# tatsy/opengl-raytracer

Measured on AMD Instinct MI355X. Metric: Mrays/s at 1920x1080, 8 bounces, higher is better.
Workload: dtype f32

## Files before the change

opengl-raytracer_amd/csrc/glrtx.hip:

```cpp
#include "glrtx.h"

#include <hip/hip_runtime.h>

#include <algorithm>
#include <cmath>
#include <cstdarg>
#include <cstdio>
#include <cstdlib>
#include <cstring>
#include <new>
#include <limits>
#include <string>
#include <vector>

#include "glrt_host.h"
#include "pt_kernel.hip.h"
#include "accumulate.hip.h"
#include "lbvh.hip.h"
#include "sahl.hip.h"
#include "refit.hip.h"
#include "query.hip.h"
#include "features.hip.h"
#include "denoise.hip.h"
#include "variance.hip.h"
// ... 1012 lines not shown
    k.fn = kWgwfKernels[trav][k.adapt][L.req.count_rays(c)];
    k.name = kWgwfNames[k.vol ? 2 : k.vine ? 0 : 1][k.adapt];
    k.lds = wgwf_lds_base(c) + (k.compact ? c->sc.n_crank * (int)sizeof(uint2) : 0);
    if (k.lds > 160 * 1024) return fail(c, GLRTX_EDEVICE, "wgwf kernel needs %d B of LDS (> 160 KiB)", k.lds);
    if (k.lds > 64 * 1024) HIP_TRY(c, hipFuncSetAttribute((const void *)k.fn, hipFuncAttributeMaxDynamicSharedMemorySize, k.lds));
    k.per_cu = 0;
    HIP_TRY(c, hipOccupancyMaxActiveBlocksPerMultiprocessor(&k.per_cu, k.fn, kBlockThreads, k.lds));
    k.per_cu = std::max(1, std::min(k.per_cu, GLRTX_WGWF_WAVES));
    if (const char *v = std::getenv("GLRTX_WGS_PER_CU")) k.per_cu = std::max(1, std::min(k.per_cu, std::atoi(v)));
    k.wg_slots = (size_t)c->n_cu * (size_t)k.per_cu;
    return GLRTX_OK;
}

void wgwf_shape(const glrtx_ctx *c, const WgwfLaunch &L, bool overlapped, bool is_fed, int share, bool device_busy, int &block_paths, int &grid) {
    const int n_frames = L.n_frames, fed_cap = L.f.fed_cap, n_samples = L.p->n_samples;
    const size_t total = L.total;
    const int resident = std::max(1, L.k.per_cu / std::max(share, 1)) * c->n_cu;
    const size_t work = total * (size_t)(is_fed ? std::max(n_frames, std::min(16, fed_cap)) : n_frames);
    block_paths = kWgPathsMax;
    if (overlapped && device_busy) { block_paths = 256; while (block_paths < kWgPathsMax && (size_t)resident * block_paths < work) block_paths *= 2; }
    else {
        const size_t tenths = (n_samples > 1 || (n_frames == 1 && !is_fed)) ? 39 : 19;
        while (block_paths > 512 && work * 10 < tenths * (size_t)resident * block_paths) block_paths /= 2;
        while (block_paths > 256 && work < (size_t)resident * block_paths) block_paths /= 2;
    }
    if (const char *v = std::getenv("GLRTX_BLOCK_PATHS")) { const int x = std::atoi(v); if (x >= 256 && x <= kWgPathsMax && (x & (x - 1)) == 0) block_paths = x; }
    grid = std::max(1, (int)std::min<size_t>((size_t)resident, (work + block_paths - 1) / block_paths));
}

int wgwf_pipe_slot(glrtx_ctx *c, WgwfLaunch &L) {
    WgwfLaunch::Form &f = L.f;
    const int n_frames = L.n_frames;
    const size_t frame_bytes = L.frame_bytes;
    glrtx_ctx::PipeSlot *&slot = L.slot = nullptr;
    int &pipe_busy = L.pipe_busy = 0, &block_paths = L.block_paths = 0, &grid = L.grid = 0;
    if (f.piped) {
        const bool fed = f.fed, busy = f.busy;
        wgwf_shape(c, L, !fed, fed, 1, busy, block_paths, grid);
        size_t slot_state_entries = (size_t)grid * block_paths;
        if (!fed) { int b2 = 0, g2 = 0; wgwf_shape(c, L, true, false, 1, !busy, b2, g2); slot_state_entries = std::max(slot_state_entries, (size_t)g2 * b2); }
        const size_t per_slot = (fed ? 0 : (size_t)kWfStatePlanes * slot_state_entries * sizeof(float4)) + (size_t)grid * kWgQueueF4 * sizeof(float4) + (fed ? 0 : frame_bytes);
        unsigned allowed = (unsigned)std::min<size_t>(c->pipe_slots, frames_budget(c) / std::max<size_t>(per_slot, 1));
        if (fed) allowed = std::min(allowed, kFedSlots);
        c->st.pipe_slots = (int32_t)allowed;
        if (allowed >= 1) {
            unsigned pick = c->pipe_next % allowed;
            for (unsigned k = 0; k < allowed; k++) {
                glrtx_ctx::PipeSlot &o = c->pipe[(c->pipe_next + k) % allowed];
                if (!o.used || hipEventQuery(o.acc_done) == hipSuccess) { pick = (c->pipe_next + k) % allowed; break; }
            }
            (void)hipGetLastError();
            c->pipe_next = pick + 1;
            slot = &c->pipe[pick];
            for (unsigned k = 0; k < kPipeSlots; k++)
                if (k != pick && c->pipe[k].used && hipEventQuery(c->pipe[k].render_done) == hipErrorNotReady) pipe_busy++;
            (void)hipGetLastError();
            if (c->pipe_share > 1 && pipe_busy > 0 && !fed) wgwf_shape(c, L, true, false, c->pipe_share, busy, block_paths, grid);
            bool ok = true;
            if (fed && slot->used) (void)hipEventSynchronize(slot->render_done);
            if (fed && slot->chunk_bytes != frame_bytes) {
                if (slot->used) (void)hipEventSynchronize(slot->acc_done);
                for (auto &ch : slot->chunks) dev_free(ch);
                std::memset(slot->feed_h->chunks, 0, sizeof slot->feed_h->chunks);
                slot->chunk_bytes = frame_bytes;
            }
            if (!fed) ok = ok && ensure(c, slot->state, (size_t)kWfStatePlanes * slot_state_entries * sizeof(float4)) == GLRTX_OK;
            ok = ok && ensure(c, slot->queues, (size_t)grid * kWgQueueF4 * sizeof(float4)) == GLRTX_OK;
            if (fed) ok = ok && ensure(c, slot->feed_d, sizeof(FeedDev)) == GLRTX_OK && feed_ensure_chunks(c, *slot, 0, n_frames, f.fed_cap, frame_bytes) == GLRTX_OK;
            else ok = ok && ensure(c, slot->planes, frame_bytes) == GLRTX_OK;
            if (!ok) {
                (void)hipGetLastError();
                c->err.clear();
                if (slot->used) (void)hipEventSynchronize(slot->acc_done);
                for (unsigned k = pick; k < kPipeSlots; k++) {
                    glrtx_ctx::PipeSlot &o = c->pipe[k];
                    if (o.used) (void)hipEventSynchronize(o.acc_done);
                    dev_free(o.state); dev_free(o.planes); dev_free(o.queues); dev_free(o.feed_d);
                    for (auto &ch : o.chunks) dev_free(ch);
                    if (o.feed_h) std::memset(o.feed_h->chunks, 0, sizeof o.feed_h->chunks);
                    o.chunk_bytes = 0;
                    o.used = false;
                }
                (void)hipGetLastError();
                c->pipe_slots = pick;
                if (pick == 0) c->pipeline = false;
                c->st.pipe_slots = (int32_t)pick;
                slot = nullptr;
                pipe_busy = 0;
            }
        }
        if (!slot) { f.piped = false; f.fed = false; }
    }
    if (!slot) {
        if (n_frames > frames_cap(c, L.p, 1)) return fail(c, GLRTX_ENOMEM, "glrtx_render_frames: %d frames exceed the frames-in-flight memory budget", n_frames);
        wgwf_shape(c, L, false, false, 1, f.busy, block_paths, grid);
    }
    if (slot) c->st.pipe_resident_max = std::max<int32_t>(c->st.pipe_resident_max, pipe_busy + 1);
    return GLRTX_OK;
}

int wgwf_args(glrtx_ctx *c, WgwfLaunch &L) {
    const glrtx_params *p = L.p;
    glrtx_ctx::PipeSlot *const slot = L.slot;
    const bool fed = L.f.fed, adapt = L.k.adapt, moments = L.req.kind == RenderReq::Moments;
    const int n_frames = L.n_frames, grid = L.grid;
    int rc;
    L.ctx_state = !slot || fed;
    L.stateBuf = L.ctx_state ? &c->wfState : &slot->state;
    L.queueBuf = slot ? &slot->queues : &c->wfQ;
    L.planeBuf = slot ? &slot->planes : &c->wfPlanes;
    L.workPtr = (unsigned *)(slot ? slot->work.p : c->work.p);
    L.rstream = slot ? slot->stream : c->stream;
    L.state_entries = (size_t)grid * (size_t)L.block_paths;
    L.state_bytes = (size_t)kWfStatePlanes * L.state_entries * sizeof(float4);
    if ((rc = ensure(c, *L.stateBuf, L.state_bytes))) return rc;
    if ((rc = ensure(c, *L.queueBuf, (size_t)grid * kWgQueueF4 * sizeof(float4)))) return rc;
    WfArgs &w = L.w;
    std::memset(&w, 0, sizeof w);
    w.state = (float4 *)L.stateBuf->p;
    w.ids = L.state_entries;
    c->st.wf_state_mib = (int32_t)((L.state_bytes + ((size_t)1 << 20) - 1) >> 20);
    w.total = (int)L.total;
    w.tiles8_x = L.tiles8_x;
    w.refill_min = kRefillMin;
    if (const char *v = std::getenv("GLRTX_REFILL_MIN")) w.refill_min = std::max(1, std::min(64, std::atoi(v)));
    w.n_frames = fed ? std::max(L.f.fed_cap, 2) : n_frames;
    w.tiles_per_frame = (int)(L.total >> 6);
    if (fed) {
        FeedHost *fh = slot->feed_h;
        for (int i = 0; i < n_frames; i++) fh->seeds[i] = make_float2(L.seeds_xy[2 * i], L.seeds_xy[2 * i + 1]);
        __atomic_store_n(&fh->frames_pub, (unsigned)n_frames, __ATOMIC_RELEASE);
        w.feed_host = slot->feed_h_dev;
        w.feed_dev = (FeedDev *)slot->feed_d.p;
        w.feed_plane_f4 = L.plane_f4;
        w.feed_margin = 64 * 4 * grid;
        if (const char *v = std::getenv("GLRTX_FEED_MARGIN")) w.feed_margin = std::max(0, std::atoi(v));
    } else {
        if (n_frames > 1) {
            if ((rc = ensure(c, c->wfSeeds, (size_t)n_frames * sizeof(float2)))) return rc;
            HIP_TRY(c, hipMemcpyAsync(c->wfSeeds.p, L.seeds_xy, (size_t)n_frames * sizeof(float2), hipMemcpyHostToDevice, c->stream));
            w.seeds = (const float2 *)c->wfSeeds.p;
            w.seeds_in_lds = n_frames <= kLdsSeeds ? 1 : 0;
        }
        if (n_frames > 1 || slot || adapt || moments) {
            if ((rc = ensure(c, *L.planeBuf, (size_t)std::max(L.n_planes, 1) * L.plane_f4 * sizeof(float4)))) return rc;
            w.planes = (float4 *)L.planeBuf->p;
        }
    }
    w.block_paths = L.block_paths;
    w.gss_div = (slot && !fed) ? 0 : 4 * grid;
    if (const char *v = std::getenv("GLRTX_GSS_DIV")) w.gss_div = std::max(0, std::atoi(v));
    w.suspend_max = kSuspendMax;
    if (const char *v = std::getenv("GLRTX_SUSPEND_MAX")) w.suspend_max = std::max(0, std::min(64, std::atoi(v)));
    w.trip_limit = (int)std::min<long long>(INT32_MAX, 64ll * std::max(p->n_samples, 1) * (p->max_depth + 2) + 64);
    if (L.k.vol) w.trip_limit = (int)std::min<long long>(INT32_MAX, 64ll * std::max(p->n_samples, 1) * 9 * (p->max_depth + 2) + 64);
    if (const char *v = std::getenv("GLRTX_TRIP_LIMIT")) w.trip_limit = std::max(1, std::atoi(v));
    w.err = c->guard_dev;
    return GLRTX_OK;
}

int wgwf_check(glrtx_ctx *c, const WgwfLaunch &L) {
    const glrtx_params *p = L.p;
    const glrtx_ctx::PipeSlot *const slot = L.slot;
    const WfArgs &w = L.w;
    const bool fed = L.f.fed, moments = L.req.kind == RenderReq::Moments;
    const int n_frames = L.n_frames, grid = L.grid, block_paths = L.block_paths, fed_cap = L.f.fed_cap;
    const size_t state_entries = L.state_entries, total = L.total, max_id = L.ids - 1;
    const size_t max_sidx = (size_t)kWfSetPlanes * state_entries + (size_t)grid * block_paths - 1;
    const size_t slice_f4 = 2 * (size_t)2 * 2 * block_paths  + (2 * (size_t)block_paths * sizeof(unsigned) + 15) / 16 ;
    static_assert(kWgSuspendAt + (size_t)kSuspendF4 * kBlockThreads == kWgQueueF4, "the suspend area closes a workgroup's slice");
    bool ok = slice_f4 <= kWgSuspendAt && max_id < (size_t)WF_INVALID && 2 * max_sidx + 1 < (size_t)WF_INVALID && (size_t)grid * block_paths <= state_entries &&
              (size_t)kWfStatePlanes * state_entries * sizeof(float4) < ((size_t)1 << 32) && (block_paths & (block_paths - 1)) == 0 && block_paths >= 256 &&
              block_paths <= kWgPathsMax && slice_f4 <= kWgQueueF4 && L.queueBuf->bytes >= (size_t)grid * kWgQueueF4 * sizeof(float4) &&
              L.stateBuf->bytes >= L.state_bytes && w.ids == state_entries && grid >= 1 && (size_t)grid <= L.k.wg_slots &&
              p->max_depth <= kWfDepthMax && p->n_samples <= kWfSampleMax && L.workPtr != nullptr;
    if (L.k.vol) ok = ok && p->n_samples <= kWfVolSampleMax && c->ext_flags == GLRTX_EXT_VOLUME && c->have_volume && c->vol.density != nullptr &&
                      c->vol.temperature != nullptr && c->n_spheres == 0 && !L.k.vine && L.k.fetch == 0 && !L.k.compact;
    if (!fed && n_frames > 1) ok = ok && c->wfSeeds.bytes >= (size_t)n_frames * sizeof(float2);
    if (w.planes) ok = ok && L.planeBuf->bytes >= (size_t)std::max(L.n_planes, 1) * L.plane_f4 * sizeof(float4);
    if (L.k.adapt) ok = ok && !fed && !slot && w.planes && c->ad_selected && c->ad_tiles == (int)(total >> 6) && c->adList.bytes >= (total >> 6) * sizeof(int) &&
                        c->adMask.bytes >= (total >> 6) && c->adHalf.bytes >= (size_t)c->ad_pitch * c->owned_rows && c->ad_pitch == c->pitch_bytes;
    if (moments) ok = ok && !fed && !slot && w.planes && c->mmM.p && c->mm_pitch == c->pitch_bytes && c->mm_rows == c->owned_rows &&
                      c->mmM.bytes >= c->pitch_bytes * (size_t)c->owned_rows;
    if (fed) ok = ok && n_frames >= 1 && n_frames <= fed_cap && fed_cap <= kFeedMaxFrames && slot->feed_d.bytes >= sizeof(FeedDev) && w.feed_host != nullptr &&
                  slot->chunks[(n_frames - 1) / kFeedChunkFrames].p != nullptr && slot->chunk_bytes == L.frame_bytes;
    if (!ok) return fail(c, GLRTX_EDEVICE, "internal: wgwf launch shapes inconsistent (ids %zu, max id %zu, grid %d of %zu slots (%d per CU), block_paths %d, frames %d, fed %d)", L.ids, max_id,
                         grid, L.k.wg_slots, L.k.per_cu, block_paths, n_frames, (int)fed);
    return GLRTX_OK;
}

template <class Src, class Sink>
void accumulate_launch(glrtx_ctx *c, const accumulate::Image &im, const Src &src, const Sink &sink) {
    hipLaunchKernelGGL(accumulate::entry(src, sink), dim3((im.width + 63) / 64, (im.rows + 3) / 4), dim3(256), 0, c->stream, im, src, sink);
}

int wgwf_issue(glrtx_ctx *c, const WgwfLaunch &L) {
    const glrtx_params *p = L.p;
    glrtx_ctx::PipeSlot *const slot = L.slot;
    const WfArgs &w = L.w;
    const bool fed = L.f.fed, adapt = L.k.adapt, vol = L.k.vol;
    const int n_frames = L.n_frames, n_planes = L.n_planes;
    const hipStream_t rstream = L.rstream;
    glrtx_ctx::LaunchRec *rec = nullptr;
    int rc;
    if ((rc = next_launch_rec(c, rec))) return rc;
    if (slot && slot->used) HIP_TRY(c, hipStreamWaitEvent(rstream, slot->acc_done, 0));
    if (L.ctx_state && c->state_used) HIP_TRY(c, hipStreamWaitEvent(rstream, c->state_done, 0));
    HIP_TRY(c, hipMemsetAsync(L.workPtr, 0, sizeof(unsigned), rstream));
    if (fed) {
        hipLaunchKernelGGL(feed_prefill_kernel, dim3(1), dim3(64), 0, rstream, (FeedDev *)slot->feed_d.p, (const FeedHost *)slot->feed_h_dev, n_frames);
        HIP_TRY(c, hipGetLastError());
    }
    HIP_TRY(c, hipEventRecord(rec->ev0, rstream));
    c->last_kernel = L.k.name;
    c->counters_stale = c->counters_stale || L.req.count_rays(c);
    const VolArgs va = vol ? c->vol : VolArgs{};
    hipLaunchKernelGGL(L.k.fn, dim3(L.grid), dim3(kBlockThreads), L.k.lds, rstream, L.a, w, L.workPtr, (float4 *)L.queueBuf->p, adapt ? (const int *)c->adList.p : nullptr,
                       adapt ? (const unsigned *)c->adCount.p : nullptr, va);
    HIP_TRY(c, hipGetLastError());
#ifdef GLRTX_RAY_LOG
    g_dbg_last = {L.a, w, L.k.lds, L.grid, (float4 *)L.queueBuf->p, L.k.fetch};
#endif
    HIP_TRY(c, hipEventRecord(rec->evm, rstream));
    if (L.ctx_state) { HIP_TRY(c, hipEventRecord(c->state_done, rstream)); c->state_used = true; }
    if (slot) {
        HIP_TRY(c, hipEventRecord(slot->render_done, rstream));
        HIP_TRY(c, hipStreamWaitEvent(c->stream, slot->render_done, 0));
        HIP_TRY(c, hipEventRecord(rec->eva, c->stream));
    }
    rec->has_eva = slot != nullptr;
    const bool pres = L.req.presents(c);
    const bool pres_fused = pres && (fed || w.planes);
    if (pres_fused && (rc = present_pass_begin(c))) return rc;
    {
        const accumulate::Image im{L.a.accum, L.a.pitch_f4, c->width, c->owned_rows};
        const accumulate::Planes flat{(const float4 *)L.planeBuf->p, n_frames, p->n_samples};
        const accumulate::Fed feed{fed ? (const FeedDev *)slot->feed_d.p : nullptr, p->n_samples};
        const glrtx_ctx::Present &P = c->pres;
        const accumulate::Present ring{(uchar4 *)P.dev.p, (size_t)c->width * (size_t)c->owned_rows, P.ring, pres ? (int)(P.seq % (uint64_t)P.ring) : 0, P.inv_gamma, P.flip};
        if (adapt) accumulate_launch(c, im, flat, accumulate::Half{(float4 *)c->adHalf.p, (const unsigned char *)c->adMask.p, L.tiles8_x});
        else if (L.req.kind == RenderReq::Moments) { if (n_planes > 0) accumulate_launch(c, im, flat, accumulate::Moments{(float4 *)c->mmM.p}); }
        else if (fed && pres) accumulate_launch(c, im, feed, ring);
        else if (fed) accumulate_launch(c, im, feed, accumulate::None{});
        else if (w.planes && pres) accumulate_launch(c, im, flat, ring);
        else if (w.planes && n_planes > 0) accumulate_launch(c, im, flat, accumulate::None{});
        HIP_TRY(c, hipGetLastError());
    }
    if (pres_fused && (rc = present_pass_end(c, n_frames))) return rc;
    if (slot) { HIP_TRY(c, hipEventRecord(slot->acc_done, c->stream)); slot->used = true; }
    HIP_TRY(c, hipEventRecord(rec->ev1, c->stream));
    rec->kernel = c->last_kernel; rec->frames = n_frames;
    c->ring_head++;
    c->st.frames_last = n_frames;
    c->st.paths += (uint64_t)c->owned_rows * (uint64_t)c->width * (uint64_t)p->n_samples * (uint64_t)n_frames;
    c->last_render_done = slot ? slot->render_done : c->state_done;
    if (fed) {
        c->open.slot = slot; c->open.p = *p; c->open.frames = n_frames; c->open.cap = L.f.fed_cap; c->open.rec = rec; c->open.frame_bytes = L.frame_bytes; c->open.vol = vol;
        c->st.feed_launches++;
    } else c->open.slot = nullptr;
    if (pres && !pres_fused) return present_resolve(c);
    return GLRTX_OK;
}

int launch_wgwf(glrtx_ctx *c, const KernelArgs &a, const glrtx_params *p, const RenderReq &req) {
    WgwfLaunch L{};
    L.p = p; L.req = req; L.a = a; L.n_frames = req.n_frames;
    L.seeds_xy = req.n_frames == 1 ? p->seed : req.seeds;
    L.tiles8_x = (c->width + 7) / 8;
    L.total = (size_t)L.tiles8_x * ((c->owned_rows + 7) / 8) * 64;
    if (L.total * 2 >= (size_t)INT32_MAX) return fail(c, GLRTX_EINVAL, "image too large for the wgwf variant");
    L.plane_f4 = (size_t)a.pitch_f4 * (size_t)c->owned_rows;
    L.plane_bytes = L.plane_f4 * sizeof(float4);
    L.frame_bytes = (size_t)std::max(p->n_samples, 1) * L.plane_bytes;
    L.n_planes = L.n_frames * p->n_samples;
    L.f = wgwf_form(c, L);
    L.ids = L.total * (size_t)(L.f.fed ? L.f.fed_cap : L.n_frames);
    if (L.ids + 1 >= (size_t)UINT32_MAX) return fail(c, GLRTX_EINVAL, "glrtx_render_frames: %d frames of %zu pixels exceed the 32-bit ray id space", L.n_frames, L.total);
    if (int rc = wgwf_kernel(c, L)) return rc;
    if (int rc = wgwf_pipe_slot(c, L)) return rc;
    if (int rc = wgwf_args(c, L)) return rc;
    if (int rc = wgwf_check(c, L)) return rc;
    return wgwf_issue(c, L);
}


void denoise_release(glrtx_ctx *c) {
    dev_free(c->ftN); dev_free(c->ftA); dev_free(c->ftCounter); dev_free(c->dnP[0]); dev_free(c->dnP[1]); dev_free(c->dnD);
    c->ft_w = 0; c->ft_rows = -1; c->dn_have = false;
    dev_free(c->ftN_spare); dev_free(c->ftA_spare); dev_free(c->accum_spare); dev_free(c->rpCount);
    c->rp_have = false;
    dev_free(c->ftG); dev_free(c->ftG_spare);
    c->mt_g_have = false;
    for (DevBuf &v : c->dnV) dev_free(v);
}

struct FilterCfg { int iterations; float sigma_c, sigma_normal, sigma_depth; int demodulate; };
FilterCfg filter_cfg(const glrtx_denoise_cfg &k) { return {k.iterations, k.sigma_color, k.sigma_normal, k.sigma_depth, k.demodulate}; }
FilterCfg filter_cfg(const glrtx_denoise_var_cfg &k) { return {k.iterations, k.sigma_lum, k.sigma_normal, k.sigma_depth, k.demodulate}; }

template <class Cfg>
int denoise_cfg_check(glrtx_ctx *c, const Cfg *cfg, const char *fn, FilterCfg &k) {
    if (!cfg) return fail(c, GLRTX_EINVAL, "%s: NULL cfg", fn);
    k = filter_cfg(*cfg);
    if (k.iterations < 1 || k.iterations > 6) return fail(c, GLRTX_EINVAL, "%s: iterations %d outside 1..6", fn, k.iterations);
    const float sg[3] = {k.sigma_c, k.sigma_normal, k.sigma_depth};
    for (float v : sg)
// ... 1921 lines not shown
    const glrtx_stats st_was = c->st;
    if ((rc = ensure(c, hist, n_rec * sizeof(unsigned))) == GLRTX_OK && (rc = ensure(c, scratch, c->pitch_bytes * (size_t)c->owned_rows)) == GLRTX_OK) {
        hipError_t e = hipMemsetAsync(hist.p, 0, n_rec * sizeof(unsigned), c->stream);
        if (e == hipSuccess) e = hipMemsetAsync(scratch.p, 0, c->pitch_bytes * (size_t)c->owned_rows, c->stream);
        if (e != hipSuccess) rc = fail(c, GLRTX_EDEVICE, "glrtx_hit_histogram: %s", hipGetErrorString(e));
        if (rc == GLRTX_OK) {
            rc = render_one(c, p, RenderReq{RenderReq::Calibration, nullptr, 1, (unsigned *)hist.p, (float4 *)scratch.p});
            seal_feed(c);
            if (rc == GLRTX_OK) rc = glrtx_sync(c);
        }
        if (rc == GLRTX_OK) {
            std::vector<unsigned> h(n_rec);
            if (hipMemcpy(h.data(), hist.p, n_rec * sizeof(unsigned), hipMemcpyDeviceToHost) != hipSuccess) rc = fail(c, GLRTX_EDEVICE, "glrtx_hit_histogram: read-back failed");
            else {
                std::fill(hist_out, hist_out + n_tri, 0u);
                for (size_t k = 0; k + 1 < n_rec; k++) hist_out[c->leaf_tri[k]] += h[k + 1];
            }
        }
    }
    dev_free(hist); dev_free(scratch);
    c->st = st_was;
    return rc;
}

int glrtx_get_stats(const glrtx_ctx *c, glrtx_stats *out) {
    if (!c || !out) return GLRTX_EINVAL;
    int dev_before = -1;
    const bool have_dev = hipGetDevice(&dev_before) == hipSuccess;
    if (hipSetDevice(c->device) == hipSuccess) (void)fold_launches(const_cast<glrtx_ctx *>(c), false);
    *out = c->st;
    if (c->counters_stale && c->counter.p && hipSetDevice(c->device) == hipSuccess &&
        hipMemcpy(c->counters_host, c->counter.p, sizeof c->counters_host, hipMemcpyDeviceToHost) == hipSuccess)
        c->counters_stale = false;
    out->rays = c->counters_host[0]; out->rays_untraced = c->counters_host[1];
    out->shadow_limited = c->sc.shadow_limited;
    if (have_dev && dev_before != c->device) (void)hipSetDevice(dev_before);
    return GLRTX_OK;
}

int glrtx_reset_stats(glrtx_ctx *c) {
    if (!c) return GLRTX_EINVAL;
    seal_feed(c);
    if (int rc = glrtx_sync(c)) return rc;
    HIP_TRY(c, hipMemset(c->counter.p, 0, 2 * sizeof(unsigned long long)));
    c->counters_host[0] = c->counters_host[1] = 0; c->counters_stale = false;
    c->st.rays = 0; c->st.rays_untraced = 0; c->st.paths = 0; c->st.launches = 0; c->st.kernel_launches = 0; c->st.kernel_ms_total = 0.0; c->st.accumulate_ms_total = 0.0; c->st.kernel_ms_last = 0.f; c->st.fallback_launches = 0; c->st.pipe_resident_max = 0; c->st.feed_launches = 0; c->st.feed_appended = 0;
    return GLRTX_OK;
}

int glrtx_present_enable(glrtx_ctx *c, int ring_images, float gamma, int flip_y) {
    if (!c) return GLRTX_EINVAL;
    return present_start(c, ring_images, gamma, flip_y, false);
}

int glrtx_present_acquire(glrtx_ctx *c, int wait, glrtx_image *out) {
    if (!c || !out) return GLRTX_EINVAL;
    glrtx_ctx::Present &P = c->pres;
    if (P.ring == 0) return fail(c, GLRTX_EINVAL, "glrtx_present_acquire: presentation is off (glrtx_present_enable)");
    if (P.acq == P.seq) { P.st.busy_returns++; return fail(c, GLRTX_EBUSY, "glrtx_present_acquire: no frame rendered since the last image was acquired"); }
    glrtx_ctx::Present::Image &im = P.img[P.acq % P.ring];
    HIP_TRY(c, hipSetDevice(c->device));
    const hipError_t e = wait ? hipEventSynchronize(im.ev) : hipEventQuery(im.ev);
    if (e == hipErrorNotReady) { (void)hipGetLastError(); P.st.busy_returns++; return fail(c, GLRTX_EBUSY, "glrtx_present_acquire: the next image is not ready"); }
    if (e != hipSuccess) return fail(c, GLRTX_EDEVICE, "glrtx_present_acquire: the image's copy failed: %s", hipGetErrorString(e));
    im.state = glrtx_ctx::Present::Image::HELD;
    P.acq++;
    P.st.delivered++;
    out->rgba = im.host;
    out->pitch_bytes = (size_t)im.width * 4;
    out->width = im.width;
    out->rows = im.rows;
    out->frame = im.frame;
    return GLRTX_OK;
}

int glrtx_present_release(glrtx_ctx *c, const glrtx_image *img) {
    if (!c || !img) return GLRTX_EINVAL;
    for (auto &im : c->pres.img)
        if (im.state == glrtx_ctx::Present::Image::HELD && im.host == img->rgba) { im.state = glrtx_ctx::Present::Image::FREE; return GLRTX_OK; }
    return fail(c, GLRTX_EINVAL, "glrtx_present_release: not an acquired image of this context");
}

int glrtx_present_get_stats(const glrtx_ctx *c, glrtx_present_stats *out) {
    if (!c || !out) return GLRTX_EINVAL;
    glrtx_ctx::Present &P = const_cast<glrtx_ctx *>(c)->pres;
    if (P.timed && P.t1) {
        int dev_before = -1;
        const bool have_dev = hipGetDevice(&dev_before) == hipSuccess;
        if (hipSetDevice(c->device) == hipSuccess && hipEventQuery(P.t1) == hipSuccess) {
            float ms = 0.f;
            if (hipEventElapsedTime(&ms, P.t0, P.t1) == hipSuccess) P.st.pass_ms_last = ms;
            P.timed = false;
        }
        (void)hipGetLastError();
        if (have_dev && dev_before != c->device) (void)hipSetDevice(dev_before);
    }
    *out = P.st;
    out->ring_images = P.ring;
    out->pending = (int32_t)(P.seq - P.acq);
    out->held = 0;
    for (const auto &im : P.img) out->held += im.state == glrtx_ctx::Present::Image::HELD;
    out->copies_last = P.copies_last;
    return GLRTX_OK;
}

#ifdef GLRTX_TRAV_STATS
int glrtx_debug_trav_stats(unsigned long long out[8]) { return take_symbol(g_trav_stats, out); }
int glrtx_debug_trav_trips(unsigned long long out[4]) { return take_symbol(g_trav_trips, out); }
int glrtx_debug_trav_sp_hist(unsigned long long out[16]) { return take_symbol(g_trav_sp_hist, out); }
int glrtx_debug_trav_hist(unsigned long long out[16]) { return take_symbol(g_trav_hist, out); }
#endif

#ifdef GLRTX_RAY_LOG
int glrtx_debug_ray_log_begin(glrtx_ctx *c, unsigned long long max_rays, unsigned max_trips) {
    if (!c) return GLRTX_EINVAL;
    HIP_TRY(c, hipSetDevice(c->device));
    int rc;
    if ((rc = ensure(c, g_dbg_log_rays, (size_t)max_rays * 2 * sizeof(float4)))) return rc;
    if ((rc = ensure(c, g_dbg_log_trips, (size_t)max_trips * sizeof(uint2)))) return rc;
    RayLog lg{(float4 *)g_dbg_log_rays.p, (uint2 *)g_dbg_log_trips.p, max_rays, max_trips, max_rays > 0 ? 1u : 0u};
    unsigned long long z = 0; unsigned zt = 0;
    HIP_TRY(c, hipMemcpyToSymbol(HIP_SYMBOL(g_ray_log), &lg, sizeof lg));
    HIP_TRY(c, hipMemcpyToSymbol(HIP_SYMBOL(g_ray_log_n), &z, sizeof z));
    HIP_TRY(c, hipMemcpyToSymbol(HIP_SYMBOL(g_ray_log_trips), &zt, sizeof zt));
    return GLRTX_OK;
}
int glrtx_debug_ray_log_copy(glrtx_ctx *c, float *rays_host, unsigned long long n_records, unsigned *trips_host, unsigned n_trips, int to_device) {
    if (!c) return GLRTX_EINVAL;
    if (int rc = glrtx_sync(c)) return rc;
    if ((size_t)n_records * 32 > g_dbg_log_rays.bytes || (size_t)n_trips * 8 > g_dbg_log_trips.bytes) return fail(c, GLRTX_EINVAL, "ray log: copy larger than the log");
    if (rays_host) HIP_TRY(c, to_device ? hipMemcpy(g_dbg_log_rays.p, rays_host, (size_t)n_records * 32, hipMemcpyHostToDevice)
                                        : hipMemcpy(rays_host, g_dbg_log_rays.p, (size_t)n_records * 32, hipMemcpyDeviceToHost));
    if (trips_host) HIP_TRY(c, to_device ? hipMemcpy(g_dbg_log_trips.p, trips_host, (size_t)n_trips * 8, hipMemcpyHostToDevice)
                                         : hipMemcpy(trips_host, g_dbg_log_trips.p, (size_t)n_trips * 8, hipMemcpyDeviceToHost));
    return GLRTX_OK;
}
int glrtx_debug_ray_log_replay(glrtx_ctx *c, int reps, double out[4]) {
    if (!c) return GLRTX_EINVAL;
    if (int rc = glrtx_sync(c)) return rc;
    RayLog lg{};
    unsigned long long n = 0; unsigned nt = 0;
    HIP_TRY(c, hipMemcpyFromSymbol(&lg, HIP_SYMBOL(g_ray_log), sizeof lg));
    HIP_TRY(c, hipMemcpyFromSymbol(&n, HIP_SYMBOL(g_ray_log_n), sizeof n));
    HIP_TRY(c, hipMemcpyFromSymbol(&nt, HIP_SYMBOL(g_ray_log_trips), sizeof nt));
    lg.on = 0u;
    HIP_TRY(c, hipMemcpyToSymbol(HIP_SYMBOL(g_ray_log), &lg, sizeof lg));
    nt = std::min(nt, lg.cap_trips);
    std::vector<uint2> tr(nt);
    HIP_TRY(c, hipMemcpy(tr.data(), lg.trips, (size_t)nt * sizeof(uint2), hipMemcpyDeviceToHost));
    unsigned long long logged = 0;
    for (const uint2 &t : tr) logged += t.y;
    DbgLastLaunch L = g_dbg_last;
    L.w.suspend_max = 0;
    using RKernel = void (*)(const KernelArgs, const WfArgs, unsigned *, float4 *, const float4 *, const uint2 *, int);
    int fetch = L.fetch;
    if (const char *v = std::getenv("GLRTX_REPLAY_PAIR_FETCH")) fetch = std::max(0, std::min(2, std::atoi(v)));
    const RKernel rk = fetch == 2 ? (RKernel)pt_replay_traverse<2> : fetch == 1 ? (RKernel)pt_replay_traverse<1> : (RKernel)pt_replay_traverse<0>;
    if (L.lds > 64 * 1024) HIP_TRY(c, hipFuncSetAttribute((const void *)rk, hipFuncAttributeMaxDynamicSharedMemorySize, L.lds));
    int per_cu = 0;
    HIP_TRY(c, hipOccupancyMaxActiveBlocksPerMultiprocessor(&per_cu, rk, kBlockThreads, L.lds));
    if (const char *v = std::getenv("GLRTX_WGS_PER_CU")) per_cu = std::max(1, std::min(per_cu, std::atoi(v)));
    const int grid = std::max(1, std::min(L.grid, per_cu * c->n_cu));
    float ms = 0.f;
    for (int r = 0; r < reps; r++) {
        HIP_TRY(c, hipMemsetAsync(c->work.p, 0, sizeof(unsigned), c->stream));
        HIP_TRY(c, hipEventRecord(c->tm0, c->stream));
        hipLaunchKernelGGL(rk, dim3(grid), dim3(kBlockThreads), L.lds, c->stream, L.a, L.w, (unsigned *)c->work.p, L.queues,
                           (const float4 *)lg.rays, (const uint2 *)lg.trips, (int)nt);
        HIP_TRY(c, hipGetLastError());
        HIP_TRY(c, hipEventRecord(c->tm1, c->stream));
        HIP_TRY(c, hipEventSynchronize(c->tm1));
        HIP_TRY(c, hipEventElapsedTime(&ms, c->tm0, c->tm1));
    }
    out[0] = ms; out[1] = (double)logged; out[2] = (double)nt; out[3] = (double)n;
    return GLRTX_OK;
}
#endif

#ifdef GLRTX_STEP_TIMING
int glrtx_debug_step_timing(unsigned long long out[4]) { return take_symbol(g_step_timing, out); }
#endif

#ifdef GLRTX_PHASE_STATS
int glrtx_debug_trip_log(unsigned out[16 * 64 * 4]) { return take_symbol(g_trip_log, out); }
int glrtx_debug_phase_cycles(unsigned long long out[8]) { return take_symbol(g_phase_cycles, out); }
#endif

int glrtx_timer_begin(glrtx_ctx *c) {
    if (!c) return GLRTX_EINVAL;
    seal_feed(c);
    HIP_TRY(c, hipSetDevice(c->device));
    HIP_TRY(c, hipEventRecord(c->tm0, c->stream));
    return GLRTX_OK;
}

int glrtx_timer_end(glrtx_ctx *c, float *ms) {
    if (!c || !ms) return GLRTX_EINVAL;
    seal_feed(c);
    HIP_TRY(c, hipSetDevice(c->device));
    HIP_TRY(c, hipEventRecord(c->tm1, c->stream));
    HIP_TRY(c, hipEventSynchronize(c->tm1));
    HIP_TRY(c, hipEventElapsedTime(ms, c->tm0, c->tm1));
    return GLRTX_OK;
}

}

struct glrtx_group {
    std::vector<glrtx_ctx *> ctx;
    std::vector<hipEvent_t> done;
    DevBuf full, full8;
    std::vector<char> peer_ok;
    int gather_copies = 0;
    int width = 0, height = 0;
    std::vector<uint8_t *> pres_host;
    std::vector<size_t> pres_bytes;
    std::string err;
};

namespace {

int gfail(glrtx_group *g, int code, const char *fmt, ...) {
    char buf[512];
    va_list ap;
    va_start(ap, fmt);
    vsnprintf(buf, sizeof buf, fmt, ap);
    va_end(ap);
    if (g) g->err = buf; else g_create_error = buf;
    return code;
}
int gsub(glrtx_group *g, int i, int rc) {
    if (rc != GLRTX_OK) g->err = "context " + std::to_string(i) + " (device " + std::to_string(g->ctx[i]->device) + "): " + g->ctx[i]->err;
    return rc;
}
#define GHIP_TRY(g, call)                                                                       \
    do {                                                                                        \
        hipError_t e_ = (call);                                                                 \
        if (e_ != hipSuccess) return gfail(g, GLRTX_EDEVICE, "%s failed: %s", #call, hipGetErrorString(e_)); \
    } while (0)

int group_gather(glrtx_group *g) {
    for (glrtx_ctx *m : g->ctx) seal_feed(m);
    glrtx_ctx *r = g->ctx[0];
    if (g->width < 1) return gfail(g, GLRTX_EINVAL, "glrtx_group: call glrtx_group_resize first");
    const size_t pitch = r->pitch_bytes;
    GHIP_TRY(g, hipSetDevice(r->device));
    if (g->full.bytes < pitch * (size_t)g->height) {
        dev_free(g->full);
        GHIP_TRY(g, hipMalloc(&g->full.p, pitch * (size_t)g->height));
        g->full.bytes = pitch * (size_t)g->height;
    }
    const int n = (int)g->ctx.size();
    g->gather_copies = 0;
    for (int i = 0; i < n; i++) {
        glrtx_ctx *c = g->ctx[i];
        if (c->pitch_bytes != pitch) return gfail(g, GLRTX_EINVAL, "glrtx_group: member accumulators have different pitches");
        if (c->owned_rows == 0) continue;
        const size_t stripe_b = (size_t)c->stripe * pitch;
        const int full_stripes = c->owned_rows / c->stripe, tail_rows = c->owned_rows % c->stripe;
        char *dst0 = (char *)g->full.p + (size_t)c->rank * stripe_b;
        if (g->peer_ok[i]) {
            GHIP_TRY(g, hipSetDevice(c->device));
            if (full_stripes > 0) {
                GHIP_TRY(g, hipMemcpy2DAsync(dst0, (size_t)c->world * stripe_b, c->accum, stripe_b, stripe_b, (size_t)full_stripes, hipMemcpyDeviceToDevice, c->stream));
                g->gather_copies++;
            }
            if (tail_rows > 0) {
                GHIP_TRY(g, hipMemcpyAsync(dst0 + (size_t)full_stripes * c->world * stripe_b, (const char *)c->accum + (size_t)full_stripes * stripe_b,
                                           (size_t)tail_rows * pitch, hipMemcpyDeviceToDevice, c->stream));
                g->gather_copies++;
            }
            GHIP_TRY(g, hipEventRecord(g->done[i], c->stream));
            GHIP_TRY(g, hipSetDevice(r->device));
            GHIP_TRY(g, hipStreamWaitEvent(r->stream, g->done[i], 0));
        } else {
            GHIP_TRY(g, hipSetDevice(c->device));
            GHIP_TRY(g, hipEventRecord(g->done[i], c->stream));
            GHIP_TRY(g, hipSetDevice(r->device));
            GHIP_TRY(g, hipStreamWaitEvent(r->stream, g->done[i], 0));
            for (int row = 0; row < c->owned_rows; row += c->stripe) {
                const int rows = std::min(c->stripe, c->owned_rows - row);
                const int y = ((row / c->stripe) * c->world + c->rank) * c->stripe;
                GHIP_TRY(g, hipMemcpyPeerAsync((char *)g->full.p + (size_t)y * pitch, r->device, (const char *)c->accum + (size_t)row * pitch, c->device,
                                               (size_t)rows * pitch, r->stream));
                g->gather_copies++;
            }
        }
    }
    return GLRTX_OK;
}

int group_present_prepare(glrtx_group *g, int n) {
    if (g->pres_host.empty() || n < 1) return GLRTX_OK;
    for (size_t i = 0; i < g->ctx.size(); i++)
        if (int rc = gsub(g, (int)i, present_prepare(g->ctx[i], n))) return rc;
    glrtx_ctx::Present &P0 = g->ctx[0]->pres;
    const size_t bytes = std::max<size_t>((size_t)g->width * 4 * (size_t)g->height, 64);
    for (int k = 0; k < n; k++) {
        const size_t at = (size_t)((P0.seq + k) % (uint64_t)P0.ring);
        if (g->pres_bytes[at] >= bytes) continue;
        if (g->pres_host[at]) GHIP_TRY(g, hipHostFree(g->pres_host[at]));
        g->pres_host[at] = nullptr; g->pres_bytes[at] = 0;
        GHIP_TRY(g, hipHostMalloc((void **)&g->pres_host[at], bytes, hipHostMallocPortable));
        g->pres_bytes[at] = bytes;
        for (glrtx_ctx *m : g->ctx) m->pres.img[at].host = g->pres_host[at];
    }
// ... 281 lines not shown
```

opengl-raytracer_amd/csrc/pt_kernel.hip.h:

```cpp
#pragma once
#include <hip/hip_runtime.h>
#include <stdint.h>

#include "trav_asm.hip.h"
#include "scan_asm.hip.h"

namespace glrtx {

constexpr int kBlockThreads = 256;
constexpr int kTile = 16;
constexpr int REF_ABSENT = INT32_MIN;
constexpr int REF_FIN = INT32_MIN;
constexpr int kMaxLdsMaterials = 256;
constexpr int kMaxLdsLights = 64;
constexpr int kTopForks = 128;

constexpr float PT_EPS = 1.0e-4f;
constexpr float PT_INFTY = 1.0e8f;
constexpr float PT_PI = 3.14159274101257324f;
constexpr float PT_2PI = 6.28318548202514648f;

struct DevScene {
    const float4 *forks;
    const float4 *nodes0;
// ... 266 lines not shown
    m = __builtin_fmaxf(m, __builtin_fmaf(dist, GLRTX_SHADOW_REL, dist));
    return limited ? fmin_c(m, PT_INFTY) : PT_INFTY;
}

struct Trav {
    float ox, oy, oz, dx, dy, dz, ix, iy, iz;
    Hit h;
    float stop_d;
    int cur, sp;
#ifdef GLRTX_TRAV_STATS
    unsigned iters;
#endif
};

DEV bool trav_init(const DevScene &sc, const float4 *root, Trav &T, float ox, float oy, float oz, float dx, float dy, float dz,
                   float limit = PT_INFTY, float stop_d = -__builtin_inff()) {
    T.ox = ox; T.oy = oy; T.oz = oz; T.dx = dx; T.dy = dy; T.dz = dz;
    T.ix = frcp(dx); T.iy = frcp(dy); T.iz = frcp(dz);
    T.h.t = limit; T.h.tri = -1; T.h.u = 0.f; T.h.v = 0.f;
    T.stop_d = stop_d;
    T.sp = 0;
    T.cur = sc.root_ref;
#ifdef GLRTX_TRAV_STATS
    T.iters = 0;
#endif
    if (sc.root_boxed) {
        float t0;
        if (!box_pass(root[0], root[1], ox, oy, oz, T.ix, T.iy, T.iz, T.h.t, t0)) return false;
    }
    return true;
}

template <bool CLOSEST, bool COMPACT = false, bool ANY = false>
DEV bool trav_step(const DevScene &sc, int *stack, Trav &T, const uint2 *ranks = nullptr, float tmin = PT_EPS) {
#ifdef GLRTX_TRAV_STATS
    trav_stats_iter(T.cur, (const void *)(sc.forks + 4 * (ptrdiff_t)T.cur), T.stop_d == -__builtin_inff(), T.sp);
    T.iters++;
#define TS_DONE atomicAdd(&g_trav_hist[T.iters <= 1 ? 0 : (32 - __clz((int)T.iters - 1)) > 15 ? 15 : (32 - __clz((int)T.iters - 1))], 1ull)
#else
#define TS_DONE
#endif
    const int cur = T.cur;
    bool need_pop = true;
    uint2 rw = make_uint2(0u, 0u);
    if constexpr (COMPACT) rw = ranks[(unsigned)cur >> 5];
    const bool is_fork = COMPACT ? ((rw.x >> ((unsigned)cur & 31u)) & 1u) != 0u : cur >= 0;
    const float4 *N = COMPACT ? sc.cnodes + 3 * (size_t)(unsigned)cur
                              : reinterpret_cast<const float4 *>(reinterpret_cast<const char *>(sc.nodes0) + ((unsigned)cur * 64u + sc.node_bias));
    float4 A, B, C, D;
    if constexpr (COMPACT) {
        A = N[0]; B = N[1]; C = N[2];
        asm volatile("" : "+v"(A.w), "+v"(B.w), "+v"(C.w));
        D = make_float4(A.w, B.w, C.w, 0.f);
    } else {
        A = N[0]; B = N[1]; C = N[2]; D = N[3];
        asm volatile("" : "+v"(A.w), "+v"(B.w), "+v"(D.x), "+v"(D.y), "+v"(D.z));
    }
    if (is_fork) {
        int l = __float_as_int(A.w), r = __float_as_int(B.w);
        if constexpr (COMPACT) {
            const unsigned rank = rw.y + (unsigned)__popc(rw.x & ((1u << ((unsigned)cur & 31u)) - 1u));
            l = (int)(2u * rank + 1u);
            r = l + 1;
        }
        float t0l, t0r;
        const bool bl = box_pass(A, B, T.ox, T.oy, T.oz, T.ix, T.iy, T.iz, T.h.t, t0l);
        const bool br = box_pass(C, D, T.ox, T.oy, T.oz, T.ix, T.iy, T.iz, T.h.t, t0r);
        const bool pl = bl;
        const bool pr = br;
        if (pl && pr) {
            reinterpret_cast<int2 *>(stack)[T.sp * kBlockThreads] = make_int2(__float_as_int(t0l), l);
            T.sp++;
        }
        T.cur = pr ? r : l;
        need_pop = !(pl || pr);
    }
    if (!is_fork) {
        const int t = COMPACT ? __float_as_int(A.w) : ~cur;
        const float tx = T.ox - A.x, ty = T.oy - A.y, tz = T.oz - A.z;
        const float px = T.dy * C.z - T.dz * C.y;
        const float py = T.dz * C.x - T.dx * C.z;
        const float pz = T.dx * C.y - T.dy * C.x;
        const float det = dot3(B.x, B.y, B.z, px, py, pz);
        const float U = dot3(tx, ty, tz, px, py, pz);
        const float inv = rcp_newton(det);
        const float u = U * inv;
        const float qx = ty * B.z - tz * B.y;
        const float qy = tz * B.x - tx * B.z;
        const float qz = tx * B.y - ty * B.x;
        const float V = dot3(T.dx, T.dy, T.dz, qx, qy, qz);
        const float v = V * inv;
        const float tt = dot3(C.x, C.y, C.z, qx, qy, qz) * inv;
        const bool hit = !(-PT_EPS < det && det < PT_EPS) && !(u < 0.0f || 1.0f < u) &&
                         !(v < 0.0f || 1.0f < inv * (U + V)) &&
                         !(tmin >= tt);
        const bool closer = hit && tt < T.h.t;
        T.h.tri = closer ? t : T.h.tri;
        if (CLOSEST) { T.h.u = closer ? u : T.h.u; T.h.v = closer ? v : T.h.v; }
        T.h.t = closer ? tt : T.h.t;
        const bool stopped = ANY ? closer : T.stop_d - T.h.t >= PT_EPS;
        const int next = __float_as_int(B.w);
        T.cur = stopped ? REF_FIN : next;
        need_pop = !stopped && next == REF_FIN;
    }
    if (need_pop) {
        float t0;
        int sp = T.sp, ref = REF_FIN;
        unsigned long long save;
        unsigned addr;
        const unsigned lds_base = (unsigned)(uintptr_t)stack;
        asm volatile(
            "s_mov_b64 %[save], exec\n"
            "1:\n\t"
            "v_cmp_ne_u32 vcc, 0, %[sp]\n\t"
            "v_cndmask_b32 %[ref], %[fin], %[ref], vcc\n\t"
            "s_and_b64 exec, exec, vcc\n\t"
            "s_cbranch_execz 2f\n\t"
            "v_add_u32 %[sp], -1, %[sp]\n\t"
            "v_lshl_add_u32 %[addr], %[sp], 11, %[base]\n\t"
            "ds_read_b32 %[ref], %[addr] offset:4\n\t"
            "ds_read_b32 %[t0], %[addr]\n\t"
            "s_waitcnt lgkmcnt(0)\n\t"
            "v_cmp_gt_f32 vcc, %[t0], %[th]\n\t"
            "s_and_b64 exec, exec, vcc\n\t"
            "s_cbranch_execnz 1b\n"
            "2:\n\t"
            "s_mov_b64 exec, %[save]"
            : [t0] "=&v"(t0), [ref] "+&v"(ref), [sp] "+&v"(sp), [save] "=&s"(save), [addr] "=&v"(addr)
            : [base] "v"(lds_base), [th] "v"(T.h.t), [fin] "v"(REF_FIN)
            : "vcc", "scc", "memory");
        static_assert(kBlockThreads * 8 == 1 << 11, "the pop loop shifts the stack index by 11: entry e of lane l at byte (e * kBlockThreads + l) * 8");
        T.sp = sp;
        T.cur = ref;
    }
#ifdef GLRTX_TRAV_STATS
    if (T.cur == REF_FIN) { TS_DONE; }
#endif
    return T.cur == REF_FIN;
}

#ifdef GLRTX_STEP_TIMING
__device__ unsigned long long g_step_timing[4];
struct StepTiming { unsigned t = 0, w = 0, n = 0; };
#define GLRTX_TS_PARAM , StepTiming &ST
#define GLRTX_TS_OPERANDS , [tt] "+&v"(ST.t), [tw] "+&v"(ST.w), [tn] "+&v"(ST.n)
#define GLRTX_TS_CLOBBERS , "s90", "s91", "s92", "s93", "s94", "s95"
#else
#define GLRTX_TS_PARAM
#define GLRTX_TS_OPERANDS
#define GLRTX_TS_CLOBBERS
#endif
constexpr int kWgwfCompact = 8;
constexpr int kWgwfVolume = 16;
template <int FETCH>
DEV void trav_steps_asm(const DevScene &sc, int *stack, Trav &T, unsigned rk GLRTX_TS_PARAM) {
    unsigned long long s_entry, s_act, s_leaf, s_bl, s_br, s_pop, s_tmp;
    const unsigned stk = (unsigned)(uintptr_t)stack;
    static_assert(kBlockThreads * 8 == 1 << 11, "trav_asm.hip.h shifts the stack index by 11: entry e of lane l at byte (e * kBlockThreads + l) * 8");
    static_assert(REF_FIN == INT32_MIN, "trav_asm.hip.h materialises REF_FIN with v_bfrev_b32 v, 1");
    const unsigned par16 = (threadIdx.x & 1u) << 4;
    const unsigned bias_e = sc.node_bias + par16, bias_o = sc.node_bias + 16u - par16;
    if constexpr ((FETCH & kWgwfCompact) != 0) {
        static_assert((FETCH & ~kWgwfCompact) == 0, "the compact layout has the one-record-per-lane fetch only");
        asm volatile(
            "s_mov_b64 %[entry], exec\n\t"
            "s_mov_b64 %[act], exec\n\t"
            GLRTX_ASM_SET_VBASE
            "v_bfrev_b32 v[GLRTX_VB+22], 1\n\t"
            GLRTX_REP(GLRTX_STEPS_PER_TRIP, GLRTX_TRAV_STEP_ASM_COMPACT)
            "99:\n\t"
            "s_mov_b64 exec, %[entry]"
            : [th] "+&v"(T.h.t), [tri] "+&v"(T.h.tri), [hu] "+&v"(T.h.u), [hv] "+&v"(T.h.v), [cur] "+&v"(T.cur), [sp] "+&v"(T.sp),
              [entry] "=&s"(s_entry), [act] "=&s"(s_act), [leaf] "=&s"(s_leaf), [bl] "=&s"(s_bl), [br] "=&s"(s_br), [pop] "=&s"(s_pop), [tmp] "=&s"(s_tmp) GLRTX_TS_OPERANDS
            : [ox] "v"(T.ox), [oy] "v"(T.oy), [oz] "v"(T.oz), [dx] "v"(T.dx), [dy] "v"(T.dy), [dz] "v"(T.dz), [ix] "v"(T.ix), [iy] "v"(T.iy), [iz] "v"(T.iz),
              [sd] "v"(T.stop_d), [stk] "v"(stk), [cbase] "s"(sc.cnodes), [rk] "s"(rk), [eps] "s"(PT_EPS)
            : "vcc", "scc", "memory", GLRTX_ASM_VCLOBBERS_COMPACT GLRTX_TS_CLOBBERS);
        return;
    }
    if (FETCH == 2) {
        asm volatile(
            "s_mov_b64 %[entry], exec\n\t"
            "s_mov_b64 %[act], exec\n\t"
            GLRTX_ASM_SET_VBASE
            "v_bfrev_b32 v[GLRTX_VB+11], 1\n\t"
            GLRTX_REP(GLRTX_STEPS_PER_TRIP_HALF, GLRTX_TRAV_STEP_ASM_PAIR GLRTX_TRAV_STEP_ASM_LANE)
            "99:\n\t"
            "s_mov_b64 exec, %[entry]"
            : [th] "+&v"(T.h.t), [tri] "+&v"(T.h.tri), [hu] "+&v"(T.h.u), [hv] "+&v"(T.h.v), [cur] "+&v"(T.cur), [sp] "+&v"(T.sp),
              [entry] "=&s"(s_entry), [act] "=&s"(s_act), [leaf] "=&s"(s_leaf), [bl] "=&s"(s_bl), [br] "=&s"(s_br), [pop] "=&s"(s_pop), [tmp] "=&s"(s_tmp) GLRTX_TS_OPERANDS
            : [ox] "v"(T.ox), [oy] "v"(T.oy), [oz] "v"(T.oz), [dx] "v"(T.dx), [dy] "v"(T.dy), [dz] "v"(T.dz), [ix] "v"(T.ix), [iy] "v"(T.iy), [iz] "v"(T.iz),
              [sd] "v"(T.stop_d), [stk] "v"(stk), [base] "s"(sc.nodes0), [bias] "s"(sc.node_bias), [eps] "s"(PT_EPS),
              [odd] "s"(0xAAAAAAAAAAAAAAAAull), [biase] "v"(bias_e), [biaso] "v"(bias_o)
            : "vcc", "scc", "memory", GLRTX_ASM_VCLOBBERS_PAIR GLRTX_TS_CLOBBERS);
        return;
    }
    if (FETCH == 1) {
        asm volatile(
            "s_mov_b64 %[entry], exec\n\t"
            "s_mov_b64 %[act], exec\n\t"
            GLRTX_ASM_SET_VBASE
            "v_bfrev_b32 v[GLRTX_VB+11], 1\n\t"
            GLRTX_REP(GLRTX_STEPS_PER_TRIP, GLRTX_TRAV_STEP_ASM_PAIR)
            "99:\n\t"
            "s_mov_b64 exec, %[entry]"
            : [th] "+&v"(T.h.t), [tri] "+&v"(T.h.tri), [hu] "+&v"(T.h.u), [hv] "+&v"(T.h.v), [cur] "+&v"(T.cur), [sp] "+&v"(T.sp),
              [entry] "=&s"(s_entry), [act] "=&s"(s_act), [leaf] "=&s"(s_leaf), [bl] "=&s"(s_bl), [br] "=&s"(s_br), [pop] "=&s"(s_pop), [tmp] "=&s"(s_tmp) GLRTX_TS_OPERANDS
            : [ox] "v"(T.ox), [oy] "v"(T.oy), [oz] "v"(T.oz), [dx] "v"(T.dx), [dy] "v"(T.dy), [dz] "v"(T.dz), [ix] "v"(T.ix), [iy] "v"(T.iy), [iz] "v"(T.iz),
              [sd] "v"(T.stop_d), [stk] "v"(stk), [base] "s"(sc.nodes0), [eps] "s"(PT_EPS),
              [odd] "s"(0xAAAAAAAAAAAAAAAAull), [biase] "v"(bias_e), [biaso] "v"(bias_o)
            : "vcc", "scc", "memory", GLRTX_ASM_VCLOBBERS_PAIR GLRTX_TS_CLOBBERS);
        return;
    }
    asm volatile(
        "s_mov_b64 %[entry], exec\n\t"
        "s_mov_b64 %[act], exec\n\t"
        GLRTX_ASM_SET_VBASE
        "v_bfrev_b32 v[GLRTX_VB+11], 1\n\t"
        GLRTX_REP(GLRTX_STEPS_PER_TRIP, GLRTX_TRAV_STEP_ASM_LANE)
        "99:\n\t"
        "s_mov_b64 exec, %[entry]"
        : [th] "+&v"(T.h.t), [tri] "+&v"(T.h.tri), [hu] "+&v"(T.h.u), [hv] "+&v"(T.h.v), [cur] "+&v"(T.cur), [sp] "+&v"(T.sp),
          [entry] "=&s"(s_entry), [act] "=&s"(s_act), [leaf] "=&s"(s_leaf), [bl] "=&s"(s_bl), [br] "=&s"(s_br), [pop] "=&s"(s_pop), [tmp] "=&s"(s_tmp) GLRTX_TS_OPERANDS
        : [ox] "v"(T.ox), [oy] "v"(T.oy), [oz] "v"(T.oz), [dx] "v"(T.dx), [dy] "v"(T.dy), [dz] "v"(T.dz), [ix] "v"(T.ix), [iy] "v"(T.iy), [iz] "v"(T.iz),
          [sd] "v"(T.stop_d), [stk] "v"(stk), [base] "s"(sc.nodes0), [bias] "s"(sc.node_bias), [eps] "s"(PT_EPS)
        : "vcc", "scc", "memory", GLRTX_ASM_VCLOBBERS GLRTX_TS_CLOBBERS);
}

template <bool CLOSEST>
DEV void tri_test(Hit &h, int t, float ox, float oy, float oz, float dx, float dy, float dz, float v0x, float v0y, float v0z, float e1x,
                  float e1y, float e1z, float e2x, float e2y, float e2z, float tmin = PT_EPS) {
    const float tx = ox - v0x, ty = oy - v0y, tz = oz - v0z;
    const float px = dy * e2z - dz * e2y;
    const float py = dz * e2x - dx * e2z;
    const float pz = dx * e2y - dy * e2x;
    const float det = dot3(e1x, e1y, e1z, px, py, pz);
    const float U = dot3(tx, ty, tz, px, py, pz);
    const float inv = rcp_newton(det);
    const float u = U * inv;
    const bool ok_u = !(-PT_EPS < det && det < PT_EPS) && !(u < 0.0f || 1.0f < u);
    if (!__any(ok_u)) return;
    const float qx = ty * e1z - tz * e1y;
    const float qy = tz * e1x - tx * e1z;
    const float qz = tx * e1y - ty * e1x;
    const float V = dot3(dx, dy, dz, qx, qy, qz);
    const float v = V * inv;
    const bool ok_v = ok_u && !(v < 0.0f || 1.0f < inv * (U + V));
    if (!__any(ok_v)) return;
    const float tt = dot3(e2x, e2y, e2z, qx, qy, qz) * inv;
    const bool hit = ok_v && !(tmin >= tt);
    const bool closer = hit && tt < h.t;
    h.tri = closer ? t : h.tri;
    if (CLOSEST) { h.u = closer ? u : h.u; h.v = closer ? v : h.v; }
    h.t = hit ? __builtin_fminf(h.t, tt) : h.t;
}

template <bool CLOSEST, int QUERY = 0>
DEV Hit trav_scan(const DevScene &sc, float ox, float oy, float oz, float dx, float dy, float dz, bool valid,
              float limit = PT_INFTY, float stop_d = -__builtin_inff(), float tmin = PT_EPS) {
    Hit h;
    h.t = limit; h.tri = -1; h.u = 0.f; h.v = 0.f;
    const float ix = frcp(dx), iy = frcp(dy), iz = frcp(dz);
    bool alive = valid;
    float t0u = 0.f, t1u = 0.f;
    if (sc.vine_uniform) {
        const float4 lo = sc.vine[0], hi = sc.vine[1];
        const float fx = (hi.x - ox) * ix, fy = (hi.y - oy) * iy, fz = (hi.z - oz) * iz;
        const float nx = (lo.x - ox) * ix, ny = (lo.y - oy) * iy, nz = (lo.z - oz) * iz;
        t1u = __builtin_fminf(__builtin_fmaxf(fx, nx), __builtin_fminf(__builtin_fmaxf(fy, ny), __builtin_fmaxf(fz, nz)));
        t0u = __builtin_fmaxf(__builtin_fminf(fx, nx), __builtin_fmaxf(__builtin_fminf(fy, ny), __builtin_fminf(fz, nz)));
#ifndef GLRTX_SCAN_CXX
        if constexpr (QUERY == 0) {
        if (valid) {
            unsigned groups = (unsigned)sc.vine_main >> 2;
            unsigned long long s_entry, s_alive, s_tmp;
            asm volatile(GLRTX_SCAN_UNIFORM_ASM
                         : [th] "+&v"(h.t), [tri] "+&v"(h.tri), [hu] "+&v"(h.u), [hv] "+&v"(h.v), [grp] "+&s"(groups), [entry] "=&s"(s_entry), [alive] "=&s"(s_alive),
                           [tmp] "=&s"(s_tmp)
                         : [ox] "v"(ox), [oy] "v"(oy), [oz] "v"(oz), [dx] "v"(dx), [dy] "v"(dy), [dz] "v"(dz), [ix] "v"(ix), [iy] "v"(iy), [iz] "v"(iz), [sd] "v"(stop_d),
                           [t0u] "v"(t0u), [t1u] "v"(t1u), [ptr] "s"(sc.vine), [eps] "s"(PT_EPS)
                         : "vcc", "scc", "memory", GLRTX_ASM_VCLOBBERS, GLRTX_SCAN_SCLOBBERS);
        }
        return h;
        }
#endif
    }
    const int n = sc.n_vine, last_at = sc.vine_main;
    typedef float rec_t __attribute__((ext_vector_type(16)));
    auto issue = [&](rec_t &r, int i) { asm volatile("s_load_dwordx16 %0, %1, 0x0" : "=s"(r) : "s"(sc.vine + 4 * (size_t)(i < n - 1 ? i : last_at + (i - (n - 1)))) : "memory"); };
    auto pair_arrive = [&](rec_t &a, rec_t &b) { asm volatile("s_waitcnt lgkmcnt(0)" : "+s"(a), "+s"(b) : : "memory"); };
    auto step = [&](const rec_t &r, int i) {
        if (alive) {
            bool pass;
            if (sc.vine_uniform && i + 1 < n) pass = __builtin_fminf(t1u, h.t) >= t0u;
            else {
                float t0;
                pass = box_pass(make_float4(r[0], r[1], r[2], 0.f), make_float4(r[4], r[5], r[6], 0.f), ox, oy, oz, ix, iy, iz, h.t, t0);
            }
            alive = pass;
            if (pass) {
                tri_test<CLOSEST>(h, __float_as_int(r[15]), ox, oy, oz, dx, dy, dz, r[3], r[7], r[8], r[9], r[10], r[11], r[12], r[13], r[14], tmin);
                if (stop_d - h.t >= PT_EPS) alive = false;
                if (QUERY == 2 && h.tri >= 0) alive = false;
            }
        }
    };
    rec_t a0, a1, b0, b1;
    issue(a0, 0);
    issue(a1, 1);
    pair_arrive(a0, a1);
    for (int i = 0; i < n; i += 4) {
        if (!__any(alive)) break;
        issue(b0, i + 2);
        issue(b1, i + 3);
        step(a0, i);
        if (i + 1 < n) step(a1, i + 1);
// ... 695 lines not shown
            acc.y = acc.y + fmin_c(P.Ly, 100.0f);
            acc.z = acc.z + fmin_c(P.Lz, 100.0f);
            acc.w = acc.w + 1.0f;
        }
        *px = acc;
    }
    flush_rays<COUNT_RAYS>(a, rays);
}

constexpr int kChunk = 256;

struct PersistKernArgs {
    KernelArgs a;
    unsigned *work_counter;
    ExtArgs ex;
    VolArgs vol;
};
DEV const PersistKernArgs *persist_kernargs() {
    auto p = __builtin_amdgcn_kernarg_segment_ptr();
    asm volatile("" : "+s"(p));
    return (const PersistKernArgs *)p;
}

template <bool COUNT_RAYS, bool EXT = false, bool VOL = false>
__global__ __launch_bounds__(kBlockThreads) void pt_render_persistent(const KernelArgs a_entry, unsigned *work_counter_entry, const ExtArgs ex_entry,
                                                                      const VolArgs vol_entry) {
    extern __shared__ __attribute__((aligned(16))) unsigned char lds_raw[];
    float4 *lds_mats;
    int *stack;
    (void)work_counter_entry; (void)ex_entry; (void)vol_entry;
    static_assert(!VOL || EXT, "the volume kernel is an extension kernel");
    lds_setup(a_entry, lds_raw, lds_mats, stack);
    float4 *lds_spheres = nullptr;
    if (EXT) lds_spheres = ext_stage_spheres(a_entry, ex_entry, lds_raw);
    const KernelArgs &a = persist_kernargs()->a;

    const int lane = threadIdx.x & 63;
    const unsigned long long lt_mask = (1ull << lane) - 1ull;
    const int tiles8_x = (a.width + 7) >> 3, tiles8_y = (a.owned_rows + 7) >> 3;
    const int total = tiles8_x * tiles8_y * 64;

    int chunk_next = 0, chunk_end = 0;
    bool exhausted = false;
    bool alive = false, fresh = false;
    int px_off = 0, sample = 0;
    float fcx = 0.f, fcy = 0.f;
    Rng rng = {0.f, 0.f, a.seed_x, a.seed_y};
    float4 acc = make_float4(0.f, 0.f, 0.f, 0.f);
    Path P;
    path_begin(P, 0.f, 0.f, 0.f, 0.f, 0.f, 1.f);
    unsigned long long rays = 0;

    for (;;) {
        const PersistKernArgs *ka = persist_kernargs();
        const KernelArgs &a = ka->a;
        unsigned *const work_counter = ka->work_counter;
        unsigned long long idle = __ballot(!alive);
        while (idle != 0ull && !exhausted) {
            if (chunk_next >= chunk_end) {
                int base = 0;
                if (lane == 0) base = (int)atomicAdd(work_counter, (unsigned)kChunk);
                base = __builtin_amdgcn_readfirstlane(base);
                if (base >= total) { exhausted = true; break; }
                chunk_next = base;
                chunk_end = base + kChunk < total ? base + kChunk : total;
            }
            const int n = __popcll(idle);
            const int avail = chunk_end - chunk_next;
            const int take = n < avail ? n : avail;
            const int rank = __popcll(idle & lt_mask);
            if (!alive && rank < take) {
                const int id = chunk_next + rank;
                const int t = id >> 6, w = id & 63;
                const int lx = (t % tiles8_x) * 8 + (w & 7);
                const int lrow = (t / tiles8_x) * 8 + (w >> 3);
                if (lx < a.width && lrow < a.owned_rows && a.n_samples > 0) {
                    const int gy = local_row_to_y(a, lrow);
                    fcx = (float)lx + 0.5f; fcy = (float)gy + 0.5f;
                    rng.x = fcx / (float)a.width; rng.y = fcy / (float)a.height;
                    px_off = lrow * a.pitch_f4 + lx;
                    acc = a.accum[px_off];
                    sample = 0;
                    alive = true; fresh = true;
                }
            }
            chunk_next += take;
            idle = __ballot(!alive);
        }
        if (!__any(alive)) {
            if (exhausted) break;
            continue;
        }
        if (alive) {
            if (fresh) {
                camera_ray(a, a.cam, rng, fcx, fcy, P);
                fresh = false;
            }
            bool finished = true;
            if (a.max_depth > 0) {
                if (VOL) finished = bounce_ext<true>(a, ka->ex, lds_spheres, lds_mats, stack, rng, P, rays, &ka->vol);
                else finished = EXT ? bounce_ext(a, ka->ex, lds_spheres, lds_mats, stack, rng, P, rays) : bounce(a, lds_mats, stack, rng, P, rays);
            }
            if (finished) {
                acc.x = acc.x + fmin_c(P.Lx, 100.0f);
                acc.y = acc.y + fmin_c(P.Ly, 100.0f);
                acc.z = acc.z + fmin_c(P.Lz, 100.0f);
                acc.w = acc.w + 1.0f;
                sample++;
                if (sample >= a.n_samples) {
                    a.accum[px_off] = acc;
                    alive = false;
                } else {
                    fresh = true;
                }
            }
        }
    }
    flush_rays<COUNT_RAYS>(persist_kernargs()->a, rays);
}

constexpr int kFeedMaxFrames = 1024;
constexpr int kFeedChunkFrames = 16;
constexpr int kFeedChunks = kFeedMaxFrames / kFeedChunkFrames;
constexpr unsigned kFeedClosed = 0x80000000u;
struct FeedHost {
    unsigned frames_pub;
    unsigned pad[31];
    float2 seeds[kFeedMaxFrames];
    float4 *chunks[kFeedChunks];
};
struct FeedDev {
    unsigned frames_known;
    unsigned pad[31];
    unsigned long long seeds[kFeedMaxFrames];
    unsigned long long chunks[kFeedChunks];
};
constexpr int kCamFloatsPadded = 36;
constexpr int kLdsSeeds = 64;
constexpr int kWfSetPlanes = 6;
struct WfArgs {
    float4 *state;
    size_t ids;
    DEV size_t plane(int k) const { size_t n = ids; asm volatile("" : "+s"(n)); return (size_t)k * n; }
    DEV float4 *A(int k, unsigned sidx) const { return reinterpret_cast<float4 *>(reinterpret_cast<char *>(state + plane(k)) + (size_t)(sidx * 16u)); }
    DEV float4 *H(unsigned sidx) const { return A(5, sidx); }
    DEV unsigned set_base(int set, int wg) const { size_t n = ids; asm volatile("" : "+s"(n)); return (unsigned)((size_t)set * kWfSetPlanes * n) + (unsigned)wg * (unsigned)block_paths; }
    int total;
    int tiles8_x;
    int refill_min;
    int block_paths;
    int gss_div;
    int suspend_max;
    int trip_limit;
    unsigned *err;
    FeedHost *feed_host;
    FeedDev *feed_dev;
    size_t feed_plane_f4;
    int feed_margin;
    const float2 *seeds;
    int seeds_in_lds;
    float4 *planes;
    int n_frames;
    int tiles_per_frame;
    DEV void split(int id, int &frame, int &pid) const {
        if (n_frames > 1) { frame = (int)((unsigned)id / (unsigned)total); pid = id - frame * total; }
        else { frame = 0; pid = id; }
    }
};
constexpr int kWfStatePlanes = 2 * kWfSetPlanes;
constexpr int kWfDepthMax = 255;
constexpr int kWfSampleMax = (1 << 20) - 1;
constexpr int kWfVolSampleMax = (1 << 16) - 1;
constexpr unsigned kWfVolShift = 24;
constexpr unsigned kWfVolPassed = 9;
constexpr unsigned WF_PENDING = 1u << 28;
constexpr unsigned WF_FINISHING = 1u << 29;
constexpr unsigned WF_RESOLVED = 1u << 30;
constexpr unsigned WF_ACCEPTED = 1u << 31;
constexpr unsigned WF_INVALID = 0xFFFFFFFFu;
constexpr int kSuspendMax = 24;
constexpr float kHitSuspended = -1.0f;
constexpr int kSuspendF4 = 4;
constexpr int kRefillMin = 16;
#ifdef GLRTX_FAULT_INJECT
constexpr unsigned kFaultPoison = 0xFFFFFFFEu;
#endif

DEV bool wf_pixel(const KernelArgs &a, const WfArgs &w, int id, int &lx, int &lrow) {
    int frame, pid;
    w.split(id, frame, pid);
    const int t = pid >> 6, k = pid & 63;
    lx = (t % w.tiles8_x) * 8 + (k & 7);
    lrow = (t / w.tiles8_x) * 8 + (k >> 3);
    return lx < a.width && lrow < a.owned_rows;
}

DEV float2 wf_seed(const KernelArgs &a, const WfArgs &w, const float *cam, int id) {
    if (w.n_frames > 1) {
        int frame, pid;
        w.split(id, frame, pid);
        if (w.seeds_in_lds) {
            const float *sd = cam + kCamFloatsPadded + 2 * frame;
            return make_float2(sd[0], sd[1]);
        }
        if (w.feed_dev != nullptr) {
            const nfloat2 v = ((glb_cf2)&w.feed_dev->seeds[0])[frame];
            return make_float2(v.x, v.y);
        }
        const nfloat2 v = ((glb_cf2)w.seeds)[frame];
        return make_float2(v.x, v.y);
    }
    return make_float2(a.seed_x, a.seed_y);
}

DEV void wf_add_sample(const KernelArgs &a, const WfArgs &w, int id, int lx, int lrow, unsigned sample, float Lx, float Ly, float Lz) {
    if (w.feed_dev != nullptr) {
        int frame, pid;
        w.split(id, frame, pid);
        typedef __attribute__((address_space(1))) nfloat4 *glb_f4;
        const glb_f4 chunk = (glb_f4)w.feed_dev->chunks[frame / kFeedChunkFrames];
        const size_t slot = (size_t)(frame % kFeedChunkFrames) * (size_t)a.n_samples + sample;
        nfloat4 v; v.x = fmin_c(Lx, 100.0f); v.y = fmin_c(Ly, 100.0f); v.z = fmin_c(Lz, 100.0f); v.w = 1.0f;
        __builtin_nontemporal_store(v, &chunk[slot * w.feed_plane_f4 + (size_t)lrow * (size_t)a.pitch_f4 + lx]);
    } else if (w.planes != nullptr) {
        int frame, pid;
        w.split(id, frame, pid);
        const size_t slot = (size_t)frame * (size_t)a.n_samples + sample;
        st_stream(&w.planes[(slot * (size_t)a.owned_rows + (size_t)lrow) * (size_t)a.pitch_f4 + lx],
                  make_float4(fmin_c(Lx, 100.0f), fmin_c(Ly, 100.0f), fmin_c(Lz, 100.0f), 1.0f));
    } else {
        float4 *px = a.accum + (size_t)lrow * a.pitch_f4 + lx;
        float4 acc = *px;
        acc.x = acc.x + fmin_c(Lx, 100.0f);
        acc.y = acc.y + fmin_c(Ly, 100.0f);
        acc.z = acc.z + fmin_c(Lz, 100.0f);
        acc.w = acc.w + 1.0f;
        *px = acc;
    }
}

DEV bool wf_start(const KernelArgs &a, const WfArgs &w, const float *cam, int id, int lx, int lrow, Rng &rng, float fcx, float fcy, Path &P, unsigned &sample) {
    for (;;) {
        if ((int)sample >= a.n_samples) return false;
        camera_ray(a, cam, rng, fcx, fcy, P);
        if (a.max_depth > 0) return true;
        wf_add_sample(a, w, id, lx, lrow, sample, 0.0f, 0.0f, 0.0f);
        sample++;
    }
}

DEV bool wf_generate_one(const KernelArgs &a, const WfArgs &w, const float *cam, int id, unsigned sidx, float4 &ray_o, float4 &ray_d) {
    int lx, lrow;
    bool go = false;
    const float2 sd = wf_seed(a, w, cam, id);
    Rng rng = {0.f, 0.f, sd.x, sd.y};
    Path P;
    unsigned sample = 0;
    if (wf_pixel(a, w, id, lx, lrow)) {
        const int gy = local_row_to_y(a, lrow);
        const float fcx = (float)lx + 0.5f, fcy = (float)gy + 0.5f;
        rng.x = fcx / (float)a.width; rng.y = fcy / (float)a.height;
        go = wf_start(a, w, cam, id, lx, lrow, rng, fcx, fcy, P, sample);
    }
    if (go) {
        st_stream(w.A(0, sidx), make_float4(P.ox, P.oy, P.oz, rng.x));
        st_stream(w.A(1, sidx), make_float4(P.dx, P.dy, P.dz, rng.y));
        st_stream(w.A(2, sidx), make_float4(1.f, 1.f, 1.f, __uint_as_float(sample << 8)));
        st_stream(w.A(3, sidx), make_float4(0.f, 0.f, 0.f, __uint_as_float((unsigned)id)));
        ray_o = make_float4(P.ox, P.oy, P.oz, __uint_as_float(sidx * 2u));
        ray_d = make_float4(P.dx, P.dy, P.dz, 0.f);
    } else st_stream(w.A(3, sidx), make_float4(0.f, 0.f, 0.f, __uint_as_float(WF_INVALID)));
    return go;
}

constexpr int kWfVolEnd = 0, kWfVolNext = 1, kWfVolExit = 2;
DEV const VolArgs *wgwf_vol();
DEV int wf_vol_trial(const KernelArgs &a, const WfArgs &w, unsigned sidx, Rng &rng, Path &P, const Hit &h, unsigned k) {
    if (h.tri < 0) { P.Lx = 1.0f; P.Ly = 0.0f; P.Lz = 1.0f; return kWfVolEnd; }
    const float ox = P.ox, oy = P.oy, oz = P.oz, dx = P.dx, dy = P.dy, dz = P.dz;
    float t = 0.0f;
    bool pass = false;
    for (int i = 0; i < 256; i++) {
        const VolArgs &vo = *wgwf_vol();
        const float dm = vo.density_max;
        t = t - lp_log(fmax_c(1.0f - pt_rand(rng), PT_EPS)) / (dm * VOL_SIGT);
        if (t >= h.t) { pass = true; break; }
        const float density = vol_lookup(vo.density, vo, ox + t * dx, oy + t * dy, oz + t * dz);
        if (density / dm > pt_rand(rng)) { pass = true; break; }
    }
    if (!pass) { P.Lx = 0.0f; P.Ly = 0.0f; P.Lz = 0.0f; return kWfVolEnd; }
    {
        unsigned si = sidx;
        asm volatile("" : "+v"(si));
        const float4 b = ld_stream(w.A(2, si)), l = ld_stream(w.A(3, si));
        P.bx = b.x; P.by = b.y; P.bz = b.z; P.Lx = l.x; P.Ly = l.y; P.Lz = l.z;
    }
    if (t >= h.t) {
        const float te = h.t + PT_EPS;
        P.ox = ox + te * dx; P.oy = oy + te * dy; P.oz = oz + te * dz;
    } else {
        P.ox = ox + t * dx; P.oy = oy + t * dy; P.oz = oz + t * dz;
        float R, G, B;
        const VolArgs &vo = *wgwf_vol();
        vol_blackbody(vol_lookup(vo.temperature, vo, P.ox, P.oy, P.oz), R, G, B);
        P.Lx = P.Lx + (P.bx * R) / VOL_SIGT; P.Ly = P.Ly + (P.by * G) / VOL_SIGT; P.Lz = P.Lz + (P.bz * B) / VOL_SIGT;
        const float theta = lp_acos(2.0f * pt_rand(rng) + -1.0f);
// ... 17 lines not shown
}

template <bool VOL = false>
DEV void wf_shade_path(const KernelArgs &a, const WfArgs &w, const float4 *lds_mats, const float *cam, unsigned &id, unsigned sidx, bool light_accepted, bool &push_ext,
                       bool &push_sh, bool &requeue, float4 &ray_o, float4 &ray_d, float4 &ray_sd, float4 &st2, float4 &st3, float4 &st4, bool &has4, unsigned long long &rays) {
    const float4 s0 = ld_stream(w.A(0, sidx)), s1 = ld_stream(w.A(1, sidx)), s2 = ld_stream(w.A(2, sidx)), s3 = ld_stream(w.A(3, sidx));
    const float4 hh = *w.H(sidx);
    id = __float_as_uint(s3.w);
    if (id == WF_INVALID) return;
    const float2 sd = wf_seed(a, w, cam, (int)id);
    Rng rng = {s0.w, s1.w, sd.x, sd.y};
    const unsigned meta = __float_as_uint(s2.w);
    unsigned sample = (meta >> 8) & (VOL ? (unsigned)kWfVolSampleMax : 0xFFFFFu);
    const unsigned vstate = VOL ? (meta >> kWfVolShift) & 0xFu : 0u;
    Path P;
    P.ox = s0.x; P.oy = s0.y; P.oz = s0.z; P.dx = s1.x; P.dy = s1.y; P.dz = s1.z;
    P.bx = s2.x; P.by = s2.y; P.bz = s2.z;
    P.depth = (int)(meta & 0xFFu);
    P.Lx = s3.x; P.Ly = s3.y; P.Lz = s3.z;
    if (meta & WF_RESOLVED) light_accepted = (meta & WF_ACCEPTED) != 0u;
    const bool rejected = (meta & WF_PENDING) != 0u && !light_accepted;
    float4 s4 = make_float4(0.f, 0.f, 0.f, 0.f);
    if (rejected) {
        s4 = ld_stream(w.A(4, sidx));
        P.Lx = s4.x; P.Ly = s4.y; P.Lz = s4.z;
    }
    bool ended = (meta & WF_FINISHING) != 0u;
    Shade sh;
    sh.has_shadow = false;
    bool vtrial = false;
    int vtrial_next = 0;
    if constexpr (VOL) {
        vtrial = vstate >= 1u && vstate <= 8u && hh.x != kHitSuspended;
        if (vtrial) {
            Hit h;
            h.t = hh.x; h.tri = __float_as_int(hh.y); h.u = hh.z; h.v = hh.w;
            const int r = wf_vol_trial(a, w, sidx, rng, P, h, vstate);
            vtrial_next = r == kWfVolNext ? (int)vstate + 1 : r == kWfVolExit ? (int)kWfVolPassed : 0;
        }
    }
    if (!ended) {
        if (hh.x == kHitSuspended) {
            unsigned m2 = meta;
            if ((meta & WF_PENDING) && !(meta & WF_RESOLVED)) m2 = meta | WF_RESOLVED | (light_accepted ? WF_ACCEPTED : 0u);
            ray_o = s0; ray_d = s1;
            st2 = make_float4(s2.x, s2.y, s2.z, __uint_as_float(m2));
            st3 = s3;
            st4 = s4;
            has4 = rejected;
            requeue = true;
            return;
        }
        Hit h;
        h.t = hh.x; h.tri = __float_as_int(hh.y); h.u = hh.z; h.v = hh.w;
        if (a.hit_hist != nullptr && h.tri >= 0) atomicAdd(&a.hit_hist[h.tri], 1u);
        if constexpr (VOL) {
            int vnext = -1;
            if (vtrial) {
                vnext = vtrial_next;
                if (vnext == 0) ended = true;
            } else if (h.tri >= 0) {
                const Surf S = surf_tri(a.sc, h);
                const Mat M = load_mat(a.sc, lds_mats, S.mtrl);
                const int type = __float_as_int(M.m0.w);
                if (type == 5 && (-(P.dz * S.nz) - (P.dy * S.ny)) - (P.dx * S.nx) >= PT_EPS) {
                    const float tt = h.t + PT_EPS;
                    P.ox = P.ox + tt * P.dx; P.oy = P.oy + tt * P.dy; P.oz = P.oz + tt * P.dz;
                    vnext = 1;
                } else if (vstate == kWfVolPassed) {
                    P.Lx = P.Lx + P.bx * M.m0.x; P.Ly = P.Ly + P.by * M.m0.y; P.Lz = P.Lz + P.bz * M.m0.z;
                }
            }
            if (vnext >= 0) {
                if (!ended) {
                    push_ext = true;
                    ray_o = make_float4(P.ox, P.oy, P.oz, rng.x);
                    ray_d = make_float4(P.dx, P.dy, P.dz, rng.y);
                    st2 = make_float4(P.bx, P.by, P.bz, __uint_as_float((unsigned)P.depth | (sample << 8) | ((unsigned)vnext << kWfVolShift)));
                    st3 = make_float4(P.Lx, P.Ly, P.Lz, s3.w);
                    return;
                }
            } else {
                shade_hit(a, lds_mats, rng, P, h, sh);
            }
        } else {
            shade_hit(a, lds_mats, rng, P, h, sh);
        }
        if (!(VOL && ended)) {
            if (sh.untraced) rays += (1ull << 32) + 1ull;
            if (sh.ended && !sh.has_shadow) { P.Lx = sh.Lpx; P.Ly = sh.Lpy; P.Lz = sh.Lpz; }
            ended = sh.ended && !sh.has_shadow;
        }
    }
    if (ended) {
        int lx, lrow;
        wf_pixel(a, w, (int)id, lx, lrow);
        const int gy = local_row_to_y(a, lrow);
        const float fcx = (float)lx + 0.5f, fcy = (float)gy + 0.5f;
        wf_add_sample(a, w, (int)id, lx, lrow, sample, P.Lx, P.Ly, P.Lz);
        sample++;
        push_ext = wf_start(a, w, cam, (int)id, lx, lrow, rng, fcx, fcy, P, sample);
        if (push_ext) {
            ray_o = make_float4(P.ox, P.oy, P.oz, rng.x);
            ray_d = make_float4(P.dx, P.dy, P.dz, rng.y);
            st2 = make_float4(1.f, 1.f, 1.f, __uint_as_float(sample << 8));
            st3 = make_float4(0.f, 0.f, 0.f, s3.w);
        }
    } else {
        push_sh = sh.has_shadow;
        push_ext = !sh.ended;
        const unsigned m2 = (unsigned)P.depth | (sample << 8) | (push_sh ? WF_PENDING : 0u) | (sh.ended ? WF_FINISHING : 0u);
        ray_o = make_float4(P.ox, P.oy, P.oz, rng.x);
        ray_d = make_float4(P.dx, P.dy, P.dz, rng.y);
        st2 = make_float4(P.bx, P.by, P.bz, __uint_as_float(m2));
        st3 = make_float4(sh.Lpx, sh.Lpy, sh.Lpz, s3.w);
        if (push_sh) { st4 = make_float4(sh.Lfx, sh.Lfy, sh.Lfz, 0.f); has4 = true; }
        ray_sd = make_float4(sh.sdx, sh.sdy, sh.sdz, sh.dist);
    }
}

#ifndef GLRTX_STEPS_PER_TRIP
#define GLRTX_STEPS_PER_TRIP 6
#endif
constexpr int kWgCtlWords = 32;
constexpr int kWgPathsMax = 4096;
constexpr size_t kWgSuspendAt = 8 * (size_t)kWgPathsMax + (size_t)kWgPathsMax / 2;
constexpr size_t kWgQueueF4 = kWgSuspendAt + (size_t)kSuspendF4 * kBlockThreads;
#ifndef GLRTX_PRIO_TRAVERSE
#define GLRTX_PRIO_TRAVERSE 3
#define GLRTX_PRIO_SHADE 0
#endif
#ifndef GLRTX_WGWF_WAVES
#define GLRTX_WGWF_WAVES 4
#endif

#ifdef GLRTX_PHASE_STATS
__device__ unsigned long long g_phase_cycles[8];
__device__ uint4 g_trip_log[16][64];
#define PH_STAMP(var) const unsigned long long var = __builtin_amdgcn_s_memtime()
#define PH_ADD(i, t0, t1) do { if (threadIdx.x == 0) atomicAdd(&g_phase_cycles[i], (t1) - (t0)); } while (0)
#else
#define PH_STAMP(var)
#define PH_ADD(i, t0, t1)
#endif

#ifdef GLRTX_RAY_LOG
struct RayLog { float4 *rays; uint2 *trips; unsigned long long cap_rays; unsigned cap_trips; unsigned on; };
__device__ RayLog g_ray_log;
__device__ unsigned long long g_ray_log_n;
__device__ unsigned g_ray_log_trips;
#endif

DEV int wgwf_suspend_max();

template <bool VINE, int FETCH>
DEV void wg_traverse_phase(const KernelArgs &a, const WfArgs &w, const float4 *root, int *stack, const float4 *rq, int n_rays,
                           unsigned *ray_head, unsigned *light_bits, unsigned long long &rays, float4 *suspend_area) {
    const int lane = threadIdx.x & 63;
    const uint2 *ranks = reinterpret_cast<const uint2 *>(light_bits + kWgPathsMax / 32);
    if (VINE) {
        for (;;) {
            int base = 0;
            if (lane == 0) base = (int)atomicAdd(ray_head, 64u);
            base = __builtin_amdgcn_readfirstlane(base);
            if (base >= n_rays) break;
            float4 o = make_float4(0.f, 0.f, 0.f, __uint_as_float(WF_INVALID)), d = o;
            if (base + lane < n_rays) { o = ld_stream(&rq[2 * (size_t)(base + lane)]); d = ld_stream(&rq[2 * (size_t)(base + lane) + 1]); }
            const unsigned r = __float_as_uint(o.w);
            const bool shadow = (r & 1u) != 0u;
            const Hit h = trav_scan<true>(a.sc, o.x, o.y, o.z, d.x, d.y, d.z, r != WF_INVALID, shadow ? shadow_limit(d.w, a.sc.shadow_limited) : PT_INFTY,
                                          shadow ? d.w : -__builtin_inff());
            if (r != WF_INVALID) {
                rays++;
                if (r & 1u) { if (nee_accepted(d.w, h.t, h.tri >= 0)) atomicOr(&light_bits[r >> 6], 1u << ((r >> 1) & 31u)); }
                else st_stream(w.H(r >> 1), make_float4(h.t, __int_as_float(h.tri), h.u, h.v));
            }
        }
        return;
    }
    const unsigned long long lt_mask = (1ull << lane) - 1ull;
    const float4 none = make_float4(0.f, 0.f, 0.f, __uint_as_float(WF_INVALID));
    float4 cur_o = none, cur_d = none;
    float cur_ix = 0.f, cur_iy = 0.f, cur_iz = 0.f;
    int cur_pos = 0, cur_cnt = 0;
    auto fetch = [&](float4 &o, float4 &d) -> int {
        int base = 0;
        if (lane == 0) base = (int)atomicAdd(ray_head, 64u);
        base = __builtin_amdgcn_readfirstlane(base);
        int cnt = n_rays - base;
        cnt = cnt < 0 ? 0 : (cnt > 64 ? 64 : cnt);
        if (lane < cnt) {
            o = ld_stream(&rq[2 * (size_t)(base + lane)]);
            d = ld_stream(&rq[2 * (size_t)(base + lane) + 1]);
            cur_ix = frcp(d.x); cur_iy = frcp(d.y); cur_iz = frcp(d.z);
            const bool shadow = (__float_as_uint(o.w) & 1u) != 0u;
            float t0;
            if (a.sc.root_boxed && !box_pass(root[0], root[1], o.x, o.y, o.z, cur_ix, cur_iy, cur_iz, shadow ? shadow_limit(d.w, a.sc.shadow_limited) : PT_INFTY, t0))
                d.w = __uint_as_float(__float_as_uint(d.w) | 0x80000000u);
        }
        return cnt;
    };
    cur_cnt = fetch(cur_o, cur_d);
    bool exhausted = cur_cnt == 0;
    const bool fetched_any = cur_cnt > 0;
    bool active = false;
    bool unsaved = false;
    unsigned rid = 0;
    Trav T;
    T.cur = 0; T.sp = 0;
    T.h.t = PT_INFTY; T.h.tri = -1; T.h.u = 0.f; T.h.v = 0.f;
#ifdef GLRTX_STEP_TIMING
    StepTiming step_timing;
#endif
    float4 *const susp = suspend_area + (size_t)kSuspendF4 * threadIdx.x;
    {
        const float4 s3 = susp[3];
        if (s3.z != 0.0f) {
            const float4 s0 = susp[0], s1 = susp[1], s2 = susp[2];
            susp[3] = make_float4(0.f, 0.f, 0.f, 0.f);
            T.ox = s0.x; T.oy = s0.y; T.oz = s0.z;
            rid = __float_as_uint(w.H(__float_as_uint(s0.w) >> 1)->y);
#ifdef GLRTX_FAULT_INJECT
            const bool fault_dropped = rid == kFaultPoison;
#endif
            T.dx = s1.x; T.dy = s1.y; T.dz = s1.z; T.stop_d = s1.w;
            T.ix = frcp(T.dx); T.iy = frcp(T.dy); T.iz = frcp(T.dz);
            T.h.t = s2.x; T.h.tri = __float_as_int(s2.y); T.h.u = s2.z; T.h.v = s2.w;
            T.cur = __float_as_int(s3.x); T.sp = __float_as_int(s3.y);
#ifdef GLRTX_TRAV_STATS
            T.iters = 0;
#endif
            active = true;
#ifdef GLRTX_FAULT_INJECT
            if (fault_dropped) active = false;
#endif
        }
    }
    auto save_hit = [&]() {
        const unsigned id = rid >> 1;
        if (rid & 1u) {
            if (nee_accepted(T.stop_d, T.h.t, T.h.tri >= 0)) atomicOr(&light_bits[id >> 5], 1u << (id & 31u));
        } else *w.H(id) = make_float4(T.h.t, __int_as_float(T.h.tri), T.h.u, T.h.v);
        unsaved = false;
    };
#ifdef GLRTX_PHASE_STATS
    unsigned long long ph_refill = 0ull, ph_refills = 0ull, ph_step = 0ull;
#endif
    for (;;) {
        unsigned long long idle = __ballot(!active);
        if ((int)__popcll(idle) >= w.refill_min || idle == ~0ull) {
#ifdef GLRTX_PHASE_STATS
            const unsigned long long rf0 = __builtin_amdgcn_s_memtime();
#endif
            while (idle != 0ull && !exhausted) {
                if (cur_pos >= cur_cnt) {
                    cur_cnt = cur_cnt == 64 ? fetch(cur_o, cur_d) : 0;
                    cur_pos = 0;
                    if (cur_cnt == 0) { exhausted = true; break; }
                }
                const int n = __popcll(idle);
                const int avail = cur_cnt - cur_pos;
                const int take = n < avail ? n : avail;
                const int rank = __popcll(idle & lt_mask);
                const int src = (cur_pos + rank) & 63;
                const float ox = __shfl(cur_o.x, src), oy = __shfl(cur_o.y, src), oz = __shfl(cur_o.z, src);
                const unsigned new_rid = (unsigned)__shfl((int)__float_as_uint(cur_o.w), src);
                const float dx = __shfl(cur_d.x, src), dy = __shfl(cur_d.y, src), dz = __shfl(cur_d.z, src);
                const float dist_m = __shfl(cur_d.w, src);
                const float ix = __shfl(cur_ix, src), iy = __shfl(cur_iy, src), iz = __shfl(cur_iz, src);
                if (!active && rank < take) {
                    if (unsaved) save_hit();
                    rid = new_rid;
                    if (rid != WF_INVALID) {
                        rays++;
                        const bool shadow = (rid & 1u) != 0u;
                        const float dist = __builtin_fabsf(dist_m);
                        T.ox = ox; T.oy = oy; T.oz = oz; T.dx = dx; T.dy = dy; T.dz = dz; T.ix = ix; T.iy = iy; T.iz = iz;
                        T.h.t = shadow ? shadow_limit(dist, a.sc.shadow_limited) : PT_INFTY; T.h.tri = -1; T.h.u = 0.f; T.h.v = 0.f;
                        T.stop_d = shadow ? dist : -__builtin_inff();
                        T.sp = 0;
                        T.cur = (FETCH & kWgwfCompact) ? 0 : a.sc.root_ref;
#ifdef GLRTX_TRAV_STATS
                        T.iters = 0;
#endif
                        active = (__float_as_uint(dist_m) & 0x80000000u) == 0u;
                        unsaved = !active;
                    }
                }
                cur_pos += take;
                idle = __ballot(!active);
            }
#ifdef GLRTX_PHASE_STATS
            ph_refill += __builtin_amdgcn_s_memtime() - rf0; ph_refills += 1ull;
#endif
        }
        if (!__any(active)) {
            if (exhausted) break;
            continue;
        }
        if (exhausted && fetched_any) {
            const unsigned long long ma = __ballot(active);
            const int suspend_max = wgwf_suspend_max();
            if (__ballot(active && (rid & 1u) != 0u) == 0ull && (int)__popcll(ma) <= suspend_max) {
                if (active) {
                    susp[0] = make_float4(T.ox, T.oy, T.oz, __uint_as_float(rid));
                    susp[1] = make_float4(T.dx, T.dy, T.dz, T.stop_d);
                    susp[2] = make_float4(T.h.t, __int_as_float(T.h.tri), T.h.u, T.h.v);
                    susp[3] = make_float4(__int_as_float(T.cur), __int_as_float(T.sp), 1.0f, 0.f);
                    float mark = kHitSuspended, zero = 0.f;
                    asm volatile("" : "+v"(mark), "+v"(zero));
                    *w.H(rid >> 1) = make_float4(mark, zero, zero, zero);
                    active = false;
                }
                break;
            }
        }
#ifdef GLRTX_PHASE_STATS
        const unsigned long long sb0 = __builtin_amdgcn_s_memtime();
#endif
#ifdef GLRTX_TRAV_STATS
        {
            const unsigned long long ma = __ballot(active);
            if (lane == 0) {
                atomicAdd(&g_trav_trips[0], 1ull); atomicAdd(&g_trav_trips[1], (unsigned long long)__popcll(ma));
                if (exhausted) { atomicAdd(&g_trav_trips[2], 1ull); atomicAdd(&g_trav_trips[3], (unsigned long long)__popcll(ma)); }
            }
        }
#endif
        if (active) {
#if defined(GLRTX_TRAV_STATS) || defined(GLRTX_CXX_STEP)
            constexpr bool CP = (FETCH & kWgwfCompact) != 0;
            bool fin = trav_step<true, CP>(a.sc, stack, T, ranks);
#pragma unroll
            for (int k = 1; k < GLRTX_STEPS_PER_TRIP; k++)
                if (!fin) fin = trav_step<true, CP>(a.sc, stack, T, ranks);
#else
#ifdef GLRTX_STEP_TIMING
            trav_steps_asm<FETCH>(a.sc, stack, T, (unsigned)(uintptr_t)ranks, step_timing);
#else
            trav_steps_asm<FETCH>(a.sc, stack, T, (unsigned)(uintptr_t)ranks);
#endif
            const bool fin = T.cur == REF_FIN;
#endif
            if (fin) {
                active = false;
                unsaved = true;
            }
        }
#ifdef GLRTX_PHASE_STATS
        ph_step += __builtin_amdgcn_s_memtime() - sb0;
#endif
    }
    if (unsaved) save_hit();
#ifdef GLRTX_PHASE_STATS
    if (threadIdx.x == 0) { atomicAdd(&g_phase_cycles[5], ph_refill); atomicAdd(&g_phase_cycles[6], ph_refills); atomicAdd(&g_phase_cycles[7], ph_step); }
#endif
#ifdef GLRTX_STEP_TIMING
    atomicAdd(&g_step_timing[0], (unsigned long long)step_timing.n);
    atomicAdd(&g_step_timing[1], (unsigned long long)step_timing.t);
    atomicAdd(&g_step_timing[2], (unsigned long long)step_timing.w);
#endif
}

template <bool VOL = false>
DEV void wg_shade_phase(const KernelArgs &a, const WfArgs &w, const float4 *lds_mats, const float *cam, const unsigned *light_bits, int n_paths,
                        float4 *rq_next, unsigned *n_rays_next, unsigned *n_paths_next, unsigned cur_base, unsigned next_base, unsigned long long &rays,
                        unsigned *moved) {
    const int lane = threadIdx.x & 63;
    const unsigned long long lt_mask = (1ull << lane) - 1ull;
    for (int j0 = 0; j0 < n_paths; j0 += kBlockThreads) {
        const int i = j0 + (int)threadIdx.x;
        bool push_ext = false, push_sh = false, requeue = false, has4 = false;
        unsigned id = WF_INVALID;
        float4 ro = make_float4(0.f, 0.f, 0.f, 0.f), rd = ro, rsd = ro, st2 = ro, st3 = ro, st4 = ro;
        const bool light_accepted = i < n_paths && ((light_bits[i >> 5] >> (i & 31)) & 1u) != 0u;
        if (i < n_paths)
            wf_shade_path<VOL>(a, w, lds_mats, cam, id, cur_base + (unsigned)i, light_accepted, push_ext, push_sh, requeue, ro, rd, rsd, st2, st3, st4, has4, rays);
        const unsigned long long me = __ballot(push_ext), ms = __ballot(push_sh), mq = __ballot(requeue), mp = me | ms | mq;
        const unsigned long long mv = __ballot(id != WF_INVALID);
        unsigned br = 0, bp = 0;
        if (lane == 0) {
            if (mv & ~mq) *moved = 1u;
            if (mp) {
                br = atomicAdd(n_rays_next, (unsigned)(__popcll(me) + __popcll(ms)));
                bp = atomicAdd(n_paths_next, (unsigned)__popcll(mp));
            }
        }
        br = __builtin_amdgcn_readfirstlane(br);
        bp = __builtin_amdgcn_readfirstlane(bp);
        const unsigned pos_next = bp + (unsigned)__popcll(mp & lt_mask);
        const unsigned sidx_next = next_base + pos_next;
        if (push_ext || push_sh || requeue) {
            st_stream(w.A(0, sidx_next), ro);
            st_stream(w.A(1, sidx_next), rd);
            st_stream(w.A(2, sidx_next), st2);
            st_stream(w.A(3, sidx_next), st3);
            if (has4) st_stream(w.A(4, sidx_next), st4);
        }
#ifdef GLRTX_FAULT_INJECT
        if (requeue) {
            *w.H(cur_base + (unsigned)i) = make_float4(kHitSuspended, __uint_as_float(kFaultPoison), 0.f, 0.f);
            *w.H(sidx_next) = make_float4(kHitSuspended, 0.f, 0.f, 0.f);
        }
#else
        if (requeue) *w.H(cur_base + (unsigned)i) = make_float4(kHitSuspended, __uint_as_float(sidx_next * 2u), 0.f, 0.f);
#endif
        if (push_ext) {
            float4 *r = rq_next + 2 * (size_t)(br + __popcll(me & lt_mask));
            r[0] = make_float4(ro.x, ro.y, ro.z, __uint_as_float(sidx_next * 2u));
            r[1] = make_float4(rd.x, rd.y, rd.z, 0.f);
        }
        if (push_sh) {
            float4 *r = rq_next + 2 * (size_t)(br + __popcll(me) + __popcll(ms & lt_mask));
            r[0] = make_float4(ro.x, ro.y, ro.z, __uint_as_float(pos_next * 2u + 1u));
            r[1] = rsd;
        }
    }
}

struct WgwfKernArgs {
    KernelArgs a;
    WfArgs w;
    unsigned *work_counter;
    float4 *wg_queues;
    const int *adapt_list;
    const unsigned *adapt_count;
    VolArgs vol;
};
DEV const WgwfKernArgs *wgwf_kernargs() {
    auto p = __builtin_amdgcn_kernarg_segment_ptr();
    asm volatile("" : "+s"(p));
    return (const WgwfKernArgs *)p;
}

DEV int wgwf_suspend_max() { return wgwf_kernargs()->w.suspend_max; }
DEV const VolArgs *wgwf_vol() { return &wgwf_kernargs()->vol; }

template <bool VOL = false>
DEV void wg_feed_topup(int kWgPaths, unsigned *ctl, int cur, unsigned *work_counter) {
    const WgwfKernArgs *k = wgwf_kernargs();
    FeedHost *fh = k->w.feed_host;
    FeedDev *fd = k->w.feed_dev;
    int lane = threadIdx.x;
    if constexpr (VOL) asm volatile("" : "+v"(lane));
    const int tpf = k->w.tiles_per_frame, gss_div = k->w.gss_div;
    const int np = (int)ctl[4 + cur];
    const bool may_take = ctl[7] == 0u && ctl[13] == 0u;
    int want = (kWgPaths - np) >> 6;
    unsigned kw = __hip_atomic_load(&fd->frames_known, __ATOMIC_RELAXED, __HIP_MEMORY_SCOPE_AGENT);
    int known = (int)(kw & ~kFeedClosed);
    bool closed = (kw & kFeedClosed) != 0u;
    const int done = (int)__hip_atomic_load(work_counter, __ATOMIC_RELAXED, __HIP_MEMORY_SCOPE_AGENT);
    unsigned wg_id = blockIdx.x;
    asm volatile("" : "+s"(wg_id));
    const bool looker = (wg_id & 31u) == 0u || np == 0;
    if (looker && may_take && want > 0 && !closed && known * tpf - done < k->w.feed_margin) {
        unsigned v = 0u;
        if (lane == 0) v = __hip_atomic_load(&fh->frames_pub, __ATOMIC_RELAXED, __HIP_MEMORY_SCOPE_SYSTEM);
        v = (unsigned)__builtin_amdgcn_readfirstlane((int)v);
        int pub = (int)(v & ~kFeedClosed);
        pub = pub > kFeedMaxFrames ? kFeedMaxFrames : pub;
        if (pub > known) {
            for (int f = known + lane; f < pub; f += 64) {
                const float sx = __hip_atomic_load(&fh->seeds[f].x, __ATOMIC_RELAXED, __HIP_MEMORY_SCOPE_SYSTEM), sy = __hip_atomic_load(&fh->seeds[f].y, __ATOMIC_RELAXED, __HIP_MEMORY_SCOPE_SYSTEM);
                __hip_atomic_store(&fd->seeds[f], (unsigned long long)__float_as_uint(sx) | ((unsigned long long)__float_as_uint(sy) << 32), __ATOMIC_RELAXED, __HIP_MEMORY_SCOPE_AGENT);
            }
            for (int c = known / kFeedChunkFrames + lane; c <= (pub - 1) / kFeedChunkFrames; c += 64) {
                unsigned long long ptr = __hip_atomic_load(reinterpret_cast<unsigned long long *>(&fh->chunks[c]), __ATOMIC_RELAXED, __HIP_MEMORY_SCOPE_SYSTEM);
                __hip_atomic_store(&fd->chunks[c], ptr, __ATOMIC_RELAXED, __HIP_MEMORY_SCOPE_AGENT);
            }
            __builtin_amdgcn_fence(__ATOMIC_RELEASE, "agent");
            __builtin_amdgcn_wave_barrier();
            if (lane == 0) __hip_atomic_fetch_max(&fd->frames_known, (unsigned)pub, __ATOMIC_RELAXED, __HIP_MEMORY_SCOPE_AGENT);
            known = pub;
        }
        if ((v & kFeedClosed) != 0u && pub == known) {
            if (lane == 0) __hip_atomic_fetch_max(&fd->frames_known, (unsigned)known | kFeedClosed, __ATOMIC_RELAXED, __HIP_MEMORY_SCOPE_AGENT);
            closed = true;
        }
    }
    if (known != (int)ctl[18]) {
        __builtin_amdgcn_fence(__ATOMIC_ACQUIRE, "agent");
        if (lane == 0) ctl[18] = (unsigned)known;
    }
    if (lane != 0) return;
    const int n_tiles = known * tpf;
    if (want > 0 && gss_div > 0) {
        const int left = n_tiles - done;
        const int share = left > 0 ? (left + gss_div - 1) / gss_div : 1;
        want = want < share ? want : share;
    }
    int base = 0, got = 0;
    unsigned p_lo = ctl[16], p_hi = ctl[17];
    if (may_take) {
        if (p_lo < p_hi) {
            const int v_hi = (int)p_hi < n_tiles ? (int)p_hi : n_tiles;
            if ((int)p_lo < v_hi) { base = (int)p_lo; got = v_hi - (int)p_lo; p_lo += (unsigned)got; }
        } else if (want > 0 && !closed) {
            base = (int)atomicAdd(work_counter, (unsigned)want);
            const int hi = base + want;
            const int v_hi = hi < n_tiles ? hi : (base < n_tiles ? n_tiles : base);
            got = v_hi - base;
            if (hi > v_hi) { p_lo = (unsigned)v_hi; p_hi = (unsigned)hi; }
        }
    }
    unsigned again = 0u;
    if (may_take && got == 0 && np == 0) {
        if (!closed) {
            unsigned expect = (unsigned)known;
            if (__hip_atomic_compare_exchange_strong(&fh->frames_pub, &expect, (unsigned)known | kFeedClosed, __ATOMIC_RELAXED, __ATOMIC_RELAXED, __HIP_MEMORY_SCOPE_SYSTEM) ||
                expect == ((unsigned)known | kFeedClosed)) {
                __hip_atomic_fetch_max(&fd->frames_known, (unsigned)known | kFeedClosed, __ATOMIC_RELAXED, __HIP_MEMORY_SCOPE_AGENT);
                closed = true;
            } else again = 1u;
        }
    }
    const unsigned turns = again ? ctl[15] + 1u : 0u;
    ctl[15] = turns;
    if (turns > 4096u) {
        unsigned *e = k->w.err;
        __hip_atomic_store(e + 1, (unsigned)known, __ATOMIC_RELAXED, __HIP_MEMORY_SCOPE_SYSTEM);
        __hip_atomic_store(e + 2, turns, __ATOMIC_RELAXED, __HIP_MEMORY_SCOPE_SYSTEM);
        __hip_atomic_store(e + 3, 0u, __ATOMIC_RELAXED, __HIP_MEMORY_SCOPE_SYSTEM);
        __hip_atomic_store(e, 3u, __ATOMIC_RELAXED, __HIP_MEMORY_SCOPE_SYSTEM);
        ctl[13] = 1u;
        again = 0u;
    }
    if (closed && (int)p_lo >= n_tiles) { ctl[7] = 1u; p_lo = p_hi = 0u; }
    ctl[16] = p_lo; ctl[17] = p_hi;
    ctl[0] = (unsigned)base; ctl[6] = (unsigned)got; ctl[14] = again;
    if (np > 0) ctl[12] = got > 0 ? 0u : ctl[12] + 1u;
}

constexpr int kWgwfAdaptive = 4;
template <bool COUNT_RAYS, bool VINE, int FETCH = 0>
__global__ __launch_bounds__(kBlockThreads, GLRTX_WGWF_WAVES) void pt_render_wgwf(const KernelArgs a, const WfArgs w, unsigned *work_counter, float4 *wg_queues,
                                                                                  const int * , const unsigned * , const VolArgs ) {
    constexpr bool ADAPT = (FETCH & kWgwfAdaptive) != 0;
    constexpr bool VOL = (FETCH & kWgwfVolume) != 0;
    constexpr int NODE_FETCH = FETCH & ~(kWgwfAdaptive | kWgwfVolume);
    static_assert(!VOL || (!VINE && NODE_FETCH == 0), "the V form has the one-record-per-lane fetch on DevScene::nodes only");
    extern __shared__ __attribute__((aligned(16))) unsigned char lds_raw[];
    float4 *lds_mats = reinterpret_cast<float4 *>(lds_raw);
    const int mat_f4 = a.sc.lds_head_f4;
    unsigned char *pl = lds_raw + (size_t)mat_f4 * sizeof(float4);
    int *stack = reinterpret_cast<int *>(pl) + 2 * threadIdx.x;
    pl += (size_t)2 * a.sc.stack_entries * kBlockThreads * sizeof(int);
    unsigned *ctl = reinterpret_cast<unsigned *>(pl);
    float4 *lds_root = reinterpret_cast<float4 *>(pl + kWgCtlWords * sizeof(unsigned));
    float *lds_cam = reinterpret_cast<float *>(pl + kWgCtlWords * sizeof(unsigned) + 32);
    unsigned *light_bits = reinterpret_cast<unsigned *>(pl + kWgCtlWords * sizeof(unsigned) + 32 + kCamFloatsPadded * 4 + kLdsSeeds * 8);
    if (threadIdx.x < kCamFloats) lds_cam[threadIdx.x] = a.cam[threadIdx.x];
    if (w.seeds_in_lds && (int)threadIdx.x < 2 * w.n_frames) lds_cam[kCamFloatsPadded + threadIdx.x] = reinterpret_cast<const float *>(w.seeds)[threadIdx.x];
    if (threadIdx.x == 64) lds_root[0] = a.sc.root_lo;
    if (threadIdx.x == 65) lds_root[1] = a.sc.root_hi;
    float4 *rayQ = wg_queues + (size_t)blockIdx.x * kWgQueueF4;
    if (a.sc.mats_in_lds) stage_mats(a, lds_mats);
    stage_lights(a, lds_mats);
    if (FETCH & kWgwfCompact) {
        uint2 *lds_ranks = reinterpret_cast<uint2 *>(light_bits + kWgPathsMax / 32);
        for (int i = threadIdx.x; i < a.sc.n_crank; i += kBlockThreads) lds_ranks[i] = a.sc.cranks[i];
    }

    const int kWgPaths = w.block_paths;
    unsigned long long rays = 0;
#ifdef GLRTX_PHASE_STATS
    if (threadIdx.x == 0 && (blockIdx.x & 63) == 0 && blockIdx.x / 64 < 16)
        g_trip_log[blockIdx.x / 64][0].y = (unsigned)(__builtin_amdgcn_s_memtime() >> 4);
#endif
    if (threadIdx.x == 0) { ctl[2] = 0u; ctl[3] = 0u; ctl[4] = 0u; ctl[5] = 0u; ctl[7] = 0u; ctl[10] = 0u; ctl[11] = 0u; ctl[12] = 0u; ctl[13] = 0u; ctl[14] = 0u; ctl[15] = 0u; ctl[16] = 0u; ctl[17] = 0u; ctl[18] = 0u; }
    if (!VINE) rayQ[kWgSuspendAt + (size_t)kSuspendF4 * threadIdx.x + 3] = make_float4(0.f, 0.f, 0.f, 0.f);
    int cur = 0;
    __syncthreads();
    for (;;) {
        PH_STAMP(pg0);
        unsigned tid_topup = threadIdx.x;
        asm volatile("" : "+v"(tid_topup));
        if (wgwf_kernargs()->w.feed_dev != nullptr) {
            if (tid_topup < 64u) wg_feed_topup<VOL>(kWgPaths, ctl, cur, work_counter);
        } else if (tid_topup == 0u) {
            const int n_tiles = (ADAPT ? (int)*wgwf_kernargs()->adapt_count : wgwf_kernargs()->w.tiles_per_frame) * wgwf_kernargs()->w.n_frames;
            int want = (kWgPaths - (int)ctl[4 + cur]) >> 6;
            int base = 0, got = 0;
            const int gss_div = wgwf_kernargs()->w.gss_div;
            if (want > 0 && ctl[7] == 0u && gss_div > 0) {
                const int left = n_tiles - (int)__hip_atomic_load(work_counter, __ATOMIC_RELAXED, __HIP_MEMORY_SCOPE_AGENT);
                const int share = left > 0 ? (left + gss_div - 1) / gss_div : 1;
                want = want < share ? want : share;
            }
            if (want > 0 && ctl[7] == 0u && ctl[13] == 0u) {
                base = (int)atomicAdd(work_counter, (unsigned)want);
                got = base < n_tiles ? (want < n_tiles - base ? want : n_tiles - base) : 0;
                if (base + want >= n_tiles) ctl[7] = 1u;
            }
            ctl[0] = (unsigned)base; ctl[6] = (unsigned)got; ctl[14] = 0u;
            ctl[12] = got > 0 ? 0u : ctl[12] + 1u;
        }
        __syncthreads();
        if (ctl[13] != 0u) break;
        const bool look_again = ctl[14] != 0u;
        {
            const int got = (int)ctl[6] * 64, tile0 = (int)ctl[0];
            {
                unsigned tid = threadIdx.x;
                asm volatile("" : "+v"(tid));
                if (tid < kWgPathsMax / 32) light_bits[tid] = 0u;
            }
            const int nr = (int)ctl[2 + cur], np = (int)ctl[4 + cur];
            float4 *rq_w = rayQ + 2 * ((size_t)cur * 2 * kWgPaths + nr);
            const WgwfKernArgs *kt = wgwf_kernargs();
            const unsigned new_base = kt->w.set_base(cur, (int)blockIdx.x) + (unsigned)np;
            for (int k = threadIdx.x; k < got; k += kBlockThreads) {
                int id = tile0 * 64 + k;
                if (ADAPT) {
                    const int g = tile0 + (k >> 6), n_active = (int)*kt->adapt_count;
                    const int frame = g / n_active;
                    id = frame * kt->w.total + kt->adapt_list[g - frame * n_active] * 64 + (k & 63);
                }
                float4 ro = make_float4(0.f, 0.f, 0.f, __uint_as_float(WF_INVALID)), rd = ro;
                const bool go = wf_generate_one(kt->a, kt->w, lds_cam, id, new_base + (unsigned)k, ro, rd);
                rq_w[2 * k] = ro;
                rq_w[2 * k + 1] = rd;
                (void)go;
            }
            __syncthreads();
            if (tid_topup == 0u) { ctl[2 + cur] = (unsigned)(nr + got); ctl[4 + cur] = (unsigned)(np + got); ctl[1] = 0u; }
        }
        __syncthreads();
        PH_STAMP(pg1);
        PH_ADD(0, pg0, pg1);
        const int n_rays = (int)ctl[2 + cur], n_paths = (int)ctl[4 + cur];
        if (n_paths == 0) {
            if (look_again) continue;
            break;
        }
        const float4 *rq = rayQ + 2 * ((size_t)cur * 2 * kWgPaths);

#ifdef GLRTX_RAY_LOG
        if (g_ray_log.on) {
            if (threadIdx.x == 0) {
                const unsigned long long base = atomicAdd(&g_ray_log_n, (unsigned long long)n_rays);
                ctl[9] = 0u;
                if (base + (unsigned long long)n_rays <= g_ray_log.cap_rays) {
                    const unsigned t = atomicAdd(&g_ray_log_trips, 1u);
                    if (t < g_ray_log.cap_trips) { g_ray_log.trips[t] = make_uint2((unsigned)base, (unsigned)n_rays); ctl[8] = (unsigned)base; ctl[9] = 1u; }
                }
            }
            __syncthreads();
            if (ctl[9]) {
                float4 *dst = g_ray_log.rays + 2 * (size_t)ctl[8];
                for (int i = threadIdx.x; i < 2 * n_rays; i += kBlockThreads) dst[i] = rq[i];
            }
            __syncthreads();
        }
#endif
        PH_STAMP(pt0);
        __builtin_amdgcn_s_setprio(GLRTX_PRIO_TRAVERSE);
        wg_traverse_phase<VINE, NODE_FETCH>(a, w, lds_root, stack, rq, n_rays, &ctl[1], light_bits, rays, rayQ + kWgSuspendAt);
        __builtin_amdgcn_s_setprio(GLRTX_PRIO_SHADE);
        PH_STAMP(pt1);
        __syncthreads();
        PH_STAMP(pt2);
        PH_ADD(1, pt0, pt1);
        PH_ADD(2, pt1, pt2);

        const WgwfKernArgs *ks = wgwf_kernargs();
        wg_shade_phase<VOL>(ks->a, ks->w, lds_mats, lds_cam, light_bits, n_paths, rayQ + 2 * ((size_t)(cur ^ 1) * 2 * kWgPaths),
                            &ctl[2 + (cur ^ 1)], &ctl[4 + (cur ^ 1)], ks->w.set_base(cur, (int)blockIdx.x), ks->w.set_base(cur ^ 1, (int)blockIdx.x), rays, &ctl[10]);
        PH_STAMP(ps1);
        __syncthreads();
        PH_STAMP(ps2);
        PH_ADD(3, pt2, ps1);
        PH_ADD(4, ps1, ps2);
#ifdef GLRTX_PHASE_STATS
        if (threadIdx.x == 0 && (blockIdx.x & 63) == 0 && blockIdx.x / 64 < 16) {
            uint4 *lg = g_trip_log[blockIdx.x / 64];
            const unsigned n = lg[0].x + 1u;
            if (n < 64u) { lg[n] = make_uint4((unsigned)n_rays, (unsigned)n_paths, (unsigned)(pt2 - pt0), (unsigned)(ps2 - pt2)); lg[0].x = n; }
        }
#endif
        unsigned tid_end = threadIdx.x;
        asm volatile("" : "+v"(tid_end));
        if (tid_end == 0u) {
            ctl[2 + cur] = 0u; ctl[4 + cur] = 0u;
            const bool idle = n_rays == 0 && ctl[10] == 0u;
            ctl[10] = 0u;
            const unsigned idle_trips = idle ? ctl[11] + 1u : 0u;
            ctl[11] = idle_trips;
            const WgwfKernArgs *kg = wgwf_kernargs();
            const unsigned code = idle_trips >= 2u ? 1u : (ctl[12] > (unsigned)kg->w.trip_limit ? 2u : 0u);
            if (code != 0u) {
                unsigned *e = kg->w.err;
                unsigned wg;
                asm volatile("v_mov_b32 %0, %1" : "=v"(wg) : "s"((unsigned)blockIdx.x));
                __hip_atomic_store(e + 1, wg, __ATOMIC_RELAXED, __HIP_MEMORY_SCOPE_SYSTEM);
                __hip_atomic_store(e + 2, ctl[12], __ATOMIC_RELAXED, __HIP_MEMORY_SCOPE_SYSTEM);
                __hip_atomic_store(e + 3, ctl[4 + (cur ^ 1)], __ATOMIC_RELAXED, __HIP_MEMORY_SCOPE_SYSTEM);
                __hip_atomic_store(e, code, __ATOMIC_RELEASE, __HIP_MEMORY_SCOPE_SYSTEM);
                ctl[13] = 1u;
            }
        }
        cur ^= 1;
    }
#ifdef GLRTX_PHASE_STATS
    if (threadIdx.x == 0 && (blockIdx.x & 63) == 0 && blockIdx.x / 64 < 16)
        g_trip_log[blockIdx.x / 64][0].z = (unsigned)(__builtin_amdgcn_s_memtime() >> 4);
#endif
    flush_rays<COUNT_RAYS>(a, rays);
}

#ifdef GLRTX_RAY_LOG
template <int FETCH>
__global__ __launch_bounds__(kBlockThreads, GLRTX_WGWF_WAVES) void pt_replay_traverse(const KernelArgs a, const WfArgs w, unsigned *work_counter, float4 *wg_queues,
                                                                                      const float4 *log, const uint2 *trips, int n_trips) {
    extern __shared__ __attribute__((aligned(16))) unsigned char lds_raw[];
    const int mat_f4 = a.sc.lds_head_f4;
    unsigned char *pl = lds_raw + (size_t)mat_f4 * sizeof(float4);
    int *stack = reinterpret_cast<int *>(pl) + 2 * threadIdx.x;
    pl += (size_t)2 * a.sc.stack_entries * kBlockThreads * sizeof(int);
    unsigned *ctl = reinterpret_cast<unsigned *>(pl);
    float4 *lds_root = reinterpret_cast<float4 *>(pl + kWgCtlWords * sizeof(unsigned));
    unsigned *light_bits = reinterpret_cast<unsigned *>(pl + kWgCtlWords * sizeof(unsigned) + 32 + kCamFloatsPadded * 4 + kLdsSeeds * 8);
    if (threadIdx.x == 64) lds_root[0] = a.sc.root_lo;
    if (threadIdx.x == 65) lds_root[1] = a.sc.root_hi;
    float4 *rayQ = wg_queues + (size_t)blockIdx.x * kWgQueueF4;
    rayQ[kWgSuspendAt + (size_t)kSuspendF4 * threadIdx.x + 3] = make_float4(0.f, 0.f, 0.f, 0.f);
    unsigned long long rays = 0;
    __syncthreads();
    for (;;) {
        if (threadIdx.x == 0) { ctl[0] = atomicAdd(work_counter, 1u); ctl[1] = 0u; }
        if (threadIdx.x < kWgPathsMax / 32) light_bits[threadIdx.x] = 0u;
        __syncthreads();
        const unsigned t = ctl[0];
        if (t >= (unsigned)n_trips) break;
        const uint2 tr = trips[t];
        __builtin_amdgcn_s_setprio(GLRTX_PRIO_TRAVERSE);
        wg_traverse_phase<false, FETCH>(a, w, lds_root, stack, log + 2 * (size_t)tr.x, (int)tr.y, &ctl[1], light_bits, rays, rayQ + kWgSuspendAt);
        __builtin_amdgcn_s_setprio(GLRTX_PRIO_SHADE);
        __syncthreads();
    }
    flush_rays<true>(a, rays);
}
#endif


constexpr float kAdaptLumFloor = 1e-3f;
constexpr int kAdaptCompactThreads = 1024;

__global__ __launch_bounds__(256) void adaptive_select_kernel(const float4 *accum, const float4 *half, int pitch_f4, int width, int rows, int tiles8_x, int n_tiles,
                                                              float threshold, int min_samples, unsigned char *mask, float *tile_err) {
    const int tile = blockIdx.x * 4 + (threadIdx.x >> 6), k = threadIdx.x & 63;
    if (tile >= n_tiles) return;
    const int x = (tile % tiles8_x) * 8 + (k & 7), y = (tile / tiles8_x) * 8 + (k >> 3);
    const bool in = x < width && y < rows;
    float d = 0.0f;
    bool force = false;
    if (in) {
        const size_t at = (size_t)y * pitch_f4 + x;
        const float4 c = ld_stream(&accum[at]), h = ld_stream(&half[at]);
        force = c.w < (float)min_samples || h.w == 0.0f;
        const float ir = c.x / c.w, ig = c.y / c.w, ib = c.z / c.w;
        const float ar = h.x / h.w, ag = h.y / h.w, ab = h.z / h.w;
        const float num = (__builtin_fabsf(ir - ar) + __builtin_fabsf(ig - ag)) + __builtin_fabsf(ib - ab);
        d = num / __builtin_sqrtf(((ir + ig) + ib) + kAdaptLumFloor);
    }
#pragma unroll
    for (int h = 32; h >= 1; h >>= 1) d = d + __shfl_xor(d, h, 64);
    const unsigned long long in_mask = __ballot(in), force_mask = __ballot(force);
    if (k == 0) {
        const float e = d / (float)__popcll(in_mask);
// ... 126 lines not shown
```

opengl-raytracer_amd/csrc/trav_asm.hip.h:

```cpp
#pragma once

#ifndef GLRTX_STEPS_PER_TRIP
#define GLRTX_STEPS_PER_TRIP 6
#endif
#ifndef GLRTX_ASM_VBASE
#define GLRTX_ASM_VBASE 96
#endif
static_assert(GLRTX_STEPS_PER_TRIP % 2 == 0, "the alternating form of the node fetch unrolls steps in pairs");
#define GLRTX_STEPS_PER_TRIP_HALF_(n) GLRTX_HALF_##n
#define GLRTX_HALF_2 1
#define GLRTX_HALF_4 2
#define GLRTX_HALF_6 3
#define GLRTX_HALF_8 4
#define GLRTX_STEPS_PER_TRIP_HALF_X(n) GLRTX_STEPS_PER_TRIP_HALF_(n)
#define GLRTX_STEPS_PER_TRIP_HALF GLRTX_STEPS_PER_TRIP_HALF_X(GLRTX_STEPS_PER_TRIP)
#define GLRTX_STR_(x) #x
#define GLRTX_STR(x) GLRTX_STR_(x)
#define GLRTX_ASM_SET_VBASE ".set GLRTX_VB, " GLRTX_STR(GLRTX_ASM_VBASE) "\n\t"
#if GLRTX_ASM_VBASE == 96
#define GLRTX_ASM_VCLOBBERS "v96", "v97", "v98", "v99", "v100", "v101", "v102", "v103", "v104", "v105", "v106", "v107", "v108", "v109", "v110", "v111", "v112", "v113", "v114", "v115", "v116", "v117"
#define GLRTX_ASM_VCLOBBERS_PAIR GLRTX_ASM_VCLOBBERS, "v118", "v119"
#define GLRTX_ASM_VCLOBBERS_COMPACT GLRTX_ASM_VCLOBBERS_PAIR
#elif GLRTX_ASM_VBASE == 72
#define GLRTX_ASM_VCLOBBERS "v72", "v73", "v74", "v75", "v76", "v77", "v78", "v79", "v80", "v81", "v82", "v83", "v84", "v85", "v86", "v87", "v88", "v89", "v90", "v91", "v92", "v93"
#define GLRTX_ASM_VCLOBBERS_PAIR GLRTX_ASM_VCLOBBERS, "v94", "v95"
#define GLRTX_ASM_VCLOBBERS_COMPACT GLRTX_ASM_VCLOBBERS_PAIR
#else
#error "GLRTX_ASM_VBASE: add the clobber list for this base"
#endif

#ifdef GLRTX_STEP_TIMING
#define GLRTX_TS_BEGIN "s_memtime s[90:91]\n\t"
#define GLRTX_TS_WAIT0 "s_memtime s[92:93]\n\t"
#define GLRTX_TS_WAIT1 "s_memtime s[94:95]\n\ts_waitcnt lgkmcnt(0)\n\ts_sub_u32 s92, s94, s92\n\t"
#define GLRTX_TS_END "s_memtime s[94:95]\n\ts_waitcnt lgkmcnt(0)\n\ts_sub_u32 s94, s94, s90\n\tv_add_u32 %[tt], s94, %[tt]\n\tv_add_u32 %[tw], s92, %[tw]\n\tv_add_u32 %[tn], 1, %[tn]\n\t"
#else
#define GLRTX_TS_BEGIN
#define GLRTX_TS_WAIT0
#define GLRTX_TS_WAIT1
#define GLRTX_TS_END
#endif


#if defined(GLRTX_STEP_TIMING)
#define GLRTX_SINGLE_WAIT
#endif
#ifndef GLRTX_SINGLE_WAIT
#define GLRTX_W3 "s_waitcnt vmcnt(3)\n\t"
#define GLRTX_W2 "s_waitcnt vmcnt(2)\n\t"
#define GLRTX_W1 "s_waitcnt vmcnt(1)\n\t"
#define GLRTX_W0 "s_waitcnt vmcnt(0)\n\t"
#else
#define GLRTX_W3 "s_waitcnt vmcnt(0)\n\t"
#define GLRTX_W2
#define GLRTX_W1
#define GLRTX_W0
#endif
#define GLRTX_TRAV_STEP_ASM_PAIR \
    GLRTX_TS_BEGIN \
    "s_andn2_b64 %[tmp], %[act], %[odd]\n\t"    \
    "s_lshl_b64 %[tmp], %[tmp], 1\n\t" \
    "s_and_b64 %[pop], %[act], %[odd]\n\t" \
    "s_lshr_b64 %[pop], %[pop], 1\n\t" \
    "s_or_b64 %[tmp], %[tmp], %[pop]\n\t" \
    "s_or_b64 %[pop], %[tmp], %[act]\n\t"    \
    "s_mov_b64 exec, %[pop]\n\t" \
    "v_cndmask_b32_e64 v[GLRTX_VB+4], -1, %[cur], %[act]\n\t"    \
    "v_cmp_gt_i32_e64 %[leaf], 0, %[cur]\n\t"    \
    "s_nop 0\n\t"    \
    "v_mov_b32_dpp v[GLRTX_VB+15], v[GLRTX_VB+4] quad_perm:[0,0,2,2] row_mask:0xf bank_mask:0xf\n\t"    \
    "v_mov_b32_dpp v[GLRTX_VB+23], v[GLRTX_VB+4] quad_perm:[1,1,3,3] row_mask:0xf bank_mask:0xf\n\t"    \
    "v_lshl_add_u32 v[GLRTX_VB+15], v[GLRTX_VB+15], 6, %[biase]\n\t"    \
    "v_lshl_add_u32 v[GLRTX_VB+23], v[GLRTX_VB+23], 6, %[biaso]\n\t"    \
    "global_load_dwordx4 v[GLRTX_VB+0:GLRTX_VB+3], v[GLRTX_VB+15], %[base]\n\t" \
    "global_load_dwordx4 v[GLRTX_VB+16:GLRTX_VB+19], v[GLRTX_VB+23], %[base]\n\t" \
    "global_load_dwordx3 v[GLRTX_VB+8:GLRTX_VB+10], v[GLRTX_VB+15], %[base] offset:32\n\t" \
    "global_load_dwordx3 v[GLRTX_VB+20:GLRTX_VB+22], v[GLRTX_VB+23], %[base] offset:32\n\t" \
    GLRTX_TS_WAIT0 "s_waitcnt vmcnt(2)\n\t" GLRTX_TS_WAIT1 \
    "v_cndmask_b32_e64 v[GLRTX_VB+4], v[GLRTX_VB+16], v[GLRTX_VB+0], %[odd]\n\t"    \
    "v_cndmask_b32_e64 v[GLRTX_VB+5], v[GLRTX_VB+17], v[GLRTX_VB+1], %[odd]\n\t" \
    "v_cndmask_b32_e64 v[GLRTX_VB+6], v[GLRTX_VB+18], v[GLRTX_VB+2], %[odd]\n\t" \
    "v_cndmask_b32_e64 v[GLRTX_VB+7], v[GLRTX_VB+19], v[GLRTX_VB+3], %[odd]\n\t" \
    "v_cndmask_b32_e64 v[GLRTX_VB+0], v[GLRTX_VB+0], v[GLRTX_VB+16], %[odd]\n\t"    \
    "v_cndmask_b32_e64 v[GLRTX_VB+1], v[GLRTX_VB+1], v[GLRTX_VB+17], %[odd]\n\t" \
    "v_cndmask_b32_e64 v[GLRTX_VB+2], v[GLRTX_VB+2], v[GLRTX_VB+18], %[odd]\n\t" \
    "v_cndmask_b32_e64 v[GLRTX_VB+3], v[GLRTX_VB+3], v[GLRTX_VB+19], %[odd]\n\t" \
    "v_mov_b32_dpp v[GLRTX_VB+4], v[GLRTX_VB+4] quad_perm:[1,0,3,2] row_mask:0xf bank_mask:0xf\n\t"    \
    "v_mov_b32_dpp v[GLRTX_VB+5], v[GLRTX_VB+5] quad_perm:[1,0,3,2] row_mask:0xf bank_mask:0xf\n\t" \
    "v_mov_b32_dpp v[GLRTX_VB+6], v[GLRTX_VB+6] quad_perm:[1,0,3,2] row_mask:0xf bank_mask:0xf\n\t" \
    "v_mov_b32_dpp v[GLRTX_VB+7], v[GLRTX_VB+7] quad_perm:[1,0,3,2] row_mask:0xf bank_mask:0xf\n\t" \
    "s_andn2_b64 exec, %[act], %[leaf]\n\t"    \
    "v_sub_f32 v[GLRTX_VB+0], v[GLRTX_VB+0], %[ox]\n\t"       \
    "v_sub_f32 v[GLRTX_VB+1], v[GLRTX_VB+1], %[oy]\n\t"                                                            \
    "v_sub_f32 v[GLRTX_VB+2], v[GLRTX_VB+2], %[oz]\n\t"                                                            \
    "v_mul_f32 v[GLRTX_VB+0], v[GLRTX_VB+0], %[ix]\n\t"                                                            \
    "v_mul_f32 v[GLRTX_VB+1], v[GLRTX_VB+1], %[iy]\n\t"                                                            \
    "v_mul_f32 v[GLRTX_VB+2], v[GLRTX_VB+2], %[iz]\n\t"                                                            \
    "v_sub_f32 v[GLRTX_VB+4], v[GLRTX_VB+4], %[ox]\n\t"                                                            \
    "v_sub_f32 v[GLRTX_VB+5], v[GLRTX_VB+5], %[oy]\n\t"                                                            \
    "v_sub_f32 v[GLRTX_VB+6], v[GLRTX_VB+6], %[oz]\n\t"                                                            \
    "v_mul_f32 v[GLRTX_VB+4], v[GLRTX_VB+4], %[ix]\n\t"                                                            \
    "v_mul_f32 v[GLRTX_VB+5], v[GLRTX_VB+5], %[iy]\n\t"                                                            \
    "v_mul_f32 v[GLRTX_VB+6], v[GLRTX_VB+6], %[iz]\n\t"                                                            \
    "v_max_f32 v[GLRTX_VB+16], v[GLRTX_VB+4], v[GLRTX_VB+0]\n\t"                                                                                                                    \
    "v_min_f32 v[GLRTX_VB+0], v[GLRTX_VB+4], v[GLRTX_VB+0]\n\t"                                                                                                                     \
    "v_max_f32 v[GLRTX_VB+17], v[GLRTX_VB+5], v[GLRTX_VB+1]\n\t"                                                                                                                    \
    "v_min_f32 v[GLRTX_VB+1], v[GLRTX_VB+5], v[GLRTX_VB+1]\n\t"                                                                                                                     \
    "v_max_f32 v[GLRTX_VB+18], v[GLRTX_VB+6], v[GLRTX_VB+2]\n\t"                                                                                                                    \
    "v_min_f32 v[GLRTX_VB+4], v[GLRTX_VB+6], v[GLRTX_VB+2]\n\t"                                                                                                                    \
    "v_min3_f32 v[GLRTX_VB+16], v[GLRTX_VB+16], v[GLRTX_VB+17], v[GLRTX_VB+18]\n\t"                                                                                                    \
    "v_max3_f32 v[GLRTX_VB+2], v[GLRTX_VB+0], v[GLRTX_VB+1], v[GLRTX_VB+4]\n\t"                                              \
    "v_min_f32 v[GLRTX_VB+16], v[GLRTX_VB+16], %[th]\n\t"                                                                                                                  \
    "v_cmp_ge_f32_e64 %[bl], v[GLRTX_VB+16], v[GLRTX_VB+2]\n\t"                                                                                   \
    "s_mov_b64 exec, %[pop]\n\t"    \
    "s_waitcnt vmcnt(0)\n\t" \
    "v_cndmask_b32_e64 v[GLRTX_VB+12], v[GLRTX_VB+20], v[GLRTX_VB+8], %[odd]\n\t"    \
    "v_cndmask_b32_e64 v[GLRTX_VB+13], v[GLRTX_VB+21], v[GLRTX_VB+9], %[odd]\n\t" \
    "v_cndmask_b32_e64 v[GLRTX_VB+14], v[GLRTX_VB+22], v[GLRTX_VB+10], %[odd]\n\t" \
    "v_cndmask_b32_e64 v[GLRTX_VB+8], v[GLRTX_VB+8], v[GLRTX_VB+20], %[odd]\n\t"    \
    "v_cndmask_b32_e64 v[GLRTX_VB+9], v[GLRTX_VB+9], v[GLRTX_VB+21], %[odd]\n\t" \
    "v_cndmask_b32_e64 v[GLRTX_VB+10], v[GLRTX_VB+10], v[GLRTX_VB+22], %[odd]\n\t" \
    "v_mov_b32_dpp v[GLRTX_VB+12], v[GLRTX_VB+12] quad_perm:[1,0,3,2] row_mask:0xf bank_mask:0xf\n\t"    \
    "v_mov_b32_dpp v[GLRTX_VB+13], v[GLRTX_VB+13] quad_perm:[1,0,3,2] row_mask:0xf bank_mask:0xf\n\t" \
    "v_mov_b32_dpp v[GLRTX_VB+14], v[GLRTX_VB+14] quad_perm:[1,0,3,2] row_mask:0xf bank_mask:0xf\n\t" \
    "s_andn2_b64 exec, %[act], %[leaf]\n\t"    \
    "v_sub_f32 v[GLRTX_VB+8], v[GLRTX_VB+8], %[ox]\n\t"       \
    "v_sub_f32 v[GLRTX_VB+9], v[GLRTX_VB+9], %[oy]\n\t"                                                            \
    "v_sub_f32 v[GLRTX_VB+10], v[GLRTX_VB+10], %[oz]\n\t"                                                            \
    "v_mul_f32 v[GLRTX_VB+8], v[GLRTX_VB+8], %[ix]\n\t"                                                            \
    "v_mul_f32 v[GLRTX_VB+9], v[GLRTX_VB+9], %[iy]\n\t"                                                            \
    "v_mul_f32 v[GLRTX_VB+10], v[GLRTX_VB+10], %[iz]\n\t"                                                            \
    "v_sub_f32 v[GLRTX_VB+12], v[GLRTX_VB+12], %[ox]\n\t"                                                            \
    "v_sub_f32 v[GLRTX_VB+13], v[GLRTX_VB+13], %[oy]\n\t"                                                            \
    "v_sub_f32 v[GLRTX_VB+14], v[GLRTX_VB+14], %[oz]\n\t"                                                            \
    "v_mul_f32 v[GLRTX_VB+12], v[GLRTX_VB+12], %[ix]\n\t"                                                            \
    "v_mul_f32 v[GLRTX_VB+13], v[GLRTX_VB+13], %[iy]\n\t"                                                            \
    "v_mul_f32 v[GLRTX_VB+14], v[GLRTX_VB+14], %[iz]\n\t"                                                            \
    "v_max_f32 v[GLRTX_VB+16], v[GLRTX_VB+12], v[GLRTX_VB+8]\n\t"                                                                                                                   \
    "v_min_f32 v[GLRTX_VB+8], v[GLRTX_VB+12], v[GLRTX_VB+8]\n\t"                                                                                                                   \
    "v_max_f32 v[GLRTX_VB+17], v[GLRTX_VB+13], v[GLRTX_VB+9]\n\t"                                                                                                                   \
    "v_min_f32 v[GLRTX_VB+9], v[GLRTX_VB+13], v[GLRTX_VB+9]\n\t"                                                                                                                   \
    "v_max_f32 v[GLRTX_VB+18], v[GLRTX_VB+14], v[GLRTX_VB+10]\n\t"                                                                                                                   \
    "v_min_f32 v[GLRTX_VB+10], v[GLRTX_VB+14], v[GLRTX_VB+10]\n\t"                                                                                                                   \
    "v_min3_f32 v[GLRTX_VB+16], v[GLRTX_VB+16], v[GLRTX_VB+17], v[GLRTX_VB+18]\n\t"                                                                                                            \
    "v_max3_f32 v[GLRTX_VB+8], v[GLRTX_VB+8], v[GLRTX_VB+9], v[GLRTX_VB+10]\n\t"                                                                                                            \
    "v_min_f32 v[GLRTX_VB+16], v[GLRTX_VB+16], %[th]\n\t"                                                                                                                  \
    "v_cmp_ge_f32_e64 %[br], v[GLRTX_VB+16], v[GLRTX_VB+8]\n\t" \
    GLRTX_TRAV_STEP_TAIL
#define GLRTX_TRAV_LANE_LOADS \
    "v_lshl_add_u32 v[GLRTX_VB+15], %[cur], 6, %[bias]\n\t"                                                                                                      \
    "global_load_dwordx4 v[GLRTX_VB+0:GLRTX_VB+3], v[GLRTX_VB+15], %[base]\n\t"                                                                                                  \
    "global_load_dwordx4 v[GLRTX_VB+4:GLRTX_VB+7], v[GLRTX_VB+15], %[base] offset:16\n\t"                                                                                      \
    "global_load_dwordx3 v[GLRTX_VB+8:GLRTX_VB+10], v[GLRTX_VB+15], %[base] offset:32\n\t"                                                                                      \
    "global_load_dwordx3 v[GLRTX_VB+12:GLRTX_VB+14], v[GLRTX_VB+15], %[base] offset:48\n\t"
#define GLRTX_TRAV_LANE_CLASSIFY \
    "v_cmp_gt_i32_e64 %[leaf], 0, %[cur]\n\t"                                                                                 \
    "s_andn2_b64 exec, exec, %[leaf]\n\t"
#define GLRTX_TRAV_LANE_FORK \
    GLRTX_TS_WAIT0 GLRTX_W3 GLRTX_TS_WAIT1                                                                                                    \
    "v_sub_f32 v[GLRTX_VB+0], v[GLRTX_VB+0], %[ox]\n\t"       \
    "v_sub_f32 v[GLRTX_VB+1], v[GLRTX_VB+1], %[oy]\n\t"                                                            \
    "v_sub_f32 v[GLRTX_VB+2], v[GLRTX_VB+2], %[oz]\n\t"                                                            \
    "v_mul_f32 v[GLRTX_VB+0], v[GLRTX_VB+0], %[ix]\n\t"                                                            \
    "v_mul_f32 v[GLRTX_VB+1], v[GLRTX_VB+1], %[iy]\n\t"                                                            \
    "v_mul_f32 v[GLRTX_VB+2], v[GLRTX_VB+2], %[iz]\n\t"                                                            \
    GLRTX_W2                                                                                                                        \
    "v_sub_f32 v[GLRTX_VB+4], v[GLRTX_VB+4], %[ox]\n\t"                                                            \
    "v_sub_f32 v[GLRTX_VB+5], v[GLRTX_VB+5], %[oy]\n\t"                                                            \
    "v_sub_f32 v[GLRTX_VB+6], v[GLRTX_VB+6], %[oz]\n\t"                                                            \
    "v_mul_f32 v[GLRTX_VB+4], v[GLRTX_VB+4], %[ix]\n\t"                                                            \
    "v_mul_f32 v[GLRTX_VB+5], v[GLRTX_VB+5], %[iy]\n\t"                                                            \
    "v_mul_f32 v[GLRTX_VB+6], v[GLRTX_VB+6], %[iz]\n\t"                                                            \
    "v_max_f32 v[GLRTX_VB+16], v[GLRTX_VB+4], v[GLRTX_VB+0]\n\t"                                                                                                                    \
    "v_min_f32 v[GLRTX_VB+0], v[GLRTX_VB+4], v[GLRTX_VB+0]\n\t"                                                                                                                     \
    "v_max_f32 v[GLRTX_VB+17], v[GLRTX_VB+5], v[GLRTX_VB+1]\n\t"                                                                                                                    \
    "v_min_f32 v[GLRTX_VB+1], v[GLRTX_VB+5], v[GLRTX_VB+1]\n\t"                                                                                                                     \
    "v_max_f32 v[GLRTX_VB+18], v[GLRTX_VB+6], v[GLRTX_VB+2]\n\t"                                                                                                                    \
    "v_min_f32 v[GLRTX_VB+4], v[GLRTX_VB+6], v[GLRTX_VB+2]\n\t"                                                                                                                    \
    "v_min3_f32 v[GLRTX_VB+16], v[GLRTX_VB+16], v[GLRTX_VB+17], v[GLRTX_VB+18]\n\t"                                                                                                    \
    "v_max3_f32 v[GLRTX_VB+2], v[GLRTX_VB+0], v[GLRTX_VB+1], v[GLRTX_VB+4]\n\t"                                              \
    "v_min_f32 v[GLRTX_VB+16], v[GLRTX_VB+16], %[th]\n\t"                                                                                                                  \
    "v_cmp_ge_f32_e64 %[bl], v[GLRTX_VB+16], v[GLRTX_VB+2]\n\t"                                                                                   \
    GLRTX_W1                                                                                                                        \
    "v_sub_f32 v[GLRTX_VB+8], v[GLRTX_VB+8], %[ox]\n\t"       \
    "v_sub_f32 v[GLRTX_VB+9], v[GLRTX_VB+9], %[oy]\n\t"                                                            \
    "v_sub_f32 v[GLRTX_VB+10], v[GLRTX_VB+10], %[oz]\n\t"                                                            \
    "v_mul_f32 v[GLRTX_VB+8], v[GLRTX_VB+8], %[ix]\n\t"                                                            \
    "v_mul_f32 v[GLRTX_VB+9], v[GLRTX_VB+9], %[iy]\n\t"                                                            \
    "v_mul_f32 v[GLRTX_VB+10], v[GLRTX_VB+10], %[iz]\n\t"                                                            \
    GLRTX_W0                                                                                                                        \
    "v_sub_f32 v[GLRTX_VB+12], v[GLRTX_VB+12], %[ox]\n\t"                                                            \
    "v_sub_f32 v[GLRTX_VB+13], v[GLRTX_VB+13], %[oy]\n\t"                                                            \
    "v_sub_f32 v[GLRTX_VB+14], v[GLRTX_VB+14], %[oz]\n\t"                                                            \
    "v_mul_f32 v[GLRTX_VB+12], v[GLRTX_VB+12], %[ix]\n\t"                                                            \
    "v_mul_f32 v[GLRTX_VB+13], v[GLRTX_VB+13], %[iy]\n\t"                                                            \
    "v_mul_f32 v[GLRTX_VB+14], v[GLRTX_VB+14], %[iz]\n\t"                                                            \
    "v_max_f32 v[GLRTX_VB+16], v[GLRTX_VB+12], v[GLRTX_VB+8]\n\t"                                                                                                                   \
    "v_min_f32 v[GLRTX_VB+8], v[GLRTX_VB+12], v[GLRTX_VB+8]\n\t"                                                                                                                   \
    "v_max_f32 v[GLRTX_VB+17], v[GLRTX_VB+13], v[GLRTX_VB+9]\n\t"                                                                                                                   \
    "v_min_f32 v[GLRTX_VB+9], v[GLRTX_VB+13], v[GLRTX_VB+9]\n\t"                                                                                                                   \
    "v_max_f32 v[GLRTX_VB+18], v[GLRTX_VB+14], v[GLRTX_VB+10]\n\t"                                                                                                                   \
    "v_min_f32 v[GLRTX_VB+10], v[GLRTX_VB+14], v[GLRTX_VB+10]\n\t"                                                                                                                   \
    "v_min3_f32 v[GLRTX_VB+16], v[GLRTX_VB+16], v[GLRTX_VB+17], v[GLRTX_VB+18]\n\t"                                                                                                            \
    "v_max3_f32 v[GLRTX_VB+8], v[GLRTX_VB+8], v[GLRTX_VB+9], v[GLRTX_VB+10]\n\t"                                                                                                            \
    "v_min_f32 v[GLRTX_VB+16], v[GLRTX_VB+16], %[th]\n\t"                                                                                                                  \
    "v_cmp_ge_f32_e64 %[br], v[GLRTX_VB+16], v[GLRTX_VB+8]\n\t"
#define GLRTX_TRAV_STEP_ASM_LANE GLRTX_TS_BEGIN GLRTX_TRAV_LANE_LOADS GLRTX_TRAV_LANE_CLASSIFY GLRTX_TRAV_LANE_FORK GLRTX_TRAV_STEP_TAIL
#ifndef GLRTX_SINGLE_WAIT
#define GLRTX_CW2 "s_waitcnt vmcnt(2)\n\t"
#define GLRTX_CW1 "s_waitcnt vmcnt(1)\n\t"
#define GLRTX_CW0 "s_waitcnt vmcnt(0)\n\t"
#else
#define GLRTX_CW2 "s_waitcnt vmcnt(0)\n\t"
#define GLRTX_CW1
#define GLRTX_CW0
#endif
#define GLRTX_TRAV_STEP_ASM_COMPACT \
    GLRTX_TS_BEGIN \
    "v_lshrrev_b32 v[GLRTX_VB+23], 5, %[cur]\n\t"                                    \
    "v_lshl_add_u32 v[GLRTX_VB+23], v[GLRTX_VB+23], 3, %[rk]\n\t" \
    "ds_read_b64 v[GLRTX_VB+20:GLRTX_VB+21], v[GLRTX_VB+23]\n\t" \
    "v_mul_u32_u24 v[GLRTX_VB+15], 48, %[cur]\n\t"                                   \
    "global_load_dwordx4 v[GLRTX_VB+0:GLRTX_VB+3], v[GLRTX_VB+15], %[cbase]\n\t" \
    "global_load_dwordx4 v[GLRTX_VB+4:GLRTX_VB+7], v[GLRTX_VB+15], %[cbase] offset:16\n\t" \
    "global_load_dwordx4 v[GLRTX_VB+8:GLRTX_VB+11], v[GLRTX_VB+15], %[cbase] offset:32\n\t" \
    "s_waitcnt lgkmcnt(0)\n\t" \
    "v_bfe_u32 v[GLRTX_VB+19], v[GLRTX_VB+20], %[cur], 1\n\t"                        \
    "v_cmp_eq_u32_e64 %[leaf], 0, v[GLRTX_VB+19]\n\t"                                \
    "v_bfm_b32 v[GLRTX_VB+19], %[cur], 0\n\t"                                        \
    "v_and_b32 v[GLRTX_VB+19], v[GLRTX_VB+19], v[GLRTX_VB+20]\n\t" \
    "v_bcnt_u32_b32 v[GLRTX_VB+19], v[GLRTX_VB+19], v[GLRTX_VB+21]\n\t"              \
    "s_andn2_b64 exec, exec, %[leaf]\n\t"                                            \
    GLRTX_TS_WAIT0 GLRTX_CW2 GLRTX_TS_WAIT1 \
    "v_sub_f32 v[GLRTX_VB+0], v[GLRTX_VB+0], %[ox]\n\t"    \
    "v_sub_f32 v[GLRTX_VB+1], v[GLRTX_VB+1], %[oy]\n\t" \
    "v_sub_f32 v[GLRTX_VB+2], v[GLRTX_VB+2], %[oz]\n\t" \
    "v_mul_f32 v[GLRTX_VB+0], v[GLRTX_VB+0], %[ix]\n\t" \
    "v_mul_f32 v[GLRTX_VB+1], v[GLRTX_VB+1], %[iy]\n\t" \
    "v_mul_f32 v[GLRTX_VB+2], v[GLRTX_VB+2], %[iz]\n\t" \
    GLRTX_CW1 \
    "v_sub_f32 v[GLRTX_VB+4], v[GLRTX_VB+4], %[ox]\n\t" \
    "v_sub_f32 v[GLRTX_VB+5], v[GLRTX_VB+5], %[oy]\n\t" \
    "v_sub_f32 v[GLRTX_VB+6], v[GLRTX_VB+6], %[oz]\n\t" \
    "v_mul_f32 v[GLRTX_VB+4], v[GLRTX_VB+4], %[ix]\n\t" \
    "v_mul_f32 v[GLRTX_VB+5], v[GLRTX_VB+5], %[iy]\n\t" \
    "v_mul_f32 v[GLRTX_VB+6], v[GLRTX_VB+6], %[iz]\n\t" \
    "v_max_f32 v[GLRTX_VB+16], v[GLRTX_VB+4], v[GLRTX_VB+0]\n\t" \
    "v_min_f32 v[GLRTX_VB+0], v[GLRTX_VB+4], v[GLRTX_VB+0]\n\t" \
    "v_max_f32 v[GLRTX_VB+17], v[GLRTX_VB+5], v[GLRTX_VB+1]\n\t" \
    "v_min_f32 v[GLRTX_VB+1], v[GLRTX_VB+5], v[GLRTX_VB+1]\n\t" \
    "v_max_f32 v[GLRTX_VB+18], v[GLRTX_VB+6], v[GLRTX_VB+2]\n\t" \
    "v_min_f32 v[GLRTX_VB+4], v[GLRTX_VB+6], v[GLRTX_VB+2]\n\t" \
    "v_min3_f32 v[GLRTX_VB+16], v[GLRTX_VB+16], v[GLRTX_VB+17], v[GLRTX_VB+18]\n\t"    \
    "v_max3_f32 v[GLRTX_VB+2], v[GLRTX_VB+0], v[GLRTX_VB+1], v[GLRTX_VB+4]\n\t"        \
    "v_min_f32 v[GLRTX_VB+16], v[GLRTX_VB+16], %[th]\n\t" \
    "v_cmp_ge_f32_e64 %[bl], v[GLRTX_VB+16], v[GLRTX_VB+2]\n\t"                      \
    GLRTX_CW0 \
    "v_sub_f32 v[GLRTX_VB+8], v[GLRTX_VB+8], %[ox]\n\t"    \
    "v_sub_f32 v[GLRTX_VB+9], v[GLRTX_VB+9], %[oy]\n\t" \
    "v_sub_f32 v[GLRTX_VB+10], v[GLRTX_VB+10], %[oz]\n\t" \
    "v_mul_f32 v[GLRTX_VB+8], v[GLRTX_VB+8], %[ix]\n\t" \
    "v_mul_f32 v[GLRTX_VB+9], v[GLRTX_VB+9], %[iy]\n\t" \
    "v_mul_f32 v[GLRTX_VB+10], v[GLRTX_VB+10], %[iz]\n\t" \
    "v_sub_f32 v[GLRTX_VB+12], v[GLRTX_VB+3], %[ox]\n\t" \
    "v_sub_f32 v[GLRTX_VB+13], v[GLRTX_VB+7], %[oy]\n\t" \
    "v_sub_f32 v[GLRTX_VB+14], v[GLRTX_VB+11], %[oz]\n\t" \
    "v_mul_f32 v[GLRTX_VB+12], v[GLRTX_VB+12], %[ix]\n\t" \
    "v_mul_f32 v[GLRTX_VB+13], v[GLRTX_VB+13], %[iy]\n\t" \
    "v_mul_f32 v[GLRTX_VB+14], v[GLRTX_VB+14], %[iz]\n\t" \
    "v_max_f32 v[GLRTX_VB+16], v[GLRTX_VB+12], v[GLRTX_VB+8]\n\t" \
    "v_min_f32 v[GLRTX_VB+8], v[GLRTX_VB+12], v[GLRTX_VB+8]\n\t" \
    "v_max_f32 v[GLRTX_VB+17], v[GLRTX_VB+13], v[GLRTX_VB+9]\n\t" \
    "v_min_f32 v[GLRTX_VB+9], v[GLRTX_VB+13], v[GLRTX_VB+9]\n\t" \
    "v_max_f32 v[GLRTX_VB+18], v[GLRTX_VB+14], v[GLRTX_VB+10]\n\t" \
    "v_min_f32 v[GLRTX_VB+10], v[GLRTX_VB+14], v[GLRTX_VB+10]\n\t" \
    "v_min3_f32 v[GLRTX_VB+16], v[GLRTX_VB+16], v[GLRTX_VB+17], v[GLRTX_VB+18]\n\t" \
    "v_max3_f32 v[GLRTX_VB+8], v[GLRTX_VB+8], v[GLRTX_VB+9], v[GLRTX_VB+10]\n\t" \
    "v_min_f32 v[GLRTX_VB+16], v[GLRTX_VB+16], %[th]\n\t" \
    "v_cmp_ge_f32_e64 %[br], v[GLRTX_VB+16], v[GLRTX_VB+8]\n\t" \
    "v_lshl_add_u32 v[GLRTX_VB+3], v[GLRTX_VB+19], 1, 1\n\t"                         \
    "v_add_u32 v[GLRTX_VB+7], 1, v[GLRTX_VB+3]\n\t"                                  \
    GLRTX_TRAV_STEP_TAIL_X("", "v[GLRTX_VB+22]")
#define GLRTX_TRAV_STEP_TAIL GLRTX_TRAV_STEP_TAIL_X("v_not_b32 v[GLRTX_VB+3], %[cur]\n\t", "v[GLRTX_VB+11]")
#define GLRTX_TRAV_STEP_TAIL_X(TRI, FIN) \
    "v_cndmask_b32_e64 %[cur], v[GLRTX_VB+3], v[GLRTX_VB+7], %[br]\n\t"                                  \
    "s_or_b64 %[tmp], %[bl], %[br]\n\t"                                                                                                                \
    "s_andn2_b64 %[pop], exec, %[tmp]\n\t"                                                                     \
    "s_and_b64 exec, %[bl], %[br]\n\t"                                                               \
    "v_lshl_add_u32 v[GLRTX_VB+15], %[sp], 11, %[stk]\n\t"                                                                                                       \
    "ds_write_b64 v[GLRTX_VB+15], v[GLRTX_VB+2:GLRTX_VB+3]\n\t"                                                                                                                  \
    "v_add_u32 %[sp], 1, %[sp]\n\t"                                                                                                                    \
    "s_and_b64 exec, %[act], %[leaf]\n\t"                                \
    "s_cbranch_scc0 21f\n\t"                                                                                                                           \
    TRI                                                                                                                                      \
    "v_mov_b32 %[cur], v[GLRTX_VB+7]\n\t"                                                   \
    "v_mul_f32 v[GLRTX_VB+16], %[dy], v[GLRTX_VB+10]\n\t"                                                                                                  \
    "v_mul_f32 v[GLRTX_VB+19], %[dz], v[GLRTX_VB+9]\n\t"                                                                                                                  \
    "v_sub_f32 v[GLRTX_VB+16], v[GLRTX_VB+16], v[GLRTX_VB+19]\n\t"                                                                                                                   \
    "v_mul_f32 v[GLRTX_VB+17], %[dz], v[GLRTX_VB+8]\n\t"                                                                                                                  \
    "v_mul_f32 v[GLRTX_VB+19], %[dx], v[GLRTX_VB+10]\n\t"                                                                                                                  \
    "v_sub_f32 v[GLRTX_VB+17], v[GLRTX_VB+17], v[GLRTX_VB+19]\n\t"                                                                                                                   \
    "v_mul_f32 v[GLRTX_VB+18], %[dx], v[GLRTX_VB+9]\n\t"                                                                                                                  \
    "v_mul_f32 v[GLRTX_VB+19], %[dy], v[GLRTX_VB+8]\n\t"                                                                                                                  \
    "v_sub_f32 v[GLRTX_VB+18], v[GLRTX_VB+18], v[GLRTX_VB+19]\n\t"                                                                                                                   \
    "v_mul_f32 v[GLRTX_VB+20], v[GLRTX_VB+6], v[GLRTX_VB+18]\n\t"                                                                          \
    "v_mul_f32 v[GLRTX_VB+19], v[GLRTX_VB+5], v[GLRTX_VB+17]\n\t"                                                                                                                   \
    "v_add_f32 v[GLRTX_VB+20], v[GLRTX_VB+20], v[GLRTX_VB+19]\n\t"                                                                                                                   \
    "v_mul_f32 v[GLRTX_VB+19], v[GLRTX_VB+4], v[GLRTX_VB+16]\n\t"                                                                                                                   \
    "v_add_f32 v[GLRTX_VB+20], v[GLRTX_VB+20], v[GLRTX_VB+19]\n\t"                                                                                                                   \
    "v_rcp_f32 v[GLRTX_VB+21], v[GLRTX_VB+20]\n\t"                                                                                                                         \
    "v_sub_f32 v[GLRTX_VB+0], %[ox], v[GLRTX_VB+0]\n\t"                                                                                          \
    "v_sub_f32 v[GLRTX_VB+1], %[oy], v[GLRTX_VB+1]\n\t"                                                                                                                    \
    "v_sub_f32 v[GLRTX_VB+2], %[oz], v[GLRTX_VB+2]\n\t"                                                                                                                    \
    "v_fma_f32 v[GLRTX_VB+19], -v[GLRTX_VB+20], v[GLRTX_VB+21], 1.0\n\t"                                                           \
    "v_fma_f32 v[GLRTX_VB+21], v[GLRTX_VB+19], v[GLRTX_VB+21], v[GLRTX_VB+21]\n\t"                                                                                                             \
    "v_mul_f32 v[GLRTX_VB+18], v[GLRTX_VB+2], v[GLRTX_VB+18]\n\t"                                                                                   \
    "v_mul_f32 v[GLRTX_VB+19], v[GLRTX_VB+1], v[GLRTX_VB+17]\n\t"                                                                                                                    \
    "v_add_f32 v[GLRTX_VB+18], v[GLRTX_VB+18], v[GLRTX_VB+19]\n\t"                                                                                                                   \
    "v_mul_f32 v[GLRTX_VB+19], v[GLRTX_VB+0], v[GLRTX_VB+16]\n\t"                                                                                                                    \
    "v_add_f32 v[GLRTX_VB+18], v[GLRTX_VB+18], v[GLRTX_VB+19]\n\t"                                                                                                                   \
    "v_mul_f32 v[GLRTX_VB+15], v[GLRTX_VB+18], v[GLRTX_VB+21]\n\t"                                                                                                            \
    "v_cmpx_nlt_f32_e64 %[tmp], |v[GLRTX_VB+20]|, %[eps]\n\t"                                                                    \
    "v_cmpx_ngt_f32 vcc, 0, v[GLRTX_VB+15]\n\t"                                                                                                    \
    "v_cmpx_nlt_f32 vcc, 1.0, v[GLRTX_VB+15]\n\t"                                                                                                  \
    "s_cbranch_execz 20f\n\t"                                                                                                                          \
    "v_mul_f32 v[GLRTX_VB+12], v[GLRTX_VB+1], v[GLRTX_VB+6]\n\t"                                                                                                    \
    "v_mul_f32 v[GLRTX_VB+19], v[GLRTX_VB+2], v[GLRTX_VB+5]\n\t"                                                                                                                    \
    "v_sub_f32 v[GLRTX_VB+12], v[GLRTX_VB+12], v[GLRTX_VB+19]\n\t"                                                                                                                   \
    "v_mul_f32 v[GLRTX_VB+13], v[GLRTX_VB+2], v[GLRTX_VB+4]\n\t"                                                                                                                    \
    "v_mul_f32 v[GLRTX_VB+19], v[GLRTX_VB+0], v[GLRTX_VB+6]\n\t"                                                                                                                    \
    "v_sub_f32 v[GLRTX_VB+13], v[GLRTX_VB+13], v[GLRTX_VB+19]\n\t"                                                                                                                   \
    "v_mul_f32 v[GLRTX_VB+14], v[GLRTX_VB+0], v[GLRTX_VB+5]\n\t"                                                                                                                    \
    "v_mul_f32 v[GLRTX_VB+19], v[GLRTX_VB+1], v[GLRTX_VB+4]\n\t"                                                                                                                    \
    "v_sub_f32 v[GLRTX_VB+14], v[GLRTX_VB+14], v[GLRTX_VB+19]\n\t"                                                                                                                   \
    "v_mul_f32 v[GLRTX_VB+7], %[dz], v[GLRTX_VB+14]\n\t"                                                                                 \
    "v_mul_f32 v[GLRTX_VB+19], %[dy], v[GLRTX_VB+13]\n\t"                                                                                                                  \
    "v_add_f32 v[GLRTX_VB+7], v[GLRTX_VB+7], v[GLRTX_VB+19]\n\t"                                                                                                                   \
    "v_mul_f32 v[GLRTX_VB+19], %[dx], v[GLRTX_VB+12]\n\t"                                                                                                                  \
    "v_add_f32 v[GLRTX_VB+7], v[GLRTX_VB+7], v[GLRTX_VB+19]\n\t"                                                                                                                   \
    "v_mul_f32 v[GLRTX_VB+16], v[GLRTX_VB+7], v[GLRTX_VB+21]\n\t"                                                                                                            \
    "v_add_f32 v[GLRTX_VB+19], v[GLRTX_VB+18], v[GLRTX_VB+7]\n\t"                                                                                                                   \
    "v_mul_f32 v[GLRTX_VB+19], v[GLRTX_VB+21], v[GLRTX_VB+19]\n\t"                                                                       \
    "v_cmpx_ngt_f32 vcc, 0, v[GLRTX_VB+16]\n\t"                                                                                                    \
    "v_cmpx_nlt_f32 vcc, 1.0, v[GLRTX_VB+19]\n\t"                                                                                        \
    "s_cbranch_execz 20f\n\t"                                                                                                                          \
    "v_mul_f32 v[GLRTX_VB+19], v[GLRTX_VB+10], v[GLRTX_VB+14]\n\t"                                                                      \
    "v_mul_f32 v[GLRTX_VB+7], v[GLRTX_VB+9], v[GLRTX_VB+13]\n\t"                                                                                                                   \
    "v_add_f32 v[GLRTX_VB+19], v[GLRTX_VB+19], v[GLRTX_VB+7]\n\t"                                                                                                                   \
    "v_mul_f32 v[GLRTX_VB+7], v[GLRTX_VB+8], v[GLRTX_VB+12]\n\t"                                                                                                                   \
    "v_add_f32 v[GLRTX_VB+19], v[GLRTX_VB+19], v[GLRTX_VB+7]\n\t"                                                                                                                   \
    "v_mul_f32 v[GLRTX_VB+19], v[GLRTX_VB+19], v[GLRTX_VB+21]\n\t"                                                                                                                   \
    "v_cmpx_nge_f32 vcc, %[eps], v[GLRTX_VB+19]\n\t"                                                                                            \
    "v_cmpx_lt_f32 vcc, v[GLRTX_VB+19], %[th]\n\t"                                                 \
    "v_mov_b32 %[tri], v[GLRTX_VB+3]\n\t"                                                                                                                        \
    "v_mov_b32 %[hu], v[GLRTX_VB+15]\n\t"                                                                                                                        \
    "v_mov_b32 %[hv], v[GLRTX_VB+16]\n\t"                                                                                                                        \
    "v_mov_b32 %[th], v[GLRTX_VB+19]\n\t"                                                                                                                        \
    "20:\n\t"                                                                                                                                          \
    "s_and_b64 exec, %[act], %[leaf]\n\t"                                                                                   \
    "v_sub_f32 v[GLRTX_VB+16], %[sd], %[th]\n\t"                                                            \
    "v_cmp_nle_f32 vcc, %[eps], v[GLRTX_VB+16]\n\t"                                                               \
    "v_cndmask_b32 %[cur], " FIN ", %[cur], vcc\n\t"                       \
    "v_cmp_eq_u32_e64 %[tmp], %[cur], " FIN "\n\t"                                                                                                       \
    "s_and_b64 vcc, vcc, %[tmp]\n\t"                                                            \
    "s_or_b64 %[pop], %[pop], vcc\n\t"                                                                                                                \
    "21:\n\t"                                                                                                                                          \
    "s_mov_b64 exec, %[pop]\n\t"                                         \
    "s_cbranch_execz 30f\n\t"                                                                                                                          \
    "10:\n\t"                                                                                                                                          \
    "v_cmp_ne_u32 vcc, 0, %[sp]\n\t"                                                                                                                   \
    "v_cndmask_b32 %[cur], " FIN ", %[cur], vcc\n\t"                                                                \
    "s_and_b64 exec, exec, vcc\n\t"                                                                                                                    \
    "s_cbranch_execz 30f\n\t"                                                                                                                          \
    "v_add_u32 %[sp], -1, %[sp]\n\t"                                                                                                                   \
    "v_lshl_add_u32 v[GLRTX_VB+15], %[sp], 11, %[stk]\n\t"                                                                                                       \
    "ds_read_b64 v[GLRTX_VB+16:GLRTX_VB+17], v[GLRTX_VB+15]\n\t"                                                                                                  \
    "s_waitcnt lgkmcnt(0)\n\t"                                                                                                                         \
    "v_mov_b32 %[cur], v[GLRTX_VB+17]\n\t"                                                                                                                       \
    "v_cmp_gt_f32 vcc, v[GLRTX_VB+16], %[th]\n\t"                                                                                                                \
    "s_and_b64 exec, exec, vcc\n\t"                                                                                                                    \
    "s_cbranch_execnz 10b\n\t"                                                                                                                         \
    "30:\n\t"                                                                                                                                          \
    "s_mov_b64 exec, %[act]\n\t"                                                                                  \
    GLRTX_TS_END                                                                                                                       \
    "v_cmpx_ne_u32_e64 %[act], %[cur], " FIN "\n\t"                                                                             \
    "s_cbranch_execz 99f\n\t"

#define GLRTX_REP1(X) X
#define GLRTX_REP2(X) X X
#define GLRTX_REP3(X) X X X
#define GLRTX_REP4(X) X X X X
#define GLRTX_REP5(X) X X X X X
#define GLRTX_REP6(X) X X X X X X
#define GLRTX_REP7(X) X X X X X X X
#define GLRTX_REP8(X) X X X X X X X X
#define GLRTX_REP_(N, X) GLRTX_REP##N(X)
#define GLRTX_REP(N, X) GLRTX_REP_(N, X)
```

Before: 10310.

## Add drain-mode BVH traversal that prefetches both child nodes when few lanes remain

Adds a drain traversal variant of the compact-layout asm step. It is used once the ray queue is exhausted and at most the suspend threshold of lanes are active. Each step speculatively loads both children's node records while testing the current node, then takes a second dependent step from the prefetched data, which hides memory latency in the tail where few lanes are busy. A no-refill control flag disables suspension once the tile feed is closed and empty, and the lane-rank calculation switches to mbcnt. The cost is extra VGPR clobbers (24 more registers), which may reduce occupancy, plus wasted bandwidth on speculative loads.

Measured after the change: 10260. About the same (-0.5%).

```diff
diff --git a/opengl-raytracer_amd/csrc/glrtx.hip b/opengl-raytracer_amd/csrc/glrtx.hip
--- a/opengl-raytracer_amd/csrc/glrtx.hip
+++ b/opengl-raytracer_amd/csrc/glrtx.hip
@@ -1188,6 +1188,8 @@
     if (const char *v = std::getenv("GLRTX_GSS_DIV")) w.gss_div = std::max(0, std::atoi(v));
     w.suspend_max = kSuspendMax;
     if (const char *v = std::getenv("GLRTX_SUSPEND_MAX")) w.suspend_max = std::max(0, std::min(64, std::atoi(v)));
+    w.drain_lanes = kSuspendMax;
+    if (const char *v = std::getenv("GLRTX_DRAIN_LOOKAHEAD")) { const int m = std::atoi(v); w.drain_lanes = m <= 0 ? 0 : (m >= 2 ? 65 : kSuspendMax); }
     w.trip_limit = (int)std::min<long long>(INT32_MAX, 64ll * std::max(p->n_samples, 1) * (p->max_depth + 2) + 64);
     if (L.k.vol) w.trip_limit = (int)std::min<long long>(INT32_MAX, 64ll * std::max(p->n_samples, 1) * 9 * (p->max_depth + 2) + 64);
     if (const char *v = std::getenv("GLRTX_TRIP_LIMIT")) w.trip_limit = std::max(1, std::atoi(v));
@@ -3415,6 +3417,7 @@
     for (const uint2 &t : tr) logged += t.y;
     DbgLastLaunch L = g_dbg_last;
     L.w.suspend_max = 0;
+    L.w.drain_lanes = 0;
     using RKernel = void (*)(const KernelArgs, const WfArgs, unsigned *, float4 *, const float4 *, const uint2 *, int);
     int fetch = L.fetch;
     if (const char *v = std::getenv("GLRTX_REPLAY_PAIR_FETCH")) fetch = std::max(0, std::min(2, std::atoi(v)));
diff --git a/opengl-raytracer_amd/csrc/pt_kernel.hip.h b/opengl-raytracer_amd/csrc/pt_kernel.hip.h
--- a/opengl-raytracer_amd/csrc/pt_kernel.hip.h
+++ b/opengl-raytracer_amd/csrc/pt_kernel.hip.h
@@ -442,6 +442,7 @@
 #endif
 constexpr int kWgwfCompact = 8;
 constexpr int kWgwfVolume = 16;
+constexpr int kWgwfDrain = 32;
 template <int FETCH>
 DEV void trav_steps_asm(const DevScene &sc, int *stack, Trav &T, unsigned rk GLRTX_TS_PARAM) {
     unsigned long long s_entry, s_act, s_leaf, s_bl, s_br, s_pop, s_tmp;
@@ -450,7 +451,24 @@
     static_assert(REF_FIN == INT32_MIN, "trav_asm.hip.h materialises REF_FIN with v_bfrev_b32 v, 1");
     const unsigned par16 = (threadIdx.x & 1u) << 4;
     const unsigned bias_e = sc.node_bias + par16, bias_o = sc.node_bias + 16u - par16;
-    if constexpr ((FETCH & kWgwfCompact) != 0) {
+    if constexpr (FETCH == (kWgwfCompact | kWgwfDrain)) {
+        unsigned long long s_dsc, s_rest;
+        asm volatile(
+            "s_mov_b64 %[entry], exec\n\t"
+            "s_mov_b64 %[act], exec\n\t"
+            GLRTX_ASM_SET_VBASE
+            GLRTX_REP(GLRTX_STEPS_PER_TRIP_HALF, GLRTX_TRAV_STEP_ASM_DRAIN)
+            "99:\n\t"
+            "s_waitcnt vmcnt(0)\n\t"
+            "s_mov_b64 exec, %[entry]"
+            : [th] "+&v"(T.h.t), [tri] "+&v"(T.h.tri), [hu] "+&v"(T.h.u), [hv] "+&v"(T.h.v), [cur] "+&v"(T.cur), [sp] "+&v"(T.sp),
+              [entry] "=&s"(s_entry), [act] "=&s"(s_act), [leaf] "=&s"(s_leaf), [bl] "=&s"(s_bl), [br] "=&s"(s_br), [pop] "=&s"(s_pop), [tmp] "=&s"(s_tmp),
+              [dsc] "=&s"(s_dsc), [rest] "=&s"(s_rest)
+            : [ox] "v"(T.ox), [oy] "v"(T.oy), [oz] "v"(T.oz), [dx] "v"(T.dx), [dy] "v"(T.dy), [dz] "v"(T.dz), [ix] "v"(T.ix), [iy] "v"(T.iy), [iz] "v"(T.iz),
+              [sd] "v"(T.stop_d), [stk] "v"(stk), [cbase] "s"(sc.cnodes), [rk] "s"(rk), [eps] "s"(PT_EPS)
+            : "vcc", "scc", "memory", GLRTX_ASM_VCLOBBERS_DRAIN);
+        return;
+    } else if constexpr ((FETCH & kWgwfCompact) != 0) {
         static_assert((FETCH & ~kWgwfCompact) == 0, "the compact layout has the one-record-per-lane fetch only");
         asm volatile(
             "s_mov_b64 %[entry], exec\n\t"
@@ -1452,6 +1470,7 @@
     int gss_div;
     int suspend_max;
     int trip_limit;
+    int drain_lanes;
     unsigned *err;
     FeedHost *feed_host;
     FeedDev *feed_dev;
@@ -1775,6 +1794,8 @@
 #endif
 
 DEV int wgwf_suspend_max();
+DEV int wgwf_drain_lanes();
+constexpr int kCtlNoRefill = 19;
 
 template <bool VINE, int FETCH>
 DEV void wg_traverse_phase(const KernelArgs &a, const WfArgs &w, const float4 *root, int *stack, const float4 *rq, int n_rays,
@@ -1801,12 +1822,14 @@
         }
         return;
     }
-    const unsigned long long lt_mask = (1ull << lane) - 1ull;
     const float4 none = make_float4(0.f, 0.f, 0.f, __uint_as_float(WF_INVALID));
     float4 cur_o = none, cur_d = none;
     float cur_ix = 0.f, cur_iy = 0.f, cur_iz = 0.f;
     int cur_pos = 0, cur_cnt = 0;
     auto fetch = [&](float4 &o, float4 &d) -> int {
+        unsigned tid = threadIdx.x;
+        asm volatile("" : "+v"(tid));
+        const int lane = (int)(tid & 63u);
         int base = 0;
         if (lane == 0) base = (int)atomicAdd(ray_head, 64u);
         base = __builtin_amdgcn_readfirstlane(base);
@@ -1826,6 +1849,17 @@
     cur_cnt = fetch(cur_o, cur_d);
     bool exhausted = cur_cnt == 0;
     const bool fetched_any = cur_cnt > 0;
+#if defined(GLRTX_TRAV_STATS) || defined(GLRTX_CXX_STEP) || defined(GLRTX_STEP_TIMING)
+    constexpr bool DRAINABLE = false;
+#else
+    constexpr bool DRAINABLE = (FETCH & kWgwfCompact) != 0;
+#endif
+    bool drain = false;
+    (void)drain;
+    if constexpr (DRAINABLE) {
+        const int drain_lanes = wgwf_drain_lanes();
+        drain = drain_lanes > 64 || (drain_lanes > 0 && cur_cnt < 64);
+    }
     bool active = false;
     bool unsaved = false;
     unsigned rid = 0;
@@ -1884,7 +1918,7 @@
                 const int n = __popcll(idle);
                 const int avail = cur_cnt - cur_pos;
                 const int take = n < avail ? n : avail;
-                const int rank = __popcll(idle & lt_mask);
+                const int rank = (int)__builtin_amdgcn_mbcnt_hi((unsigned)(idle >> 32), __builtin_amdgcn_mbcnt_lo((unsigned)idle, 0u));
                 const int src = (cur_pos + rank) & 63;
                 const float ox = __shfl(cur_o.x, src), oy = __shfl(cur_o.y, src), oz = __shfl(cur_o.z, src);
                 const unsigned new_rid = (unsigned)__shfl((int)__float_as_uint(cur_o.w), src);
@@ -1923,7 +1957,7 @@
         }
         if (exhausted && fetched_any) {
             const unsigned long long ma = __ballot(active);
-            const int suspend_max = wgwf_suspend_max();
+            const int suspend_max = ray_head[kCtlNoRefill - 1] != 0u ? 0 : wgwf_suspend_max();
             if (__ballot(active && (rid & 1u) != 0u) == 0ull && (int)__popcll(ma) <= suspend_max) {
                 if (active) {
                     susp[0] = make_float4(T.ox, T.oy, T.oz, __uint_as_float(rid));
@@ -1938,6 +1972,9 @@
                 break;
             }
         }
+        if constexpr (DRAINABLE) {
+            if (exhausted && !drain) drain = (int)__popcll(__ballot(active)) <= wgwf_drain_lanes();
+        }
 #ifdef GLRTX_PHASE_STATS
         const unsigned long long sb0 = __builtin_amdgcn_s_memtime();
 #endif
@@ -1961,7 +1998,10 @@
 #ifdef GLRTX_STEP_TIMING
             trav_steps_asm<FETCH>(a.sc, stack, T, (unsigned)(uintptr_t)ranks, step_timing);
 #else
-            trav_steps_asm<FETCH>(a.sc, stack, T, (unsigned)(uintptr_t)ranks);
+            if constexpr (DRAINABLE) {
+                if (drain) trav_steps_asm<kWgwfCompact | kWgwfDrain>(a.sc, stack, T, (unsigned)(uintptr_t)ranks);
+                else trav_steps_asm<FETCH>(a.sc, stack, T, (unsigned)(uintptr_t)ranks);
+            } else trav_steps_asm<FETCH>(a.sc, stack, T, (unsigned)(uintptr_t)ranks);
 #endif
             const bool fin = T.cur == REF_FIN;
 #endif
@@ -1996,7 +2036,9 @@
         bool push_ext = false, push_sh = false, requeue = false, has4 = false;
         unsigned id = WF_INVALID;
         float4 ro = make_float4(0.f, 0.f, 0.f, 0.f), rd = ro, rsd = ro, st2 = ro, st3 = ro, st4 = ro;
-        const bool light_accepted = i < n_paths && ((light_bits[i >> 5] >> (i & 31)) & 1u) != 0u;
+        int bit = i;
+        asm volatile("" : "+v"(bit));
+        const bool light_accepted = i < n_paths && ((light_bits[i >> 5] >> (bit & 31)) & 1u) != 0u;
         if (i < n_paths)
             wf_shade_path<VOL>(a, w, lds_mats, cam, id, cur_base + (unsigned)i, light_accepted, push_ext, push_sh, requeue, ro, rd, rsd, st2, st3, st4, has4, rays);
         const unsigned long long me = __ballot(push_ext), ms = __ballot(push_sh), mq = __ballot(requeue), mp = me | ms | mq;
@@ -2057,6 +2099,7 @@
 }
 
 DEV int wgwf_suspend_max() { return wgwf_kernargs()->w.suspend_max; }
+DEV int wgwf_drain_lanes() { return wgwf_kernargs()->w.drain_lanes; }
 DEV const VolArgs *wgwf_vol() { return &wgwf_kernargs()->vol; }
 
 template <bool VOL = false>
@@ -2152,6 +2195,7 @@
     if (closed && (int)p_lo >= n_tiles) { ctl[7] = 1u; p_lo = p_hi = 0u; }
     ctl[16] = p_lo; ctl[17] = p_hi;
     ctl[0] = (unsigned)base; ctl[6] = (unsigned)got; ctl[14] = again;
+    if (ctl[7] != 0u && got == 0) ctl[kCtlNoRefill] = 1u;
     if (np > 0) ctl[12] = got > 0 ? 0u : ctl[12] + 1u;
 }
 
@@ -2191,7 +2235,7 @@
     if (threadIdx.x == 0 && (blockIdx.x & 63) == 0 && blockIdx.x / 64 < 16)
         g_trip_log[blockIdx.x / 64][0].y = (unsigned)(__builtin_amdgcn_s_memtime() >> 4);
 #endif
-    if (threadIdx.x == 0) { ctl[2] = 0u; ctl[3] = 0u; ctl[4] = 0u; ctl[5] = 0u; ctl[7] = 0u; ctl[10] = 0u; ctl[11] = 0u; ctl[12] = 0u; ctl[13] = 0u; ctl[14] = 0u; ctl[15] = 0u; ctl[16] = 0u; ctl[17] = 0u; ctl[18] = 0u; }
+    if (threadIdx.x == 0) { ctl[2] = 0u; ctl[3] = 0u; ctl[4] = 0u; ctl[5] = 0u; ctl[7] = 0u; ctl[10] = 0u; ctl[11] = 0u; ctl[12] = 0u; ctl[13] = 0u; ctl[14] = 0u; ctl[15] = 0u; ctl[16] = 0u; ctl[17] = 0u; ctl[18] = 0u; ctl[kCtlNoRefill] = 0u; }
     if (!VINE) rayQ[kWgSuspendAt + (size_t)kSuspendF4 * threadIdx.x + 3] = make_float4(0.f, 0.f, 0.f, 0.f);
     int cur = 0;
     __syncthreads();
@@ -2218,6 +2262,7 @@
             }
             ctl[0] = (unsigned)base; ctl[6] = (unsigned)got; ctl[14] = 0u;
             ctl[12] = got > 0 ? 0u : ctl[12] + 1u;
+            if (ctl[7] != 0u && got == 0) ctl[kCtlNoRefill] = 1u;
         }
         __syncthreads();
         if (ctl[13] != 0u) break;
@@ -2238,7 +2283,9 @@
                 if (ADAPT) {
                     const int g = tile0 + (k >> 6), n_active = (int)*kt->adapt_count;
                     const int frame = g / n_active;
-                    id = frame * kt->w.total + kt->adapt_list[g - frame * n_active] * 64 + (k & 63);
+                    int kk = k;
+                    asm volatile("" : "+v"(kk));
+                    id = frame * kt->w.total + kt->adapt_list[g - frame * n_active] * 64 + (kk & 63);
                 }
                 float4 ro = make_float4(0.f, 0.f, 0.f, __uint_as_float(WF_INVALID)), rd = ro;
                 const bool go = wf_generate_one(kt->a, kt->w, lds_cam, id, new_base + (unsigned)k, ro, rd);
diff --git a/opengl-raytracer_amd/csrc/trav_asm.hip.h b/opengl-raytracer_amd/csrc/trav_asm.hip.h
--- a/opengl-raytracer_amd/csrc/trav_asm.hip.h
+++ b/opengl-raytracer_amd/csrc/trav_asm.hip.h
@@ -21,10 +21,12 @@
 #define GLRTX_ASM_VCLOBBERS "v96", "v97", "v98", "v99", "v100", "v101", "v102", "v103", "v104", "v105", "v106", "v107", "v108", "v109", "v110", "v111", "v112", "v113", "v114", "v115", "v116", "v117"
 #define GLRTX_ASM_VCLOBBERS_PAIR GLRTX_ASM_VCLOBBERS, "v118", "v119"
 #define GLRTX_ASM_VCLOBBERS_COMPACT GLRTX_ASM_VCLOBBERS_PAIR
+#define GLRTX_ASM_VCLOBBERS_DRAIN GLRTX_ASM_VCLOBBERS, "v72", "v73", "v74", "v75", "v76", "v77", "v78", "v79", "v80", "v81", "v82", "v83", "v84", "v85", "v86", "v87", "v88", "v89", "v90", "v91", "v92", "v93", "v94", "v95"
 #elif GLRTX_ASM_VBASE == 72
 #define GLRTX_ASM_VCLOBBERS "v72", "v73", "v74", "v75", "v76", "v77", "v78", "v79", "v80", "v81", "v82", "v83", "v84", "v85", "v86", "v87", "v88", "v89", "v90", "v91", "v92", "v93"
 #define GLRTX_ASM_VCLOBBERS_PAIR GLRTX_ASM_VCLOBBERS, "v94", "v95"
 #define GLRTX_ASM_VCLOBBERS_COMPACT GLRTX_ASM_VCLOBBERS_PAIR
+#define GLRTX_ASM_VCLOBBERS_DRAIN GLRTX_ASM_VCLOBBERS, "v48", "v49", "v50", "v51", "v52", "v53", "v54", "v55", "v56", "v57", "v58", "v59", "v60", "v61", "v62", "v63", "v64", "v65", "v66", "v67", "v68", "v69", "v70", "v71"
 #else
 #error "GLRTX_ASM_VBASE: add the clobber list for this base"
 #endif
@@ -215,30 +217,15 @@
 #define GLRTX_CW1
 #define GLRTX_CW0
 #endif
-#define GLRTX_TRAV_STEP_ASM_COMPACT \
-    GLRTX_TS_BEGIN \
-    "v_lshrrev_b32 v[GLRTX_VB+23], 5, %[cur]\n\t"                                    \
-    "v_lshl_add_u32 v[GLRTX_VB+23], v[GLRTX_VB+23], 3, %[rk]\n\t" \
-    "ds_read_b64 v[GLRTX_VB+20:GLRTX_VB+21], v[GLRTX_VB+23]\n\t" \
-    "v_mul_u32_u24 v[GLRTX_VB+15], 48, %[cur]\n\t"                                   \
-    "global_load_dwordx4 v[GLRTX_VB+0:GLRTX_VB+3], v[GLRTX_VB+15], %[cbase]\n\t" \
-    "global_load_dwordx4 v[GLRTX_VB+4:GLRTX_VB+7], v[GLRTX_VB+15], %[cbase] offset:16\n\t" \
-    "global_load_dwordx4 v[GLRTX_VB+8:GLRTX_VB+11], v[GLRTX_VB+15], %[cbase] offset:32\n\t" \
-    "s_waitcnt lgkmcnt(0)\n\t" \
-    "v_bfe_u32 v[GLRTX_VB+19], v[GLRTX_VB+20], %[cur], 1\n\t"                        \
-    "v_cmp_eq_u32_e64 %[leaf], 0, v[GLRTX_VB+19]\n\t"                                \
-    "v_bfm_b32 v[GLRTX_VB+19], %[cur], 0\n\t"                                        \
-    "v_and_b32 v[GLRTX_VB+19], v[GLRTX_VB+19], v[GLRTX_VB+20]\n\t" \
-    "v_bcnt_u32_b32 v[GLRTX_VB+19], v[GLRTX_VB+19], v[GLRTX_VB+21]\n\t"              \
-    "s_andn2_b64 exec, exec, %[leaf]\n\t"                                            \
-    GLRTX_TS_WAIT0 GLRTX_CW2 GLRTX_TS_WAIT1 \
+#define GLRTX_TRAV_COMPACT_FORK(WA, WB, WC) \
+    WA \
     "v_sub_f32 v[GLRTX_VB+0], v[GLRTX_VB+0], %[ox]\n\t"    \
     "v_sub_f32 v[GLRTX_VB+1], v[GLRTX_VB+1], %[oy]\n\t" \
     "v_sub_f32 v[GLRTX_VB+2], v[GLRTX_VB+2], %[oz]\n\t" \
     "v_mul_f32 v[GLRTX_VB+0], v[GLRTX_VB+0], %[ix]\n\t" \
     "v_mul_f32 v[GLRTX_VB+1], v[GLRTX_VB+1], %[iy]\n\t" \
     "v_mul_f32 v[GLRTX_VB+2], v[GLRTX_VB+2], %[iz]\n\t" \
-    GLRTX_CW1 \
+    WB \
     "v_sub_f32 v[GLRTX_VB+4], v[GLRTX_VB+4], %[ox]\n\t" \
     "v_sub_f32 v[GLRTX_VB+5], v[GLRTX_VB+5], %[oy]\n\t" \
     "v_sub_f32 v[GLRTX_VB+6], v[GLRTX_VB+6], %[oz]\n\t" \
@@ -255,7 +242,7 @@
     "v_max3_f32 v[GLRTX_VB+2], v[GLRTX_VB+0], v[GLRTX_VB+1], v[GLRTX_VB+4]\n\t"        \
     "v_min_f32 v[GLRTX_VB+16], v[GLRTX_VB+16], %[th]\n\t" \
     "v_cmp_ge_f32_e64 %[bl], v[GLRTX_VB+16], v[GLRTX_VB+2]\n\t"                      \
-    GLRTX_CW0 \
+    WC \
     "v_sub_f32 v[GLRTX_VB+8], v[GLRTX_VB+8], %[ox]\n\t"    \
     "v_sub_f32 v[GLRTX_VB+9], v[GLRTX_VB+9], %[oy]\n\t" \
     "v_sub_f32 v[GLRTX_VB+10], v[GLRTX_VB+10], %[oz]\n\t" \
@@ -279,10 +266,107 @@
     "v_min_f32 v[GLRTX_VB+16], v[GLRTX_VB+16], %[th]\n\t" \
     "v_cmp_ge_f32_e64 %[br], v[GLRTX_VB+16], v[GLRTX_VB+8]\n\t" \
     "v_lshl_add_u32 v[GLRTX_VB+3], v[GLRTX_VB+19], 1, 1\n\t"                         \
-    "v_add_u32 v[GLRTX_VB+7], 1, v[GLRTX_VB+3]\n\t"                                  \
+    "v_add_u32 v[GLRTX_VB+7], 1, v[GLRTX_VB+3]\n\t"
+#define GLRTX_TRAV_STEP_ASM_COMPACT \
+    GLRTX_TS_BEGIN \
+    "v_lshrrev_b32 v[GLRTX_VB+23], 5, %[cur]\n\t"                                    \
+    "v_lshl_add_u32 v[GLRTX_VB+23], v[GLRTX_VB+23], 3, %[rk]\n\t" \
+    "ds_read_b64 v[GLRTX_VB+20:GLRTX_VB+21], v[GLRTX_VB+23]\n\t" \
+    "v_mul_u32_u24 v[GLRTX_VB+15], 48, %[cur]\n\t"                                   \
+    "global_load_dwordx4 v[GLRTX_VB+0:GLRTX_VB+3], v[GLRTX_VB+15], %[cbase]\n\t" \
+    "global_load_dwordx4 v[GLRTX_VB+4:GLRTX_VB+7], v[GLRTX_VB+15], %[cbase] offset:16\n\t" \
+    "global_load_dwordx4 v[GLRTX_VB+8:GLRTX_VB+11], v[GLRTX_VB+15], %[cbase] offset:32\n\t" \
+    "s_waitcnt lgkmcnt(0)\n\t" \
+    "v_bfe_u32 v[GLRTX_VB+19], v[GLRTX_VB+20], %[cur], 1\n\t"                        \
+    "v_cmp_eq_u32_e64 %[leaf], 0, v[GLRTX_VB+19]\n\t"                                \
+    "v_bfm_b32 v[GLRTX_VB+19], %[cur], 0\n\t"                                        \
+    "v_and_b32 v[GLRTX_VB+19], v[GLRTX_VB+19], v[GLRTX_VB+20]\n\t" \
+    "v_bcnt_u32_b32 v[GLRTX_VB+19], v[GLRTX_VB+19], v[GLRTX_VB+21]\n\t"              \
+    "s_andn2_b64 exec, exec, %[leaf]\n\t"                                            \
+    GLRTX_TRAV_COMPACT_FORK(GLRTX_TS_WAIT0 GLRTX_CW2 GLRTX_TS_WAIT1, GLRTX_CW1, GLRTX_CW0) \
     GLRTX_TRAV_STEP_TAIL_X("", "v[GLRTX_VB+22]")
+#define GLRTX_TRAV_STEP_ASM_DRAIN \
+    "v_lshrrev_b32 v[GLRTX_VB+16], 5, %[cur]\n\t"                                    \
+    "v_lshl_add_u32 v[GLRTX_VB+16], v[GLRTX_VB+16], 3, %[rk]\n\t" \
+    "ds_read_b64 v[GLRTX_VB+20:GLRTX_VB+21], v[GLRTX_VB+16]\n\t" \
+    "v_mul_u32_u24 v[GLRTX_VB+15], 48, %[cur]\n\t" \
+    "global_load_dwordx4 v[GLRTX_VB+0:GLRTX_VB+3], v[GLRTX_VB+15], %[cbase]\n\t" \
+    "global_load_dwordx4 v[GLRTX_VB+4:GLRTX_VB+7], v[GLRTX_VB+15], %[cbase] offset:16\n\t" \
+    "global_load_dwordx4 v[GLRTX_VB+8:GLRTX_VB+11], v[GLRTX_VB+15], %[cbase] offset:32\n\t" \
+    "s_waitcnt lgkmcnt(0)\n\t" \
+    "v_bfe_u32 v[GLRTX_VB+19], v[GLRTX_VB+20], %[cur], 1\n\t" \
+    "v_cmp_eq_u32_e64 %[leaf], 0, v[GLRTX_VB+19]\n\t" \
+    "v_bfm_b32 v[GLRTX_VB+19], %[cur], 0\n\t" \
+    "v_and_b32 v[GLRTX_VB+19], v[GLRTX_VB+19], v[GLRTX_VB+20]\n\t" \
+    "v_bcnt_u32_b32 v[GLRTX_VB+19], v[GLRTX_VB+19], v[GLRTX_VB+21]\n\t" \
+    "s_andn2_b64 exec, exec, %[leaf]\n\t"                                            \
+    "v_mul_u32_u24 v[GLRTX_VB+15], 96, v[GLRTX_VB+19]\n\t" \
+    "global_load_dwordx4 v[GLRTX_VB-24:GLRTX_VB-21], v[GLRTX_VB+15], %[cbase] offset:48\n\t" \
+    "global_load_dwordx4 v[GLRTX_VB-20:GLRTX_VB-17], v[GLRTX_VB+15], %[cbase] offset:64\n\t" \
+    "global_load_dwordx4 v[GLRTX_VB-16:GLRTX_VB-13], v[GLRTX_VB+15], %[cbase] offset:80\n\t" \
+    "global_load_dwordx4 v[GLRTX_VB-12:GLRTX_VB-9], v[GLRTX_VB+15], %[cbase] offset:96\n\t" \
+    "global_load_dwordx4 v[GLRTX_VB-8:GLRTX_VB-5], v[GLRTX_VB+15], %[cbase] offset:112\n\t" \
+    "global_load_dwordx4 v[GLRTX_VB-4:GLRTX_VB-1], v[GLRTX_VB+15], %[cbase] offset:128\n\t" \
+    GLRTX_TRAV_COMPACT_FORK(GLRTX_DW8, GLRTX_DW7, GLRTX_DW6)                         \
+    "s_mov_b64 exec, %[act]\n\t"                                                    \
+    "v_bfrev_b32 v[GLRTX_VB+11], 1\n\t"                                             \
+    "s_andn2_b64 exec, %[act], %[leaf]\n\t"                                         \
+    GLRTX_TRAV_STEP_TAIL_BODY("", "v[GLRTX_VB+11]") \
+    "v_cmpx_ne_u32_e64 %[act], %[cur], v[GLRTX_VB+11]\n\t" \
+    "s_cbranch_execz 99f\n\t" \
+    "s_or_b64 %[dsc], %[bl], %[br]\n\t"                                              \
+    "s_cbranch_scc0 40f\n\t" \
+    "s_andn2_b64 %[rest], %[act], %[dsc]\n\t"                                        \
+    "s_mov_b64 %[act], %[dsc]\n\t" \
+    "s_mov_b64 exec, %[dsc]\n\t" \
+    "v_lshrrev_b32 v[GLRTX_VB+16], 5, %[cur]\n\t" \
+    "v_lshl_add_u32 v[GLRTX_VB+16], v[GLRTX_VB+16], 3, %[rk]\n\t" \
+    "ds_read_b64 v[GLRTX_VB+20:GLRTX_VB+21], v[GLRTX_VB+16]\n\t" \
+    "s_waitcnt vmcnt(0)\n\t" \
+    "v_cndmask_b32_e64 v[GLRTX_VB+0], v[GLRTX_VB-24], v[GLRTX_VB-12], %[br]\n\t" \
+    "v_cndmask_b32_e64 v[GLRTX_VB+1], v[GLRTX_VB-23], v[GLRTX_VB-11], %[br]\n\t" \
+    "v_cndmask_b32_e64 v[GLRTX_VB+2], v[GLRTX_VB-22], v[GLRTX_VB-10], %[br]\n\t" \
+    "v_cndmask_b32_e64 v[GLRTX_VB+3], v[GLRTX_VB-21], v[GLRTX_VB-9], %[br]\n\t" \
+    "v_cndmask_b32_e64 v[GLRTX_VB+4], v[GLRTX_VB-20], v[GLRTX_VB-8], %[br]\n\t" \
+    "v_cndmask_b32_e64 v[GLRTX_VB+5], v[GLRTX_VB-19], v[GLRTX_VB-7], %[br]\n\t" \
+    "v_cndmask_b32_e64 v[GLRTX_VB+6], v[GLRTX_VB-18], v[GLRTX_VB-6], %[br]\n\t" \
+    "v_cndmask_b32_e64 v[GLRTX_VB+7], v[GLRTX_VB-17], v[GLRTX_VB-5], %[br]\n\t" \
+    "v_cndmask_b32_e64 v[GLRTX_VB+8], v[GLRTX_VB-16], v[GLRTX_VB-4], %[br]\n\t" \
+    "v_cndmask_b32_e64 v[GLRTX_VB+9], v[GLRTX_VB-15], v[GLRTX_VB-3], %[br]\n\t" \
+    "v_cndmask_b32_e64 v[GLRTX_VB+10], v[GLRTX_VB-14], v[GLRTX_VB-2], %[br]\n\t" \
+    "v_cndmask_b32_e64 v[GLRTX_VB+11], v[GLRTX_VB-13], v[GLRTX_VB-1], %[br]\n\t" \
+    "s_waitcnt lgkmcnt(0)\n\t" \
+    "v_bfe_u32 v[GLRTX_VB+19], v[GLRTX_VB+20], %[cur], 1\n\t" \
+    "v_cmp_eq_u32_e64 %[leaf], 0, v[GLRTX_VB+19]\n\t" \
+    "v_bfm_b32 v[GLRTX_VB+19], %[cur], 0\n\t" \
+    "v_and_b32 v[GLRTX_VB+19], v[GLRTX_VB+19], v[GLRTX_VB+20]\n\t" \
+    "v_bcnt_u32_b32 v[GLRTX_VB+19], v[GLRTX_VB+19], v[GLRTX_VB+21]\n\t" \
+    "s_andn2_b64 exec, exec, %[leaf]\n\t" \
+    GLRTX_TRAV_COMPACT_FORK(, , ) \
+    "s_mov_b64 exec, %[act]\n\t"                                                    \
+    "v_bfrev_b32 v[GLRTX_VB+11], 1\n\t"                                             \
+    "s_andn2_b64 exec, %[act], %[leaf]\n\t"                                         \
+    GLRTX_TRAV_STEP_TAIL_BODY("", "v[GLRTX_VB+11]") \
+    "v_cmp_ne_u32_e64 %[act], %[cur], v[GLRTX_VB+11]\n\t"                            \
+    "s_or_b64 %[act], %[act], %[rest]\n\t" \
+    "40:\n\t" \
+    "s_mov_b64 exec, %[act]\n\t" \
+    "s_cbranch_execz 99f\n\t"
+#ifndef GLRTX_SINGLE_WAIT
+#define GLRTX_DW8 "s_waitcnt vmcnt(8)\n\t"
+#define GLRTX_DW7 "s_waitcnt vmcnt(7)\n\t"
+#define GLRTX_DW6 "s_waitcnt vmcnt(6)\n\t"
+#else
+#define GLRTX_DW8 "s_waitcnt vmcnt(6)\n\t"
+#define GLRTX_DW7
+#define GLRTX_DW6
+#endif
 #define GLRTX_TRAV_STEP_TAIL GLRTX_TRAV_STEP_TAIL_X("v_not_b32 v[GLRTX_VB+3], %[cur]\n\t", "v[GLRTX_VB+11]")
 #define GLRTX_TRAV_STEP_TAIL_X(TRI, FIN) \
+    GLRTX_TRAV_STEP_TAIL_BODY(TRI, FIN) \
+    "v_cmpx_ne_u32_e64 %[act], %[cur], " FIN "\n\t"                                                                             \
+    "s_cbranch_execz 99f\n\t"
+#define GLRTX_TRAV_STEP_TAIL_BODY(TRI, FIN) \
     "v_cndmask_b32_e64 %[cur], v[GLRTX_VB+3], v[GLRTX_VB+7], %[br]\n\t"                                  \
     "s_or_b64 %[tmp], %[bl], %[br]\n\t"                                                                                                                \
     "s_andn2_b64 %[pop], exec, %[tmp]\n\t"                                                                     \
@@ -382,9 +466,7 @@
     "s_cbranch_execnz 10b\n\t"                                                                                                                         \
     "30:\n\t"                                                                                                                                          \
     "s_mov_b64 exec, %[act]\n\t"                                                                                  \
-    GLRTX_TS_END                                                                                                                       \
-    "v_cmpx_ne_u32_e64 %[act], %[cur], " FIN "\n\t"                                                                             \
-    "s_cbranch_execz 99f\n\t"
+    GLRTX_TS_END
 
 #define GLRTX_REP1(X) X
 #define GLRTX_REP2(X) X X
```
